# Chemical118/TREW

Hardware: NVIDIA B200
Metric: Gbases/s for trew short 5 32 at 1/2/4/8 B200; % of HBM roofline (higher is better)
Workload: dtype u64

## Files before the change

### trew_b200/csrc/device_ctx.cu

```cuda
#include <algorithm>
#include <chrono>
#include <cstdarg>
#include <cstdio>
#include <cstdlib>
#include <cstring>
#include <string>
#include <thread>
#include <vector>

#include <cuda_runtime.h>

#include "host_internal.h"
#include "scan_kernels.cuh"

using namespace trew;

namespace {

struct SlotRes {
    void* h_buf = nullptr;
    void* d_buf = nullptr;
    unsigned char* h_inv = nullptr;
    unsigned char* d_inv = nullptr;
    size_t inv_cap = 0;
    unsigned int* h_keys = nullptr;
    unsigned int* d_survivors = nullptr;
    unsigned int* d_counters = nullptr;
    unsigned char* d_scratch = nullptr;
    size_t scratch_bytes = 0;
    size_t survivors_cap = 0;
    cudaStream_t stream = nullptr;
    cudaEvent_t ev_start = nullptr, ev_done = nullptr;
    bool in_flight = false;
};

struct RangeInfo { uint32_t r0, r1; uint64_t bases; uint32_t max_len; };

}

struct trew_resident {
    void* d_buf = nullptr;
    DevBatch batch{};
    uint32_t n_reads = 0, n_units = 0, max_read_len = 0;
    uint64_t bases = 0;
    unsigned int* d_survivors = nullptr;
    unsigned int* d_counters = nullptr;
    unsigned char* d_scratch = nullptr;
    size_t scratch_bytes = 0;
    cudaEvent_t ev[4] = {nullptr, nullptr, nullptr, nullptr};
    bool ev_pending = false;
};

struct trew_ctx {
    trew_config cfg{};
    int sm_count = 0;
    LaunchPlan plan{};
    cudaStream_t aux_stream = nullptr;
    cudaEvent_t ev_join = nullptr;
    int resident_streams = 1;
    uint64_t resident_seq = 0;
    DevCfg dcfg{};
    size_t n_slots = 0;
    unsigned int* d_error = nullptr;
    unsigned short* d_thr = nullptr;
    unsigned long long* d_total_surv = nullptr;
    std::vector<SlotRes> slots;
    size_t next_slot = 0;
    size_t staging_bytes = 0;
    cudaStream_t main_stream = nullptr;
    cudaEvent_t ev_a = nullptr, ev_b = nullptr;
    trew_entry* d_entries = nullptr; size_t d_entries_cap = 0;
    trew_entry* d_sorted = nullptr; size_t d_sorted_cap = 0;
    trew_entry* d_concat = nullptr; size_t d_concat_cap = 0;
    bool sorted_valid = false;
    void* d_sort_tmp = nullptr; size_t sort_tmp_bytes = 0;
    unsigned int* d_n = nullptr;
    uint64_t n_export = 0;
    bool export_valid = false;
    trew_stats stats{};
    Pool* pool = nullptr;
    bool own_pool = true;
    std::string err;
    std::vector<RangeInfo> ranges_tmp;
    unsigned int keys_seen = 0;
    bool sparse_val = true;
    unsigned int exact_flags = 0;
    std::vector<InvList> inv_tmp;
    IngestScratch ingest;
    cudaEvent_t ev_t0 = nullptr, ev_t1 = nullptr;
    double screen_ms = 0, decide_ms = 0, exact_ms = 0; uint64_t n_prof_scans = 0;
    std::vector<trew_resident*> pending_prof;
    void* h_export = nullptr; size_t h_export_bytes = 0;
    unsigned int report_min = 0;
    trew_entry* d_filtered = nullptr; size_t d_filtered_cap = 0;
};

namespace {

int fail(trew_ctx* c, int status, const char* fmt, ...) {
    char buf[512];
    va_list ap; va_start(ap, fmt); vsnprintf(buf, sizeof(buf), fmt, ap); va_end(ap);
    if (c) c->err = buf;
    return status;
}

#define CK(call)                                                                                         \
    do {                                                                                                 \
        cudaError_t e_ = (call);                                                                         \
        if (e_ != cudaSuccess) return fail(ctx, TREW_ERR_CUDA, "%s: %s", #call, cudaGetErrorString(e_)); \
    } while (0)

void build_thr(double B, std::vector<unsigned short>& thr) {
    thr.assign(kThrTableSize, 0xFFFF);
    for (int T = 1; T < kThrTableSize; T++) {
        int lo = 0, hi = T;
        while (lo < hi) {
            int mid = (lo + hi) / 2;
            if ((double)mid / (double)T >= B) hi = mid; else lo = mid + 1;
        }
        thr[T] = (unsigned short)lo;
    }
}

int run_cap_for(const trew_config& cfg, uint32_t max_read_len) {
    uint32_t w = max_read_len;
    if (cfg.mode == TREW_MODE_LONG) w = std::min<uint32_t>(max_read_len, 2u * (uint32_t)cfg.slice_length);
    w = std::min<uint32_t>(w, (uint32_t)kMaxWindow);
    return (int)std::max<uint32_t>((w + 2 + 7) & ~7u, 32u);
}

constexpr unsigned int kLongThreadCap = 32768;

size_t scratch_need(const trew_ctx* ctx, uint32_t max_read_len, uint32_t n_units, unsigned int* stride, size_t* long_off,
                    unsigned int* s_cap, unsigned int* max_slices) {
    unsigned int st = 16;
    if (ctx->cfg.mode == TREW_MODE_LONG) st = 2u * (max_read_len / (uint32_t)ctx->cfg.slice_length + 2u);
    st = (st + 15u) & ~15u;
    *stride = st;
    size_t bytes = ((size_t)st * (size_t)exact_warps_total(ctx->sm_count) + 255) & ~(size_t)255;
    *long_off = bytes;
    *s_cap = 0; *max_slices = 0;
    if (long_thread_path_applies(ctx->dcfg) && (ctx->exact_flags & 16u)) {
        *s_cap = std::min<unsigned int>(std::max<unsigned int>(n_units, 1u), kLongThreadCap);
        *max_slices = max_read_len / (uint32_t)ctx->cfg.slice_length + 1u;
        bytes += long_thread_scratch_bytes(*s_cap, *max_slices);
    }
    return bytes;
}

constexpr int kScanCounters = 8;

static int env_blocks_thread() {
    static const int v = [] { const char* e = getenv("TREW_GRID_THREAD"); int x = e && *e ? atoi(e) : 0; return x > 0 ? x : 0; }();
    return v;
}

int launch_scan(trew_ctx* ctx, const DevBatch& b, uint32_t n_units, uint32_t max_read_len, unsigned int* d_survivors,
                unsigned int* d_counters, unsigned char** d_scratch, size_t* scratch_bytes, cudaStream_t st,
                cudaEvent_t* ev = nullptr) {
    unsigned int stride, s_cap, max_slices;
    size_t long_off;
    size_t need = scratch_need(ctx, max_read_len, n_units, &stride, &long_off, &s_cap, &max_slices);
    if (need > *scratch_bytes) {
        if (*d_scratch) { CK(cudaStreamSynchronize(st)); CK(cudaFree(*d_scratch)); *d_scratch = nullptr; }
        CK(cudaMalloc((void**)d_scratch, need));
        *scratch_bytes = need;
    }
    ctx->export_valid = false;
    CK(cudaMemsetAsync(d_counters, 0, kScanCounters * sizeof(unsigned int), st));
    if (ev) CK(cudaEventRecord(ev[0], st));
    const bool thread_path = thread_path_applies(ctx->dcfg, max_read_len) && !(ctx->exact_flags & 4u) && n_units < (1u << 28);
    launch_filter(ctx->dcfg, b, n_units, max_read_len, d_survivors + n_units, d_counters + 2, d_survivors, d_counters, ctx->plan, st,
                  ev ? ev[1] : nullptr, thread_path ? d_survivors + n_units - 1 : nullptr, thread_path ? d_counters + 4 : nullptr,
                  d_counters + 7);
    if (ev) CK(cudaEventRecord(ev[2], st));
    ExactArgs a{};
    a.survivors = d_survivors; a.n_survivors = d_counters; a.work_counter = d_counters + 1;
    a.slice_scratch = *d_scratch; a.slice_scratch_stride = stride; a.run_cap = run_cap_for(ctx->cfg, max_read_len);
    a.total_survivors = ctx->d_total_surv;
    a.packed_probes = n_units < (1u << 28) ? 1 : 0;
    a.exp_flags = ctx->exact_flags;
    if (thread_path) {
        unsigned int* hard = d_survivors + n_units;
        launch_exact_thread(ctx->dcfg, b, d_survivors, d_counters, a.packed_probes, hard, d_counters + 3, ctx->d_total_surv,
                            ctx->sm_count, env_blocks_thread(), d_counters + 6, st);
        ExactArgs ab = a;
        ab.survivors = d_survivors + n_units - 1; ab.reverse = 1; ab.n_survivors = d_counters + 4;
        launch_exact(ctx->dcfg, b, ab, ctx->plan, st);
        a.survivors = hard; a.n_survivors = d_counters + 3; a.work_counter = d_counters + 5; a.total_survivors = nullptr;
        ctx->stats.kernel_launches += 2;
    } else if (s_cap > 0 && n_units < (1u << 28)) {
        unsigned int* hard = d_survivors + n_units;
        launch_long_thread(ctx->dcfg, b, d_survivors, d_counters, a.packed_probes, s_cap, max_slices, *d_scratch + long_off, hard,
                           d_counters + 3, ctx->d_total_surv, ctx->sm_count, st);
        a.survivors = hard; a.n_survivors = d_counters + 3; a.total_survivors = nullptr;
        ctx->stats.kernel_launches += 3;
    }
    launch_exact(ctx->dcfg, b, a, ctx->plan, st);
    if (ev) CK(cudaEventRecord(ev[3], st));
    CK(cudaGetLastError());
    ctx->stats.kernel_launches += 3;
    return TREW_OK;
}

int retire_slot(trew_ctx* ctx, SlotRes& s) {
    if (!s.in_flight) return TREW_OK;
    CK(cudaEventSynchronize(s.ev_done));
    float ms = 0.f;
    CK(cudaEventElapsedTime(&ms, s.ev_start, s.ev_done));
    ctx->stats.device_ms += ms;
    s.in_flight = false;
    ctx->keys_seen = std::max(ctx->keys_seen, *s.h_keys);
    return TREW_OK;
}

int export_sorted(trew_ctx* ctx, uint64_t* n_out);
int check_device_error(trew_ctx* ctx);

int grow_table_to(trew_ctx* ctx, size_t min_slots) {
    size_t new_slots = ctx->n_slots;
    while (new_slots < ((size_t)1 << 28) && new_slots < min_slots) new_slots <<= 1;
    if (new_slots == ctx->n_slots) return TREW_OK;
    uint64_t n = 0;
    int rc = export_sorted(ctx, &n);
    if (rc) return rc;
    Slot* d_new = nullptr;
    CK(cudaMalloc((void**)&d_new, new_slots * sizeof(Slot)));
    CK(cudaMemsetAsync(d_new, 0, new_slots * sizeof(Slot), ctx->main_stream));
    CK(cudaMemsetAsync(ctx->d_error + 1, 0, sizeof(unsigned int), ctx->main_stream));
    Slot* d_old = ctx->dcfg.slots;
    ctx->dcfg.slots = d_new; ctx->dcfg.slot_mask = (unsigned int)(new_slots - 1); ctx->n_slots = new_slots;
    launch_merge_entries(ctx->dcfg, ctx->d_entries, (unsigned int)n, ctx->main_stream);
    CK(cudaGetLastError());
    CK(cudaStreamSynchronize(ctx->main_stream));
    CK(cudaFree(d_old));
    ctx->stats.kernel_launches += 1;
    ctx->keys_seen = (unsigned int)n;
    for (auto& sl : ctx->slots) *sl.h_keys = (unsigned int)n;
    return check_device_error(ctx);
}

int maybe_grow_table(trew_ctx* ctx) {
    if ((size_t)ctx->keys_seen * 16 <= ctx->n_slots) return TREW_OK;
    unsigned int keys = 0;
    CK(cudaMemcpy(&keys, ctx->d_error + 1, sizeof(keys), cudaMemcpyDeviceToHost));
    ctx->keys_seen = std::max(ctx->keys_seen, keys);
    if ((size_t)keys * 4 <= ctx->n_slots) return TREW_OK;
    return grow_table_to(ctx, (size_t)keys * 8);
}

int submit_ranges(trew_ctx* ctx, const ChunkView& cv, const RangeInfo* rg, int n_ranges) {
    uint64_t total_bases = 0; uint32_t max_len = 0;
    for (int i = 0; i < n_ranges; i++) { total_bases += rg[i].bases; max_len = std::max(max_len, rg[i].max_len); }
    const uint32_t n = n_ranges ? rg[n_ranges - 1].r1 - rg[0].r0 : 0u;
    if (n == 0) return TREW_OK;
    SlotRes& s = ctx->slots[ctx->next_slot];
    ctx->next_slot = (ctx->next_slot + 1) % ctx->slots.size();
    static const bool trace = getenv("TREW_SUBMIT_TRACE") != nullptr;
    auto now = [] { return std::chrono::duration<double, std::milli>(std::chrono::steady_clock::now().time_since_epoch()).count(); };
    const double t0 = trace ? now() : 0;
    int rc = retire_slot(ctx, s);
    if (rc) return rc;
    const double t1 = trace ? now() : 0;
    if ((rc = maybe_grow_table(ctx)) != TREW_OK) return rc;
    const double t2 = now();
    BatchView v;
    batch_layout(s.h_buf, n, total_bases, &v);
    std::vector<uint64_t> bit0((size_t)n_ranges);
    uint64_t acc = 0;
    for (int i = 0; i < n_ranges; i++) { bit0[i] = acc; acc += rg[i].bases; }
    v.bit_off[n] = (uint32_t)total_bases;
    const uint32_t first = rg[0].r0;
    std::vector<uint64_t> side_flat((size_t)3 * n_ranges);
    uint64_t (*side)[3] = (uint64_t (*)[3])side_flat.data();
    if (ctx->inv_tmp.size() < (size_t)n_ranges) ctx->inv_tmp.resize((size_t)n_ranges);
    auto pack = [&](bool list) {
        pack_prepare(bit0.data(), n_ranges, total_bases, v);
        ctx->pool->run(n_ranges, [&](int i) {
            pack_chunk_range(cv, rg[i].r0, rg[i].r1, rg[i].r0 - first, bit0[i], v, side[i], list ? &ctx->inv_tmp[(size_t)i] : nullptr, list,
                             rg[i].bases);
        });
        pack_fixup(bit0.data(), side, n_ranges, v);
    };
    size_t n_inv = 0;
    bool sparse = ctx->sparse_val;
    pack(sparse);
    const bool tail_pad = (total_bases & 31) != 0;
    if (sparse) {
        n_inv = tail_pad ? 1 : 0;
        for (int i = 0; i < n_ranges; i++) n_inv += ctx->inv_tmp[(size_t)i].size();
        if (n_inv > s.inv_cap) { sparse = false; pack(false); }
    }

    const double t3 = now();
    ctx->stats.host_pack_bytes += total_bases; ctx->stats.host_pack_ms += t3 - t2;
    CK(cudaEventRecord(s.ev_start, s.stream));
    const size_t head_bytes = (size_t)((char*)v.val - (char*)s.h_buf);
    unsigned int* d_val = (unsigned int*)((char*)s.d_buf + head_bytes);
    size_t sent = v.bytes;
    if (sparse) {
        std::vector<size_t> at((size_t)n_ranges + 1, 0);
        for (int i = 0; i < n_ranges; i++) at[(size_t)i + 1] = at[(size_t)i] + ctx->inv_tmp[(size_t)i].bytes();
        ctx->pool->run(n_ranges, [&](int i) {
            const InvList& l = ctx->inv_tmp[(size_t)i];
            if (l.bytes()) memcpy(s.h_inv + at[(size_t)i], l.buf.get(), l.bytes());
        });
        if (tail_pad) inv_record(s.h_inv + at[(size_t)n_ranges], (uint32_t)total_bases, (1ULL << (32 - (total_bases & 31))) - 1ULL);
        const size_t ones_words = (size_t)((total_bases + 31) / 32);
        CK(cudaMemsetAsync(d_val, 0xFF, ones_words * 4, s.stream));
        CK(cudaMemsetAsync(d_val + ones_words, 0, (v.plane_words - ones_words) * 4, s.stream));
        CK(cudaMemcpyAsync(s.d_buf, s.h_buf, head_bytes, cudaMemcpyHostToDevice, s.stream));
        if (n_inv) {
            CK(cudaMemcpyAsync(s.d_inv, s.h_inv, n_inv * kInvRecBytes, cudaMemcpyHostToDevice, s.stream));
            launch_clear_invalid(d_val, (const unsigned int*)s.d_inv, (unsigned int)n_inv, s.stream);
            ctx->stats.kernel_launches += 1;
        }
        sent = head_bytes + n_inv * kInvRecBytes;
    } else {
        CK(cudaMemcpyAsync(s.d_buf, s.h_buf, v.bytes, cudaMemcpyHostToDevice, s.stream));
    }
    DevBatch b{};
    b.n_reads = n;
    b.bit_off = (const unsigned int*)s.d_buf;
    b.hi = (const unsigned int*)((char*)s.d_buf + ((char*)v.hi - (char*)s.h_buf));
    b.lo = b.hi + v.plane_words; b.val = d_val;
    uint32_t n_units = ctx->cfg.mode == TREW_MODE_PAIR ? n / 2 : n;
    rc = launch_scan(ctx, b, n_units, max_len, s.d_survivors, s.d_counters, &s.d_scratch, &s.scratch_bytes, s.stream);
    if (rc) return rc;
    CK(cudaMemcpyAsync(s.h_keys, ctx->d_error + 1, sizeof(unsigned int), cudaMemcpyDeviceToHost, s.stream));
    CK(cudaEventRecord(s.ev_done, s.stream));
    s.in_flight = true;
    ctx->stats.reads += n; ctx->stats.bases += total_bases; ctx->stats.units += n_units; ctx->stats.h2d_bytes += sent;
    if (trace)
        fprintf(stderr, "[submit] %u reads: wait slot %.3f ms, table check %.3f ms, pack %.3f ms, enqueue %.3f ms\n", n, t1 - t0, t2 - t1,
                t3 - t2, now() - t3);
    return TREW_OK;
}

int submit_chunk_view(trew_ctx* ctx, const ChunkView& cv, uint32_t n) {
    if (n == 0) return TREW_OK;
    const uint32_t unit = cv.unit;
    const uint32_t n_units = n / unit;
    uint64_t span = 0;
    for (int sd = 0; sd < (int)unit; sd++) {
        const int32_t* l = cv.locs[sd];
        span += (uint64_t)std::max<int64_t>(0, (int64_t)l[2 * (size_t)(n_units - 1) + 1] - l[0] + 1);
    }
    uint64_t by_size = span / std::max<uint64_t>(1, ctx->staging_bytes / 16) + 1;
    uint32_t n_ranges = (uint32_t)std::min<uint64_t>(n_units, std::max<uint64_t>(by_size, (uint64_t)ctx->pool->size() * 4));
    auto& rg = ctx->ranges_tmp;
    rg.resize(n_ranges);
    for (uint32_t i = 0; i < n_ranges; i++) {
        rg[i].r0 = (uint32_t)((uint64_t)n_units * i / n_ranges) * unit;
        rg[i].r1 = (uint32_t)((uint64_t)n_units * (i + 1) / n_ranges) * unit;
    }
    ctx->pool->run((int)n_ranges, [&](int i) { chunk_stats(cv, rg[i].r0, rg[i].r1, &rg[i].bases, &rg[i].max_len); });
    uint32_t mx = 0;
    for (auto& r : rg) mx = std::max(mx, r.max_len);
    if (ctx->cfg.mode == TREW_MODE_SHORT && mx > 1000)
        return fail(ctx, TREW_ERR_TOO_LONG, "%s", trew_status_string(TREW_ERR_TOO_LONG));
    if (ctx->cfg.mode == TREW_MODE_PAIR && mx > (uint32_t)kMaxWindow) return fail(ctx, TREW_ERR_TOO_LONG, "paired read longer than %d", kMaxWindow);
    const size_t cap = ctx->slots[0].survivors_cap;
    uint32_t g = 0;
    while (g < n_ranges) {
        uint32_t h = g; uint64_t bases = 0; uint64_t reads = 0;
        while (h < n_ranges) {
            uint64_t nb = bases + rg[h].bases, nr = reads + (rg[h].r1 - rg[h].r0);
            if (batch_bytes((uint32_t)nr, nb) > ctx->staging_bytes || nr > cap || nb >= 0xfffff000ULL) break;
            bases = nb; reads = nr; h++;
        }
        if (h == g) {
            if (rg[g].r1 - rg[g].r0 <= unit)
                return fail(ctx, TREW_ERR_ARG, "a single read/pair (%llu bases) does not fit a staging buffer of %zu bytes",
                            (unsigned long long)rg[g].bases, ctx->staging_bytes);
            std::vector<RangeInfo> fine;
            for (uint32_t r = rg[g].r0; r < rg[g].r1; r += unit) {
                RangeInfo f{r, r + unit, 0, 0};
                chunk_stats(cv, f.r0, f.r1, &f.bases, &f.max_len);
                fine.push_back(f);
            }
            size_t a = 0;
            while (a < fine.size()) {
                size_t e = a; uint64_t fb = 0, fr = 0;
                while (e < fine.size()) {
                    uint64_t nb = fb + fine[e].bases, nr = fr + unit;
                    if (batch_bytes((uint32_t)nr, nb) > ctx->staging_bytes || nr > cap || nb >= 0xfffff000ULL) break;
                    fb = nb; fr = nr; e++;
                }
                if (e == a)
                    return fail(ctx, TREW_ERR_ARG, "a single read/pair (%llu bases) does not fit a staging buffer of %zu bytes",
                                (unsigned long long)fine[a].bases, ctx->staging_bytes);
                std::vector<RangeInfo> merged;
                size_t per = std::max<size_t>(1, (e - a) / (size_t)ctx->pool->size());
                for (size_t i = a; i < e; i += per) {
                    RangeInfo m{fine[i].r0, 0, 0, 0};
                    for (size_t j = i; j < std::min(e, i + per); j++) { m.r1 = fine[j].r1; m.bases += fine[j].bases; m.max_len = std::max(m.max_len, fine[j].max_len); }
                    merged.push_back(m);
                }
                int rc = submit_ranges(ctx, cv, merged.data(), (int)merged.size());
                if (rc) return rc;
                a = e;
            }
            g++;
            continue;
        }
        int rc = submit_ranges(ctx, cv, rg.data() + g, (int)(h - g));
        if (rc) return rc;
        g = h;
    }
    return TREW_OK;
}

int collect_prof(trew_ctx* ctx) {
    for (trew_resident* r : ctx->pending_prof) {
        if (!r->ev_pending) continue;
        CK(cudaEventSynchronize(r->ev[3]));
        float a = 0, b = 0, c = 0;
        CK(cudaEventElapsedTime(&a, r->ev[0], r->ev[1]));
        CK(cudaEventElapsedTime(&b, r->ev[1], r->ev[2]));
        CK(cudaEventElapsedTime(&c, r->ev[2], r->ev[3]));
        ctx->screen_ms += a; ctx->decide_ms += b; ctx->exact_ms += c; ctx->n_prof_scans++;
        ctx->stats.device_ms += a + b + c;
        r->ev_pending = false;
    }
    ctx->pending_prof.clear();
    return TREW_OK;
}

int join_aux(trew_ctx* ctx) {
    if (ctx->resident_streams != 2) return TREW_OK;
    CK(cudaEventRecord(ctx->ev_join, ctx->aux_stream));
    CK(cudaStreamWaitEvent(ctx->main_stream, ctx->ev_join, 0));
    return TREW_OK;
}

int fork_aux(trew_ctx* ctx) {
    if (ctx->resident_streams != 2) return TREW_OK;
    CK(cudaEventRecord(ctx->ev_join, ctx->main_stream));
    CK(cudaStreamWaitEvent(ctx->aux_stream, ctx->ev_join, 0));
    return TREW_OK;
}

int check_device_error(trew_ctx* ctx) {
    unsigned int e = 0;
    CK(cudaMemcpy(&e, ctx->d_error, sizeof(e), cudaMemcpyDeviceToHost));
    if (e == 3u) return fail(ctx, TREW_ERR_TABLE_FULL, "device count table full (%zu slots): raise table_log2_slots", ctx->n_slots);
    if (e) return fail(ctx, TREW_ERR_CUDA, "device error flag %u", e);
    return TREW_OK;
}

}

extern "C" {

int trew_abi_version(void) { return TREW_ABI_VERSION; }

const char* trew_status_string(int status) {
    switch (status) {
        case TREW_OK: return "ok";
        case TREW_ERR_ARG: return "bad argument";
        case TREW_ERR_CUDA: return "CUDA failure";
        case TREW_ERR_TABLE_FULL: return "device count table full";
        case TREW_ERR_TOO_LONG: return "This mode is designed for short-read sequencing. Please use 'trew long'.";
        case TREW_ERR_IO: return "file I/O error";
        case TREW_ERR_PAIRING: return "paired-end record mismatch";
        case TREW_ERR_NOMEM: return "memory allocation failure";
        default: return "unknown status";
    }
}

static thread_local std::string g_create_error;

static int default_host_threads(int asked) {
    return asked > 0 ? asked : (int)std::min(64u, std::max(1u, std::thread::hardware_concurrency()));
}

const char* trew_dev_last_error(const trew_ctx* ctx) { return ctx ? ctx->err.c_str() : g_create_error.c_str(); }

static int create_ctx(const trew_config* cfg, trew_ctx** out, std::string& g_create_error, Pool* shared_pool) {
    if (!cfg || !out) return TREW_ERR_ARG;
    *out = nullptr;
    g_create_error.clear();
    auto bad_arg = [&](const char* msg) { g_create_error = msg; return TREW_ERR_ARG; };
    if (cfg->mode < 0 || cfg->mode > 2) return bad_arg("mode must be TREW_MODE_SHORT, _PAIR or _LONG");
    if (cfg->min_mer < 3 || cfg->max_mer > 64 || cfg->min_mer > cfg->max_mer) return bad_arg("need 3 <= MIN_MER <= MAX_MER <= 64");
    if (!(0 < cfg->low_baseline && cfg->low_baseline <= 1) || !(0 < cfg->high_baseline && cfg->high_baseline <= 1) ||
        cfg->low_baseline > cfg->high_baseline) return bad_arg("need 0 < LOW_BASELINE <= HIGH_BASELINE <= 1");
    if (cfg->mode == TREW_MODE_LONG && cfg->slice_length > 0 && cfg->slice_length < 2 * cfg->max_mer)
        return bad_arg("SLICE_LENGTH must be greater than or equal to twice of MAX_MER.");
    if (cfg->mode == TREW_MODE_LONG && cfg->slice_length > 512)
        return bad_arg("SLICE_LENGTH above 512 is not supported by the GPU path (a slice of up to 2*SLICE_LENGTH-1 bases must fit "
                       "a 1023-base window); use -s 512 or less.");
    trew_ctx* ctx = new trew_ctx();
    ctx->cfg = *cfg;
    if (ctx->cfg.slice_length <= 0) ctx->cfg.slice_length = 150;
    auto bail = [&](int rc) { g_create_error = ctx->err; trew_dev_destroy(ctx); return rc; };
#define CKC(call)                                                                                   \
    do {                                                                                            \
        cudaError_t e_ = (call);                                                                    \
        if (e_ != cudaSuccess) { fail(ctx, TREW_ERR_CUDA, "%s: %s", #call, cudaGetErrorString(e_)); return bail(TREW_ERR_CUDA); } \
    } while (0)
    const bool timing = getenv("TREW_CLI_TIMING") != nullptr;
    auto now = [] { return std::chrono::duration<double, std::milli>(std::chrono::steady_clock::now().time_since_epoch()).count(); };
    double t_prev = now();
    auto lap = [&](const char* what) {
        if (!timing) return;
        const double t = now();
        fprintf(stderr, "[trew] create, device %d: %s %.1f ms\n", cfg->device, what, t - t_prev);
        t_prev = t;
    };
    int ndev = 0;
    CKC(cudaGetDeviceCount(&ndev));
    lap("driver init");
    if (cfg->device < 0 || cfg->device >= ndev) { fail(ctx, TREW_ERR_CUDA, "no CUDA device %d (found %d)", cfg->device, ndev); return bail(TREW_ERR_CUDA); }
    CKC(cudaSetDevice(cfg->device));
    cudaDeviceProp prop;
    CKC(cudaGetDeviceProperties(&prop, cfg->device));
    ctx->sm_count = prop.multiProcessorCount;
    ctx->plan = default_launch_plan(ctx->sm_count);
    {
        auto env_int = [](const char* name, int dflt) { const char* e = getenv(name); return e && *e ? atoi(e) : dflt; };
        int v;
        if ((v = env_int("TREW_GRID_SCREEN", 0)) > 0) ctx->plan.screen_blocks = ctx->sm_count * v;
        if ((v = env_int("TREW_GRID_DECIDE", 0)) > 0) ctx->plan.decide_blocks = ctx->sm_count * v;
        if ((v = env_int("TREW_GRID_EXACT", 0)) > 0) ctx->plan.exact_blocks = std::min(ctx->plan.exact_blocks, ctx->sm_count * v);
        ctx->resident_streams = env_int("TREW_RESIDENT_STREAMS", 1) >= 2 ? 2 : 1;
        ctx->sparse_val = env_int("TREW_DENSE_VAL", 0) == 0;
        ctx->exact_flags = (unsigned int)env_int("TREW_EXACT_FLAGS", 0);
    }
    int lg = cfg->table_log2_slots > 0 ? cfg->table_log2_slots : 22;
    if (lg < 10 || lg > 28) { fail(ctx, TREW_ERR_ARG, "table_log2_slots out of range"); return bail(TREW_ERR_ARG); }
    ctx->n_slots = (size_t)1 << lg;
    Slot* d_slots = nullptr;
    CKC(cudaMalloc((void**)&d_slots, ctx->n_slots * sizeof(Slot)));
    CKC(cudaMemset(d_slots, 0, ctx->n_slots * sizeof(Slot)));
    lap("primary context + count table");
    CKC(cudaMalloc((void**)&ctx->d_error, 2 * sizeof(unsigned int)));
    CKC(cudaMemset(ctx->d_error, 0, 2 * sizeof(unsigned int)));
    CKC(cudaMalloc((void**)&ctx->d_total_surv, sizeof(unsigned long long)));
    CKC(cudaMemset(ctx->d_total_surv, 0, sizeof(unsigned long long)));
    std::vector<unsigned short> thr;
    build_thr(cfg->low_baseline, thr);
    std::vector<unsigned short> thr_hi;
    build_thr(cfg->high_baseline, thr_hi);
    CKC(cudaMalloc((void**)&ctx->d_thr, 2 * thr.size() * sizeof(unsigned short)));
    CKC(cudaMemcpy(ctx->d_thr, thr.data(), thr.size() * sizeof(unsigned short), cudaMemcpyHostToDevice));
    CKC(cudaMemcpy(ctx->d_thr + thr.size(), thr_hi.data(), thr_hi.size() * sizeof(unsigned short), cudaMemcpyHostToDevice));
    ctx->dcfg.mode = cfg->mode; ctx->dcfg.min_mer = cfg->min_mer; ctx->dcfg.max_mer = cfg->max_mer;
    ctx->dcfg.slice_len = ctx->cfg.slice_length; ctx->dcfg.low = cfg->low_baseline; ctx->dcfg.high = cfg->high_baseline;
    ctx->dcfg.slots = d_slots; ctx->dcfg.slot_mask = (unsigned int)(ctx->n_slots - 1);
    ctx->dcfg.error_flag = ctx->d_error; ctx->dcfg.thr_low = ctx->d_thr; ctx->dcfg.thr_high = ctx->d_thr + kThrTableSize;
    CKC(prepare_exact(kMaxWindow + 9));
    lap("kernel attributes (module load)");
    CKC(cudaStreamCreateWithFlags(&ctx->main_stream, cudaStreamNonBlocking));
    CKC(cudaStreamCreateWithFlags(&ctx->aux_stream, cudaStreamNonBlocking));
    CKC(cudaEventCreateWithFlags(&ctx->ev_join, cudaEventDisableTiming));
    CKC(cudaEventCreate(&ctx->ev_a));
    CKC(cudaEventCreate(&ctx->ev_b));
    CKC(cudaEventCreate(&ctx->ev_t0));
    CKC(cudaEventCreate(&ctx->ev_t1));
    ctx->staging_bytes = cfg->staging_bytes ? (size_t)cfg->staging_bytes : ((size_t)64 << 20);
    int ns = cfg->n_staging > 0 ? cfg->n_staging : 3;
    ctx->slots.resize((size_t)ns);
    for (auto& s : ctx->slots) {
        CKC(cudaHostAlloc(&s.h_buf, ctx->staging_bytes, cudaHostAllocDefault));
        CKC(cudaMalloc(&s.d_buf, ctx->staging_bytes));
        s.inv_cap = ctx->staging_bytes / 8 / kInvRecBytes;
        CKC(cudaHostAlloc((void**)&s.h_inv, (s.inv_cap + 1) * kInvRecBytes, cudaHostAllocDefault));
        CKC(cudaMalloc((void**)&s.d_inv, (s.inv_cap + 1) * kInvRecBytes));
        CKC(cudaHostAlloc((void**)&s.h_keys, sizeof(unsigned int), cudaHostAllocDefault));
        *s.h_keys = 0;
        s.survivors_cap = ctx->staging_bytes / 8;
        CKC(cudaMalloc((void**)&s.d_survivors, 2 * s.survivors_cap * sizeof(unsigned int)));
        CKC(cudaMalloc((void**)&s.d_counters, kScanCounters * sizeof(unsigned int)));
        CKC(cudaStreamCreateWithFlags(&s.stream, cudaStreamNonBlocking));
        CKC(cudaEventCreate(&s.ev_start));
        CKC(cudaEventCreate(&s.ev_done));
    }
    CKC(cudaMalloc((void**)&ctx->d_n, sizeof(unsigned int)));
    lap("staging ring (pinned + device buffers)");
    if (shared_pool) { ctx->pool = shared_pool; ctx->own_pool = false; }
    else ctx->pool = new Pool(default_host_threads(cfg->host_threads));
#undef CKC
    *out = ctx;
    return TREW_OK;
}

int trew_dev_create(const trew_config* cfg, trew_ctx** out) { return create_ctx(cfg, out, g_create_error, nullptr); }

void trew_dev_destroy(trew_ctx* ctx) {
    if (!ctx) return;
    cudaSetDevice(ctx->cfg.device);
    cudaDeviceSynchronize();
    for (auto& s : ctx->slots) {
        if (s.h_buf) cudaFreeHost(s.h_buf);
        if (s.d_buf) cudaFree(s.d_buf);
        if (s.h_inv) cudaFreeHost(s.h_inv);
        if (s.d_inv) cudaFree(s.d_inv);
        if (s.h_keys) cudaFreeHost(s.h_keys);
        if (s.d_survivors) cudaFree(s.d_survivors);
        if (s.d_counters) cudaFree(s.d_counters);
        if (s.d_scratch) cudaFree(s.d_scratch);
        if (s.stream) cudaStreamDestroy(s.stream);
        if (s.ev_start) cudaEventDestroy(s.ev_start);
        if (s.ev_done) cudaEventDestroy(s.ev_done);
    }
    if (ctx->dcfg.slots) cudaFree(ctx->dcfg.slots);
    if (ctx->d_error) cudaFree(ctx->d_error);
    if (ctx->d_thr) cudaFree(ctx->d_thr);
    if (ctx->d_total_surv) cudaFree(ctx->d_total_surv);
    if (ctx->d_entries) cudaFree(ctx->d_entries);
    if (ctx->d_sorted) cudaFree(ctx->d_sorted);
    if (ctx->d_concat) cudaFree(ctx->d_concat);
    if (ctx->d_filtered) cudaFree(ctx->d_filtered);
    if (ctx->d_sort_tmp) cudaFree(ctx->d_sort_tmp);
    if (ctx->d_n) cudaFree(ctx->d_n);
    if (ctx->h_export) cudaFreeHost(ctx->h_export);
    if (ctx->main_stream) cudaStreamDestroy(ctx->main_stream);
    if (ctx->aux_stream) cudaStreamDestroy(ctx->aux_stream);
    if (ctx->ev_join) cudaEventDestroy(ctx->ev_join);
    if (ctx->ev_a) cudaEventDestroy(ctx->ev_a);
    if (ctx->ev_b) cudaEventDestroy(ctx->ev_b);
    if (ctx->ev_t0) cudaEventDestroy(ctx->ev_t0);
    if (ctx->ev_t1) cudaEventDestroy(ctx->ev_t1);
    if (ctx->own_pool) delete ctx->pool;
    delete ctx;
}

int trew_dev_submit_chunk(trew_ctx* ctx, const char* buffer1, const int32_t* locs1, uint32_t n1,
                          const char* buffer2, const int32_t* locs2, uint32_t n2) {
    if (!ctx) return TREW_ERR_ARG;
    CK(cudaSetDevice(ctx->cfg.device));
    const bool pair = ctx->cfg.mode == TREW_MODE_PAIR;
    if (pair ? (!buffer2 && n2) : (buffer2 != nullptr || n2 != 0)) return fail(ctx, TREW_ERR_ARG, "second chunk only in pair mode");
    if ((n1 && (!buffer1 || !locs1)) || (n2 && !locs2)) return fail(ctx, TREW_ERR_ARG, "null chunk");
    ChunkView cv{{buffer1, buffer2}, {locs1, locs2}, {nullptr, nullptr}, pair ? 2u : 1u};
    const uint32_t n = pair ? 2u * std::min(n1, n2) : n1;
    if (n == 0) return TREW_OK;
    for (int sd = 0; sd < (pair ? 2 : 1); sd++) {
        const int32_t* l = cv.locs[sd];
        uint32_t cnt = pair ? n / 2 : n;
        int32_t last = l[2 * (size_t)(cnt - 1) + 1];
        if (last >= l[2 * (size_t)(cnt - 1)]) cv.end[sd] = cv.buf[sd] + last + 1;
    }
    return submit_chunk_view(ctx, cv, n);
}

int trew_dev_submit_packed(trew_ctx* ctx, const trew_batch* batch) {
    if (!ctx || !batch) return TREW_ERR_ARG;
    CK(cudaSetDevice(ctx->cfg.device));
    uint32_t n = batch->n_reads;
    if (n == 0) return TREW_OK;
    uint64_t bases = batch->bit_off[n];
    size_t bytes = batch_bytes(n, bases);
    if (bytes > ctx->staging_bytes || n > ctx->slots[0].survivors_cap)
        return fail(ctx, TREW_ERR_ARG, "packed batch (%zu bytes) larger than a staging buffer (%zu)", bytes, ctx->staging_bytes);
    if (batch->bit_off[0] != 0) return fail(ctx, TREW_ERR_ARG, "bit_off[0] must be 0");
    SlotRes& s = ctx->slots[ctx->next_slot];
    ctx->next_slot = (ctx->next_slot + 1) % ctx->slots.size();
    int rc = retire_slot(ctx, s);
    if (rc) return rc;
    BatchView v;
    batch_layout(s.h_buf, n, bases, &v);
    size_t words = (size_t)((bases + 31) / 32);
    memcpy(v.bit_off, batch->bit_off, (size_t)(n + 1) * 4);
    const uint32_t* src[3] = {batch->hi, batch->lo, batch->val};
    uint32_t* dst[3] = {v.hi, v.lo, v.val};
    ctx->pool->run(3, [&](int i) {
        memcpy(dst[i], src[i], words * 4);
        memset(dst[i] + words, 0, (v.plane_words - words) * 4);
    });
    CK(cudaEventRecord(s.ev_start, s.stream));
    CK(cudaMemcpyAsync(s.d_buf, s.h_buf, v.bytes, cudaMemcpyHostToDevice, s.stream));
    DevBatch b{};
    b.n_reads = n;
    b.bit_off = (const unsigned int*)s.d_buf;
    b.hi = (const unsigned int*)((char*)s.d_buf + ((char*)v.hi - (char*)s.h_buf));
    b.lo = b.hi + v.plane_words; b.val = b.lo + v.plane_words;
    uint32_t n_units = ctx->cfg.mode == TREW_MODE_PAIR ? n / 2 : n;
    rc = launch_scan(ctx, b, n_units, batch->max_read_len, s.d_survivors, s.d_counters, &s.d_scratch, &s.scratch_bytes, s.stream);
    if (rc) return rc;
    CK(cudaMemcpyAsync(s.h_keys, ctx->d_error + 1, sizeof(unsigned int), cudaMemcpyDeviceToHost, s.stream));
    CK(cudaEventRecord(s.ev_done, s.stream));
    s.in_flight = true;
    ctx->stats.reads += n; ctx->stats.bases += bases; ctx->stats.units += n_units; ctx->stats.h2d_bytes += v.bytes;
    return TREW_OK;
}

int trew_dev_upload(trew_ctx* ctx, const trew_batch* batch, trew_resident** out) {
    if (!ctx || !batch || !out) return TREW_ERR_ARG;
    CK(cudaSetDevice(ctx->cfg.device));
    uint32_t n = batch->n_reads;
    uint64_t bases = n ? batch->bit_off[n] : 0;
    trew_resident* r = new trew_resident();
    size_t bytes = batch_bytes(n, bases);
    std::vector<char> tmp(bytes, 0);
    BatchView v;
    batch_layout(tmp.data(), n, bases, &v);
    size_t words = (size_t)((bases + 31) / 32);
    if (n) {
        memcpy(v.bit_off, batch->bit_off, (size_t)(n + 1) * 4);
        memcpy(v.hi, batch->hi, words * 4); memcpy(v.lo, batch->lo, words * 4); memcpy(v.val, batch->val, words * 4);
    }
    CK(cudaMalloc(&r->d_buf, bytes));
    CK(cudaMemcpy(r->d_buf, tmp.data(), bytes, cudaMemcpyHostToDevice));
    r->batch.n_reads = n;
    r->batch.bit_off = (const unsigned int*)r->d_buf;
    r->batch.hi = (const unsigned int*)((char*)r->d_buf + ((char*)v.hi - tmp.data()));
    r->batch.lo = r->batch.hi + v.plane_words; r->batch.val = r->batch.lo + v.plane_words;
    r->n_reads = n; r->n_units = ctx->cfg.mode == TREW_MODE_PAIR ? n / 2 : n; r->max_read_len = batch->max_read_len; r->bases = bases;
    CK(cudaMalloc((void**)&r->d_survivors, 2 * (size_t)std::max<uint32_t>(r->n_units, 1) * sizeof(unsigned int)));
    CK(cudaMalloc((void**)&r->d_counters, kScanCounters * sizeof(unsigned int)));
    *out = r;
    return TREW_OK;
}

int trew_dev_scan_resident(trew_ctx* ctx, const trew_resident* rb) {
    if (!ctx || !rb) return TREW_ERR_ARG;
    CK(cudaSetDevice(ctx->cfg.device));
    trew_resident* r = const_cast<trew_resident*>(rb);
    ctx->keys_seen = std::max<unsigned int>(ctx->keys_seen, (unsigned int)(ctx->n_slots / 16 + 1));
    if (r->ev_pending) { int rc0 = collect_prof(ctx); if (rc0) return rc0; }
    if (!r->ev[0]) for (int i = 0; i < 4; i++) CK(cudaEventCreate(&r->ev[i]));
    cudaStream_t st = (ctx->resident_streams == 2 && (ctx->resident_seq++ & 1)) ? ctx->aux_stream : ctx->main_stream;
    CK(cudaEventRecord(ctx->ev_a, st));
    int rc = launch_scan(ctx, r->batch, r->n_units, r->max_read_len, r->d_survivors, r->d_counters, &r->d_scratch,
                         &r->scratch_bytes, st, r->ev);
    r->ev_pending = true; ctx->pending_prof.push_back(r);
    if (rc) return rc;
    CK(cudaEventRecord(ctx->ev_b, st));
    ctx->stats.reads += r->n_reads; ctx->stats.bases += r->bases; ctx->stats.units += r->n_units;
    return TREW_OK;
}

void trew_dev_free_resident(trew_ctx* ctx, trew_resident* r) {
    if (!r) return;
    if (ctx) { cudaSetDevice(ctx->cfg.device); cudaStreamSynchronize(ctx->main_stream); cudaStreamSynchronize(ctx->aux_stream); collect_prof(ctx); }
    for (int i = 0; i < 4; i++) if (r->ev[i]) cudaEventDestroy(r->ev[i]);
    if (r->d_buf) cudaFree(r->d_buf);
    if (r->d_survivors) cudaFree(r->d_survivors);
    if (r->d_counters) cudaFree(r->d_counters);
    if (r->d_scratch) cudaFree(r->d_scratch);
    delete r;
}

int trew_dev_sync(trew_ctx* ctx) {
    if (!ctx) return TREW_ERR_ARG;
    CK(cudaSetDevice(ctx->cfg.device));
    for (auto& s : ctx->slots) { int rc = retire_slot(ctx, s); if (rc) return rc; }
    { int rc = join_aux(ctx); if (rc) return rc; }
    CK(cudaStreamSynchronize(ctx->main_stream));
    { int rc = collect_prof(ctx); if (rc) return rc; }
    return check_device_error(ctx);
}

}

namespace {

int export_entries(trew_ctx* ctx, bool need_sorted, const trew_entry** out, uint64_t* n_out) {
    int rc = trew_dev_sync(ctx);
    if (rc) return rc;
    if (!ctx->export_valid) {
        unsigned int n = 0;
        for (int pass = 0; pass < 2; pass++) {
            CK(cudaMemsetAsync(ctx->d_n, 0, sizeof(unsigned int), ctx->main_stream));
            if (pass == 0 && ctx->d_entries_cap == 0) {
                ctx->d_entries_cap = (size_t)1 << 20;
                CK(cudaMalloc((void**)&ctx->d_entries, ctx->d_entries_cap * sizeof(trew_entry)));
            }
            launch_compact(ctx->dcfg.slots, (unsigned int)ctx->n_slots, ctx->d_entries, ctx->d_n, ctx->main_stream,
                           (unsigned int)ctx->d_entries_cap);
            CK(cudaGetLastError());
            ctx->stats.kernel_launches += 1;
            CK(cudaMemcpyAsync(&n, ctx->d_n, sizeof(n), cudaMemcpyDeviceToHost, ctx->main_stream));
            CK(cudaStreamSynchronize(ctx->main_stream));
            if (n <= ctx->d_entries_cap) break;
            CK(cudaFree(ctx->d_entries));
            ctx->d_entries = nullptr;
            ctx->d_entries_cap = (size_t)n + n / 4 + 1024;
            CK(cudaMalloc((void**)&ctx->d_entries, ctx->d_entries_cap * sizeof(trew_entry)));
        }
        ctx->n_export = n;
        ctx->export_valid = true;
        ctx->sorted_valid = false;
    }
    const unsigned int n = (unsigned int)ctx->n_export;
    if (need_sorted && !ctx->sorted_valid) {
        if (n > ctx->d_sorted_cap) {
            if (ctx->d_sorted) CK(cudaFree(ctx->d_sorted));
            ctx->d_sorted = nullptr;
            ctx->d_sorted_cap = std::max<size_t>((size_t)n + n / 4 + 1024, (size_t)1 << 20);
            CK(cudaMalloc((void**)&ctx->d_sorted, ctx->d_sorted_cap * sizeof(trew_entry)));
        }
        if (n == 1) CK(cudaMemcpyAsync(ctx->d_sorted, ctx->d_entries, sizeof(trew_entry), cudaMemcpyDeviceToDevice, ctx->main_stream));
        if (n > 1) {
            const bool wide = ctx->cfg.max_mer > 32;
            size_t need = 0;
            CK(sort_entries_radix(ctx->d_entries, ctx->d_sorted, n, wide, nullptr, &need, ctx->main_stream));
            if (need > ctx->sort_tmp_bytes) {
                if (ctx->d_sort_tmp) CK(cudaFree(ctx->d_sort_tmp));
                ctx->d_sort_tmp = nullptr;
                ctx->sort_tmp_bytes = need + need / 4;
                CK(cudaMalloc(&ctx->d_sort_tmp, ctx->sort_tmp_bytes));
            }
            size_t bytes = ctx->sort_tmp_bytes;
            CK(sort_entries_radix(ctx->d_entries, ctx->d_sorted, n, wide, ctx->d_sort_tmp, &bytes, ctx->main_stream));
            ctx->stats.kernel_launches += wide ? 11 : 8;
        }
        CK(cudaStreamSynchronize(ctx->main_stream));
        ctx->sorted_valid = true;
    }
    if (out) *out = need_sorted ? ctx->d_sorted : ctx->d_entries;
    if (n_out) *n_out = n;
    return TREW_OK;
}

int export_sorted(trew_ctx* ctx, uint64_t* n_out) { return export_entries(ctx, false, nullptr, n_out); }

int rows_to_host(trew_ctx* ctx, const trew_entry* d_rows, uint64_t n, const trew_entry** entries, uint64_t* n_entries) {
    size_t need_host = (size_t)n * sizeof(trew_entry) + 64;
    if (need_host > ctx->h_export_bytes) {
        if (ctx->h_export) CK(cudaFreeHost(ctx->h_export));
        ctx->h_export = nullptr;
        size_t cap = std::max(need_host * 2, (size_t)1 << 20);
        CK(cudaHostAlloc(&ctx->h_export, cap, cudaHostAllocDefault));
        ctx->h_export_bytes = cap;
    }
    if (n) {
        CK(cudaMemcpyAsync(ctx->h_export, d_rows, n * sizeof(trew_entry), cudaMemcpyDeviceToHost, ctx->main_stream));
        CK(cudaStreamSynchronize(ctx->main_stream));
    }
    ctx->stats.d2h_bytes += n * sizeof(trew_entry) + 4;
    if (entries) *entries = (const trew_entry*)ctx->h_export;
    if (n_entries) *n_entries = n;
    return TREW_OK;
}

int finish_rows(trew_ctx* ctx, const trew_entry* d_in, uint64_t n_in, bool combine, const trew_entry** entries, uint64_t* n_entries) {
    auto ensure = [&](trew_entry** buf, size_t* cap, size_t want) -> int {
        if (want <= *cap) return TREW_OK;
        if (*buf) CK(cudaFree(*buf));
        *buf = nullptr;
        *cap = std::max<size_t>(want + want / 4 + 1024, (size_t)1 << 20);
        CK(cudaMalloc((void**)buf, *cap * sizeof(trew_entry)));
        return TREW_OK;
    };
    auto ensure_tmp = [&](size_t need) -> int {
        if (need <= ctx->sort_tmp_bytes) return TREW_OK;
        CK(cudaStreamSynchronize(ctx->main_stream));
        if (ctx->d_sort_tmp) CK(cudaFree(ctx->d_sort_tmp));
        ctx->d_sort_tmp = nullptr;
        ctx->sort_tmp_bytes = need + need / 4;
        CK(cudaMalloc(&ctx->d_sort_tmp, ctx->sort_tmp_bytes));
        return TREW_OK;
    };
    int rc;
    if ((rc = ensure(&ctx->d_sorted, &ctx->d_sorted_cap, (size_t)n_in)) != TREW_OK) return rc;
    if ((rc = ensure(&ctx->d_filtered, &ctx->d_filtered_cap, (size_t)n_in)) != TREW_OK) return rc;
    ctx->sorted_valid = false;
    const bool wide = ctx->cfg.max_mer > 32;
    const trew_entry* src = d_in;
    unsigned int n = (unsigned int)n_in;
    if (ctx->report_min > 0 && n > 0) {
        size_t need = 0;
        CK(filter_report_rows(src, n, ctx->report_min, ctx->d_filtered, ctx->d_n, nullptr, &need, ctx->main_stream));
        if ((rc = ensure_tmp(need)) != TREW_OK) return rc;
        size_t bytes = ctx->sort_tmp_bytes;
        CK(filter_report_rows(src, n, ctx->report_min, ctx->d_filtered, ctx->d_n, ctx->d_sort_tmp, &bytes, ctx->main_stream));
        CK(cudaMemcpyAsync(&n, ctx->d_n, sizeof(n), cudaMemcpyDeviceToHost, ctx->main_stream));
        CK(cudaStreamSynchronize(ctx->main_stream));
        ctx->stats.kernel_launches += 5;
        src = ctx->d_filtered;
    }
    if (n == 1) CK(cudaMemcpyAsync(ctx->d_sorted, src, sizeof(trew_entry), cudaMemcpyDeviceToDevice, ctx->main_stream));
    if (n > 1) {
        size_t need = 0;
        CK(sort_entries_radix(src, ctx->d_sorted, n, wide, nullptr, &need, ctx->main_stream));
        if ((rc = ensure_tmp(need)) != TREW_OK) return rc;
        size_t bytes = ctx->sort_tmp_bytes;
        CK(sort_entries_radix(src, ctx->d_sorted, n, wide, ctx->d_sort_tmp, &bytes, ctx->main_stream));
        ctx->stats.kernel_launches += wide ? 11 : 8;
    }
    const trew_entry* rows = ctx->d_sorted;
    if (combine && n > 0) {
        size_t need = 0;
        CK(combine_sorted_rows(ctx->d_sorted, n, ctx->d_filtered, ctx->d_n, nullptr, &need, ctx->main_stream));
        if ((rc = ensure_tmp(need)) != TREW_OK) return rc;
        size_t bytes = ctx->sort_tmp_bytes;
        CK(combine_sorted_rows(ctx->d_sorted, n, ctx->d_filtered, ctx->d_n, ctx->d_sort_tmp, &bytes, ctx->main_stream));
        CK(cudaMemcpyAsync(&n, ctx->d_n, sizeof(n), cudaMemcpyDeviceToHost, ctx->main_stream));
        CK(cudaStreamSynchronize(ctx->main_stream));
        ctx->stats.kernel_launches += 3;
        rows = ctx->d_filtered;
    }
    return rows_to_host(ctx, rows, n, entries, n_entries);
}

}

extern "C" {

int trew_dev_export_device(trew_ctx* ctx, const trew_entry** d_entries, uint64_t* n_entries) {
    if (!ctx) return TREW_ERR_ARG;
    return export_entries(ctx, true, d_entries, n_entries);
}

int trew_dev_finish(trew_ctx* ctx, const trew_entry** entries, uint64_t* n_entries) {
    if (!ctx) return TREW_ERR_ARG;
    uint64_t n = 0;
    const trew_entry* d_rows = nullptr;
    if (ctx->report_min > 0) {
        int rc = export_entries(ctx, false, &d_rows, &n);
        if (rc) return rc;
        return finish_rows(ctx, d_rows, n, false, entries, n_entries);
    }
    int rc = export_entries(ctx, true, &d_rows, &n);
    if (rc) return rc;
    return rows_to_host(ctx, d_rows, n, entries, n_entries);
}

int trew_dev_finish_merged(trew_ctx* ctx, const trew_entry* const* d_lists, const uint64_t* n_rows, uint32_t n_lists,
                           const trew_entry** entries, uint64_t* n_entries) {
    if (!ctx || (n_lists && (!d_lists || !n_rows))) return TREW_ERR_ARG;
    uint64_t n0 = 0;
    const trew_entry* d_own = nullptr;
    int rc = export_entries(ctx, false, &d_own, &n0);
    if (rc) return rc;
    uint64_t total = n0;
    for (uint32_t i = 0; i < n_lists; i++) total += n_rows[i];
    if (total > 0xfffffff0ULL) return fail(ctx, TREW_ERR_ARG, "too many rows to merge (%llu)", (unsigned long long)total);
    auto ensure = [&](trew_entry** buf, size_t* cap) -> int {
        if (total <= *cap) return TREW_OK;
        if (*buf) CK(cudaFree(*buf));
        *buf = nullptr;
        *cap = std::max<size_t>((size_t)total + total / 4 + 1024, (size_t)1 << 20);
        CK(cudaMalloc((void**)buf, *cap * sizeof(trew_entry)));
        return TREW_OK;
    };
    if ((rc = ensure(&ctx->d_concat, &ctx->d_concat_cap)) != TREW_OK) return rc;
    uint64_t at = 0;
    if (n0) CK(cudaMemcpyAsync(ctx->d_concat, d_own, n0 * sizeof(trew_entry), cudaMemcpyDeviceToDevice, ctx->main_stream));
    at += n0;
    for (uint32_t i = 0; i < n_lists; i++) {
        if (n_rows[i]) CK(cudaMemcpyAsync(ctx->d_concat + at, d_lists[i], n_rows[i] * sizeof(trew_entry), cudaMemcpyDeviceToDevice, ctx->main_stream));
        at += n_rows[i];
    }
    return finish_rows(ctx, ctx->d_concat, total, true, entries, n_entries);
}

int trew_dev_export_rows(trew_ctx* ctx, trew_entry* d_rows, uint64_t capacity_rows, uint64_t* n_rows) {
    if (!ctx || !n_rows) return TREW_ERR_ARG;
    uint64_t n = 0;
    const trew_entry* d_src = nullptr;
    int rc = export_entries(ctx, false, &d_src, &n);
    if (rc) return rc;
    *n_rows = n;
    if (!d_rows) return TREW_OK;
    if (n > capacity_rows) return fail(ctx, TREW_ERR_ARG, "row buffer too small: %llu rows, capacity %llu", (unsigned long long)n,
                                       (unsigned long long)capacity_rows);
    if (n) CK(cudaMemcpyAsync(d_rows, d_src, n * sizeof(trew_entry), cudaMemcpyDeviceToDevice, ctx->main_stream));
    CK(cudaStreamSynchronize(ctx->main_stream));
    return TREW_OK;
}

int trew_dev_merge_rows(trew_ctx* ctx, const trew_entry* d_rows, uint64_t n_rows) {
    if (!ctx || (n_rows && !d_rows) || n_rows > 0xffffffffULL) return TREW_ERR_ARG;
    CK(cudaSetDevice(ctx->cfg.device));
    ctx->export_valid = false;
    ctx->keys_seen = std::max<unsigned int>(ctx->keys_seen, (unsigned int)(ctx->n_slots / 16 + 1));
    launch_merge_entries(ctx->dcfg, d_rows, (unsigned int)n_rows, ctx->main_stream);
    CK(cudaGetLastError());
    ctx->stats.kernel_launches += n_rows ? 1 : 0;
    return TREW_OK;
}

int trew_dev_set_report_filter(trew_ctx* ctx, uint32_t min_total) {
    if (!ctx) return TREW_ERR_ARG;
    ctx->report_min = min_total;
    return TREW_OK;
}

int trew_dev_reserve(trew_ctx* ctx, uint64_t expected_new_keys) {
    if (!ctx) return TREW_ERR_ARG;
    int rc = trew_dev_sync(ctx);
    if (rc) return rc;
    unsigned int keys = 0;
    CK(cudaMemcpy(&keys, ctx->d_error + 1, sizeof(keys), cudaMemcpyDeviceToHost));
    const uint64_t want = ((uint64_t)keys + expected_new_keys) * 4;
    if (want <= ctx->n_slots) return TREW_OK;
    return grow_table_to(ctx, (size_t)std::min<uint64_t>(want, (uint64_t)1 << 28));
}

int trew_dev_reset(trew_ctx* ctx) {
    if (!ctx) return TREW_ERR_ARG;
    int rc = trew_dev_sync(ctx);
    if (rc && rc != TREW_ERR_TABLE_FULL) return rc;
    ctx->export_valid = false;
    CK(cudaMemsetAsync(ctx->dcfg.slots, 0, ctx->n_slots * sizeof(Slot), ctx->main_stream));
    CK(cudaMemsetAsync(ctx->d_error, 0, 2 * sizeof(unsigned int), ctx->main_stream));
    CK(cudaStreamSynchronize(ctx->main_stream));
    ctx->keys_seen = 0;
    for (auto& sl : ctx->slots) *sl.h_keys = 0;
    return TREW_OK;
}

int trew_dev_get_stats(trew_ctx* ctx, trew_stats* out) {
    if (!ctx || !out) return TREW_ERR_ARG;
    CK(cudaSetDevice(ctx->cfg.device));
    unsigned long long s = 0;
    CK(cudaMemcpy(&s, ctx->d_total_surv, sizeof(s), cudaMemcpyDeviceToHost));
    ctx->stats.survivors = s;
    *out = ctx->stats;
    return TREW_OK;
}

int trew_dev_last_resident_ms(trew_ctx* ctx, float* ms) {
    if (!ctx || !ms) return TREW_ERR_ARG;
    CK(cudaEventSynchronize(ctx->ev_b));
    CK(cudaEventElapsedTime(ms, ctx->ev_a, ctx->ev_b));
    return TREW_OK;
}

int trew_dev_timer_start(trew_ctx* ctx) {
    if (!ctx) return TREW_ERR_ARG;
    CK(cudaSetDevice(ctx->cfg.device));
    CK(cudaEventRecord(ctx->ev_t0, ctx->main_stream));
    return fork_aux(ctx);
}

int trew_dev_timer_stop(trew_ctx* ctx, float* ms) {
    if (!ctx || !ms) return TREW_ERR_ARG;
    CK(cudaSetDevice(ctx->cfg.device));
    { int rc = join_aux(ctx); if (rc) return rc; }
    CK(cudaEventRecord(ctx->ev_t1, ctx->main_stream));
    CK(cudaEventSynchronize(ctx->ev_t1));
    CK(cudaEventElapsedTime(ms, ctx->ev_t0, ctx->ev_t1));
    return TREW_OK;
}

int trew_dev_kernel_times(trew_ctx* ctx, double* screen_ms, double* decide_ms, double* exact_ms, uint64_t* n_scans) {
    if (!ctx) return TREW_ERR_ARG;
    CK(cudaSetDevice(ctx->cfg.device));
    { int rc0 = join_aux(ctx); if (rc0) return rc0; }
    CK(cudaStreamSynchronize(ctx->main_stream));
    int rc = collect_prof(ctx);
    if (rc) return rc;
    if (screen_ms) *screen_ms = ctx->screen_ms;
    if (decide_ms) *decide_ms = ctx->decide_ms;
    if (exact_ms) *exact_ms = ctx->exact_ms;
    if (n_scans) *n_scans = ctx->n_prof_scans;
    ctx->screen_ms = ctx->decide_ms = ctx->exact_ms = 0; ctx->n_prof_scans = 0;
    return TREW_OK;
}

int trew_synth_resident(trew_ctx* ctx, uint64_t seed, uint32_t n_reads, uint32_t read_len, uint32_t tel_ppm,
                        uint32_t half_ppm, uint32_t n_ppm, uint32_t sub_ppm, trew_resident** out) {
    return trew_synth_resident_ex(ctx, seed, n_reads, read_len, tel_ppm, half_ppm, n_ppm, sub_ppm, 0, out);
}

int trew_synth_resident_ex(trew_ctx* ctx, uint64_t seed, uint32_t n_reads, uint32_t read_len, uint32_t tel_ppm,
                           uint32_t half_ppm, uint32_t n_ppm, uint32_t sub_ppm, uint32_t flavor, trew_resident** out) {
    if (!ctx || !out || read_len == 0 || flavor > 2 || (uint64_t)n_reads * read_len >= 0xfffff000ULL) return TREW_ERR_ARG;
    CK(cudaSetDevice(ctx->cfg.device));
    auto thr = [](uint32_t ppm) { return (unsigned int)(((unsigned long long)ppm << 32) / 1000000ULL); };
    uint64_t bases = (uint64_t)n_reads * read_len;
    size_t bytes = batch_bytes(n_reads, bases);
    trew_resident* r = new trew_resident();
    CK(cudaMalloc(&r->d_buf, bytes));
    BatchView v;
    batch_layout(r->d_buf, n_reads, bases, &v);
    launch_synth(seed, n_reads, read_len, thr(tel_ppm), thr(half_ppm), thr(n_ppm), thr(sub_ppm), flavor, v.bit_off, v.hi, v.lo, v.val,
                 v.plane_words, ctx->main_stream);
    CK(cudaGetLastError());
    CK(cudaStreamSynchronize(ctx->main_stream));
    r->batch.n_reads = n_reads; r->batch.bit_off = v.bit_off; r->batch.hi = v.hi; r->batch.lo = v.lo; r->batch.val = v.val;
    r->n_reads = n_reads; r->n_units = ctx->cfg.mode == TREW_MODE_PAIR ? n_reads / 2 : n_reads;
    r->max_read_len = read_len; r->bases = bases;
    CK(cudaMalloc((void**)&r->d_survivors, 2 * (size_t)std::max<uint32_t>(r->n_units, 1) * sizeof(unsigned int)));
    CK(cudaMalloc((void**)&r->d_counters, kScanCounters * sizeof(unsigned int)));
    *out = r;
    return TREW_OK;
}

int trew_dev_process_file(trew_ctx* ctx, const char* file1, int is_gz1, const char* file2, int is_gz2) {
    if (!ctx || !file1) return TREW_ERR_ARG;
    if ((ctx->cfg.mode == TREW_MODE_PAIR) != (file2 != nullptr)) return fail(ctx, TREW_ERR_ARG, "second file only in pair mode");
    const size_t chunk = 0;
    IngestResult r = ingest_file(ctx->cfg.mode, ctx->cfg.slice_length, file1, is_gz1 != 0, file2, is_gz2 != 0, chunk,
                                 [&](const char* b1, const std::vector<int32_t>& l1, const char* b2, const std::vector<int32_t>& l2) {
                                     return trew_dev_submit_chunk(ctx, b1, l1.data(), (uint32_t)(l1.size() / 2), b2,
                                                                  b2 ? l2.data() : nullptr, b2 ? (uint32_t)(l2.size() / 2) : 0u);
                                 },
                                 ctx->pool, &ctx->ingest);
    if (r.status != TREW_OK && r.status != TREW_ERR_CUDA && !r.message.empty()) ctx->err = r.message;
    return r.status;
}

}


struct trew_multi {
    std::vector<trew_ctx*> ctx;
    Pool* pool = nullptr;
    size_t next = 0;
    std::string err;
    std::vector<trew_entry*> d_peer; std::vector<size_t> d_peer_cap;
};

namespace {
int mfail(trew_multi* m, int status, const std::string& msg) { if (m) m->err = msg; return status; }
}

extern "C" {

int trew_multi_create(const trew_config* cfg, const int32_t* devices, int32_t n_devices, trew_multi** out) {
    if (!cfg || !out || n_devices < 0 || (n_devices > 0 && !devices)) return TREW_ERR_ARG;
    *out = nullptr;
    std::vector<int32_t> dev;
    if (n_devices == 0) {
        int nd = 0;
        if (cudaGetDeviceCount(&nd) != cudaSuccess || nd <= 0) { g_create_error = "no CUDA device"; return TREW_ERR_CUDA; }
        for (int i = 0; i < nd; i++) dev.push_back(i);
    } else {
        dev.assign(devices, devices + n_devices);
    }
    trew_multi* m = new trew_multi();
    m->pool = new Pool(default_host_threads(cfg->host_threads));
    int rc = TREW_OK;
    {
        std::vector<trew_ctx*> made(dev.size(), nullptr);
        std::vector<int> rcs(dev.size(), TREW_OK);
        std::vector<std::string> errs(dev.size());
        std::vector<std::thread> th;
        auto make = [&](size_t i) {
            trew_config c = *cfg;
            c.device = dev[i];
            rcs[i] = create_ctx(&c, &made[i], errs[i], m->pool);
        };
        for (size_t i = 1; i < dev.size(); i++) th.emplace_back(make, i);
        make(0);
        for (auto& t : th) t.join();
        for (size_t i = 0; i < dev.size(); i++) {
            if (rcs[i] != TREW_OK && rc == TREW_OK) { rc = rcs[i]; g_create_error = errs[i]; }
            if (made[i]) m->ctx.push_back(made[i]);
        }
    }
    if (rc != TREW_OK) { trew_multi_destroy(m); return rc; }
    for (size_t i = 1; i < m->ctx.size(); i++) {
        int can = 0;
        if (dev[i] != dev[0] && cudaDeviceCanAccessPeer(&can, dev[0], dev[i]) == cudaSuccess && can) {
            cudaSetDevice(dev[0]);
            cudaError_t e = cudaDeviceEnablePeerAccess(dev[i], 0);
            if (e != cudaSuccess) cudaGetLastError();
        }
    }
    m->d_peer.assign(m->ctx.size(), nullptr);
    m->d_peer_cap.assign(m->ctx.size(), 0);
    *out = m;
    return TREW_OK;
}

void trew_multi_destroy(trew_multi* m) {
    if (!m) return;
    if (!m->ctx.empty()) {
        cudaSetDevice(m->ctx[0]->cfg.device);
        for (trew_entry* p : m->d_peer) if (p) cudaFree(p);
    }
    for (trew_ctx* x : m->ctx) trew_dev_destroy(x);
    delete m->pool;
    delete m;
}

int trew_multi_device_count(const trew_multi* m) { return m ? (int)m->ctx.size() : 0; }

const char* trew_multi_last_error(const trew_multi* m) { return m ? m->err.c_str() : g_create_error.c_str(); }

trew_ctx* trew_multi_ctx(trew_multi* m, int32_t i) { return m && i >= 0 && (size_t)i < m->ctx.size() ? m->ctx[(size_t)i] : nullptr; }

int trew_multi_submit_chunk(trew_multi* m, const char* buffer1, const int32_t* locs1, uint32_t n1, const char* buffer2,
                            const int32_t* locs2, uint32_t n2) {
    if (!m) return TREW_ERR_ARG;
    trew_ctx* x = m->ctx[m->next];
    m->next = (m->next + 1) % m->ctx.size();
    int rc = trew_dev_submit_chunk(x, buffer1, locs1, n1, buffer2, locs2, n2);
    if (rc != TREW_OK) return mfail(m, rc, x->err);
    return TREW_OK;
}

int trew_multi_process_file(trew_multi* m, const char* file1, int is_gz1, const char* file2, int is_gz2) {
    if (!m || !file1) return TREW_ERR_ARG;
    trew_ctx* x0 = m->ctx[0];
    if ((x0->cfg.mode == TREW_MODE_PAIR) != (file2 != nullptr)) return mfail(m, TREW_ERR_ARG, "second file only in pair mode");
    IngestResult r = ingest_file(x0->cfg.mode, x0->cfg.slice_length, file1, is_gz1 != 0, file2, is_gz2 != 0, 0,
                                 [&](const char* b1, const std::vector<int32_t>& l1, const char* b2, const std::vector<int32_t>& l2) {
                                     return trew_multi_submit_chunk(m, b1, l1.data(), (uint32_t)(l1.size() / 2), b2, b2 ? l2.data() : nullptr,
                                                                    b2 ? (uint32_t)(l2.size() / 2) : 0u);
                                 },
                                 m->pool, &x0->ingest);
    if (r.status != TREW_OK && !r.message.empty()) m->err = r.message;
    return r.status;
}

int trew_multi_reset(trew_multi* m) {
    if (!m) return TREW_ERR_ARG;
    for (trew_ctx* x : m->ctx) { int rc = trew_dev_reset(x); if (rc != TREW_OK) return mfail(m, rc, x->err); }
    m->next = 0;
    return TREW_OK;
}

int trew_multi_finish(trew_multi* m, const trew_entry** entries, uint64_t* n_entries) {
    if (!m) return TREW_ERR_ARG;
    trew_ctx* x0 = m->ctx[0];
    const size_t nd = m->ctx.size();
    if (nd == 1) {
        int rc = trew_dev_finish(x0, entries, n_entries);
        return rc == TREW_OK ? rc : mfail(m, rc, x0->err);
    }
    std::vector<const trew_entry*> d_src(nd, nullptr);
    std::vector<uint64_t> n_rows(nd, 0);
    for (size_t i = 1; i < nd; i++) {
        int rc = export_entries(m->ctx[i], false, &d_src[i], &n_rows[i]);
        if (rc != TREW_OK) return mfail(m, rc, m->ctx[i]->err);
    }
    trew_ctx* ctx = x0;
    CK(cudaSetDevice(x0->cfg.device));
    std::vector<const trew_entry*> lists;
    std::vector<uint64_t> sizes;
    for (size_t i = 1; i < nd; i++) {
        if (n_rows[i] == 0) continue;
        if (n_rows[i] > m->d_peer_cap[i]) {
            if (m->d_peer[i]) CK(cudaFree(m->d_peer[i]));
            m->d_peer[i] = nullptr;
            m->d_peer_cap[i] = (size_t)n_rows[i] + n_rows[i] / 4 + 1024;
            CK(cudaMalloc((void**)&m->d_peer[i], m->d_peer_cap[i] * sizeof(trew_entry)));
        }
        CK(cudaMemcpyPeerAsync(m->d_peer[i], x0->cfg.device, d_src[i], m->ctx[i]->cfg.device, n_rows[i] * sizeof(trew_entry), x0->main_stream));
        lists.push_back(m->d_peer[i]);
        sizes.push_back(n_rows[i]);
    }
    int rc = trew_dev_finish_merged(x0, lists.data(), sizes.data(), (uint32_t)lists.size(), entries, n_entries);
    return rc == TREW_OK ? rc : mfail(m, rc, x0->err);
}

int trew_multi_set_report_filter(trew_multi* m, uint32_t min_total) {
    if (!m) return TREW_ERR_ARG;
    return trew_dev_set_report_filter(m->ctx[0], min_total);
}

int trew_multi_get_stats(trew_multi* m, trew_stats* out) {
    if (!m || !out) return TREW_ERR_ARG;
    trew_stats t;
    memset(&t, 0, sizeof(t));
    for (trew_ctx* x : m->ctx) {
        trew_stats s;
        int rc = trew_dev_get_stats(x, &s);
        if (rc != TREW_OK) return mfail(m, rc, x->err);
        t.reads += s.reads; t.bases += s.bases; t.units += s.units; t.survivors += s.survivors;
        t.kernel_launches += s.kernel_launches; t.h2d_bytes += s.h2d_bytes; t.d2h_bytes += s.d2h_bytes;
        t.host_pack_bytes += s.host_pack_bytes; t.host_pack_ms += s.host_pack_ms;
        t.device_ms = std::max(t.device_ms, s.device_ms);
    }
    *out = t;
    return TREW_OK;
}

}
```

### trew_b200/csrc/scan_kernels.cu

```cuda
#include "scan_kernels.cuh"
#include "exact_thread.cuh"

#include <cstdio>

namespace trew {

typedef unsigned int u32;
typedef unsigned long long u64;
typedef unsigned __int128 u128;


__device__ __forceinline__ u32 lane_id() { return threadIdx.x & 31; }

__device__ __forceinline__ u32 low_mask(int bits) {
    return bits >= 32 ? 0xffffffffu : ((1u << bits) - 1u);
}

__device__ __forceinline__ u32 prefix_xor32(u32 x) {
    x ^= x << 1; x ^= x << 2; x ^= x << 4; x ^= x << 8; x ^= x << 16;
    return x;
}

__device__ __forceinline__ u64 mix64(u64 x) {
    x ^= x >> 33; x *= 0xff51afd7ed558ccdULL; x ^= x >> 33; x *= 0xc4ceb9fe1a85ec53ULL; x ^= x >> 33;
    return x;
}


__device__ __noinline__ void table_add_impl(Slot* slots, u32 slot_mask, u32* error_flag, u32 meta, u64 lo, u64 hi, u64 cnt) {
#ifdef TREW_EXP_NOADD
    return;
#endif
    u64 h = mix64(lo ^ mix64(hi + 0x9e3779b97f4a7c15ULL * (u64)(meta + 1)));
    u32 i = (u32)h & slot_mask;
    for (u32 probe = 0; probe <= slot_mask; probe++, i = (i + 1) & slot_mask) {
        Slot* s = slots + i;
        const uint4 a = __ldcg(reinterpret_cast<const uint4*>(s)), c = __ldcg(reinterpret_cast<const uint4*>(s) + 1);
        u32 st = c.w;
        if (st == 2u) {
            if (c.z == meta && a.x == (u32)lo && a.y == (u32)(lo >> 32) && a.z == (u32)hi && a.w == (u32)(hi >> 32)) {
                atomicAdd(&s->count, cnt);
                return;
            }
            __threadfence();
            if (__ldcg(&s->meta) == meta && __ldcg(&s->seq_lo) == lo && __ldcg(&s->seq_hi) == hi) {
                atomicAdd(&s->count, cnt);
                return;
            }
            continue;
        }
        int outcome = 0;
        do {
            st = atomicCAS(&s->state, 0u, 1u);
            if (st == 0u) {
                s->seq_lo = lo; s->seq_hi = hi; s->meta = meta;
                __threadfence();
                atomicExch(&s->state, 2u);
                atomicAdd(&s->count, cnt);
                atomicAdd(error_flag + 1, 1u);
                outcome = 1;
            } else if (st == 2u) {
                __threadfence();
                if (__ldcg(&s->meta) == meta && __ldcg(&s->seq_lo) == lo && __ldcg(&s->seq_hi) == hi) {
                    atomicAdd(&s->count, cnt);
                    outcome = 1;
                } else outcome = 2;
            }
        } while (outcome == 0);
        if (outcome == 1) return;
    }
    atomicExch(error_flag, 3u);
}

__global__ void merge_entries_kernel(Slot* slots, u32 slot_mask, u32* error_flag, const trew_entry* __restrict__ e, u32 n) {
    for (u32 i = blockIdx.x * blockDim.x + threadIdx.x; i < n; i += gridDim.x * blockDim.x)
        table_add_impl(slots, slot_mask, error_flag, ((u32)e[i].table << 8) | (u32)e[i].k, e[i].seq_lo, e[i].seq_hi, e[i].count);
}

void launch_merge_entries(const DevCfg& cfg, const trew_entry* entries, unsigned int n, cudaStream_t stream) {
    if (n) merge_entries_kernel<<<(n + 255) / 256, 256, 0, stream>>>(cfg.slots, cfg.slot_mask, cfg.error_flag, entries, n);
}


__host__ __device__ inline u32 synth_hash(u64 seed, u64 a, u64 b) {
    u64 x = seed + 0x9e3779b97f4a7c15ULL * (a + 1) + 0xbf58476d1ce4e5b9ULL * (b + 1);
    x ^= x >> 30; x *= 0xbf58476d1ce4e5b9ULL; x ^= x >> 27; x *= 0x94d049bb133111ebULL; x ^= x >> 31;
    return (u32)(x >> 32);
}

__global__ void synth_kernel(u64 seed, u32 n_reads, u32 L, u32 tel_thr, u32 half_thr, u32 n_thr, u32 sub_thr, u32 flavor,
                             u32* __restrict__ bit_off, u32* __restrict__ hi, u32* __restrict__ lo, u32* __restrict__ val,
                             size_t plane_words) {
    const u64 total = (u64)n_reads * L;
    const size_t stride = (size_t)gridDim.x * blockDim.x;
    for (size_t i = (size_t)blockIdx.x * blockDim.x + threadIdx.x; i <= n_reads; i += stride) bit_off[i] = (u32)(i * L);
    const int unit_f[6] = {0, 0, 3, 1, 1, 1};
    const int unit_r[6] = {2, 2, 2, 0, 3, 3};
    for (size_t w = (size_t)blockIdx.x * blockDim.x + threadIdx.x; w < plane_words; w += stride) {
        u32 h = 0, l = 0, v = 0;
        for (int b = 0; b < 32; b++) {
            u64 pos = (u64)w * 32 + b;
            if (pos >= total) break;
            u64 r = pos / L; u32 j = (u32)(pos % L);
            const u64 frag = flavor == 1 ? r >> 1 : r;
            u32 kind = synth_hash(seed, frag, 0xffffffffULL);
            u32 aux = synth_hash(seed, frag, 0xfffffffeULL);
            u32 code = synth_hash(seed, r, j) & 3u;
            bool tel = kind < tel_thr;
            bool halfk = !tel && kind < tel_thr + half_thr;
            if (halfk) tel = ((aux >> 8) & 1u) ? (j < L / 2) : (j >= L / 2);
            if (flavor == 2 && tel) {
                u32 tl = 500u + synth_hash(seed, frag, 0xfffffffdULL) % 4501u;
                if (tl > L) tl = L;
                tel = ((aux >> 9) & 1u) ? (j < tl) : (j >= L - tl);
            }
            if (tel) {
                u32 phase = aux % 6u;
                bool rc = (((aux >> 4) & 1u) ^ (flavor == 1 ? (u32)(r & 1u) : 0u)) != 0u;
                u32 idx = (j + phase) % 6u;
                u32 c = rc ? unit_r[idx] : unit_f[idx];
                u32 sh = synth_hash(seed ^ 0x5555555555555555ULL, r, j);
                code = sh < sub_thr ? (sh >> 3) & 3u : c;
            }
            bool inval = synth_hash(seed ^ 0xaaaaaaaaaaaaaaaaULL, r, j) < n_thr;
            if (!inval) { v |= 1u << b; h |= (code >> 1) << b; l |= (code & 1u) << b; }
        }
        hi[w] = h; lo[w] = l; val[w] = v;
    }
}

void launch_synth(unsigned long long seed, unsigned int n_reads, unsigned int read_len, unsigned int tel_thr,
                  unsigned int half_thr, unsigned int n_thr, unsigned int sub_thr, unsigned int flavor, unsigned int* bit_off,
                  unsigned int* hi, unsigned int* lo, unsigned int* val, size_t plane_words, cudaStream_t stream) {
    synth_kernel<<<1184, 256, 0, stream>>>(seed, n_reads, read_len, tel_thr, half_thr, n_thr, sub_thr, flavor, bit_off, hi, lo, val,
                                            plane_words);
}


struct Probe { u32 pos; int wl, k0, k1; };

__device__ __forceinline__ int unit_probes(const DevCfg& c, const DevBatch& b, u32 u, Probe* p) {
    const int MINM = c.min_mer, MAXM = c.max_mer;
    int np = 0;
    if (c.mode == 0) {
        u32 b0 = __ldg(b.bit_off + u);
        int n = (int)(__ldg(b.bit_off + u + 1) - b0);
        if (n < 2 * MINM) return 0;
        if (n >= 4 * MINM) {
            int kmax = min(n / 4, MAXM);
            p[np++] = Probe{b0, n / 2, MINM, kmax};
            p[np++] = Probe{b0 + (u32)(n - (n + 1) / 2), (n + 1) / 2, MINM, kmax};
        }
        if (4 * MAXM > n) p[np++] = Probe{b0, n, max(n / 4 + 1, MINM), min(n / 2, MAXM)};
    } else if (c.mode == 1) {
        u32 a0 = __ldg(b.bit_off + 2 * u), a1 = __ldg(b.bit_off + 2 * u + 1), a2 = __ldg(b.bit_off + 2 * u + 2);
        int n1 = (int)(a1 - a0), n2 = (int)(a2 - a1);
        int n = min(n1, n2);
        if (n < 2 * MINM) return 0;
        if (n >= 4 * MINM) {
            int kmax = min(n / 4, MAXM);
            p[np++] = Probe{a0, n1 / 2, MINM, kmax};
            p[np++] = Probe{a1, n2 / 2, MINM, kmax};
        }
        if (4 * MAXM > n) {
            int lo = max(n / 4 + 1, MINM), hi = min(n / 2, MAXM);
            p[np++] = Probe{a0, n1, lo, hi};
            p[np++] = Probe{a1, n2, lo, hi};
        }
    } else {
        u32 b0 = __ldg(b.bit_off + u);
        int n = (int)(__ldg(b.bit_off + u + 1) - b0);
        const int SL = c.slice_len;
        if (n < SL) return 0;
        int snum = n / SL, mid = (snum + 1) / 2, bonus = n % SL;
        int l1 = SL + (1 == mid ? bonus : 0);
        p[np++] = Probe{b0, l1, MINM, MAXM};
        if (snum > 1) {
            int l2 = SL + (snum == mid ? bonus : 0);
            p[np++] = Probe{b0 + (u32)(n - l2), l2, MINM, MAXM};
        }
    }
    return np;
}


template <int NW>
__device__ __forceinline__ void load_bits(const u32* __restrict__ plane, u32 pos, u32 (&out)[NW]) {
    const u32* p = plane + (pos >> 5);
    u32 sh = pos & 31;
    u32 prev = __ldg(p);
#pragma unroll
    for (int j = 0; j < NW; j++) {
        u32 nxt = __ldg(p + j + 1);
        out[j] = __funnelshift_r(prev, nxt, sh);
        prev = nxt;
    }
}

template <int NW>
__device__ __forceinline__ void mask_bits(u32 (&x)[NW], int wl) {
#pragma unroll
    for (int j = 0; j < NW; j++) {
        int v = wl - 32 * j;
        x[j] &= v <= 0 ? 0u : low_mask(v);
    }
}

template <int NW>
__device__ __forceinline__ void prefix_xor_excl(const u32 (&in)[NW], u32 (&out)[NW]) {
    u32 carry = 0, prev_top = 0;
#pragma unroll
    for (int j = 0; j < NW; j++) {
        u32 inc = prefix_xor32(in[j]) ^ carry;
        out[j] = (inc << 1) | prev_top;
        prev_top = inc >> 31;
        carry = 0u - prev_top;
    }
}

template <int NW>
__device__ __forceinline__ void shr1(u32 (&x)[NW]) {
#pragma unroll
    for (int j = 0; j < NW; j++) x[j] = __funnelshift_r(x[j], j + 1 < NW ? x[j + 1] : 0u, 1);
}

template <int NW>
__device__ __forceinline__ void shr_var(const u32 (&in)[NW], int k, u32 (&out)[NW]) {
#pragma unroll
    for (int j = 0; j < NW; j++) out[j] = in[j];
    for (int s = k >> 5; s > 0; s--) {
#pragma unroll
        for (int j = 0; j < NW; j++) out[j] = j + 1 < NW ? out[j + 1] : 0u;
    }
    u32 r = k & 31;
#pragma unroll
    for (int j = 0; j < NW; j++) out[j] = __funnelshift_r(out[j], j + 1 < NW ? out[j + 1] : 0u, r);
}

template <int NW>
__device__ __forceinline__ void sliding_and(u32 (&a)[NW], int k) {
    u32 t[NW];
    int w = 1;
    while (2 * w <= k) {
        shr_var<NW>(a, w, t);
#pragma unroll
        for (int j = 0; j < NW; j++) a[j] &= t[j];
        w *= 2;
    }
    if (k > w) {
        shr_var<NW>(a, k - w, t);
#pragma unroll
        for (int j = 0; j < NW; j++) a[j] &= t[j];
    }
}

__device__ __forceinline__ void csa(u32 a, u32 b, u32 c, u32& s, u32& cy) {
    s = a ^ b ^ c;
    cy = (a & b) | (c & (a ^ b));
}

template <int NW>
__device__ __forceinline__ int popc_multi(const u32 (&x)[NW]) {
    if constexpr (NW == 1) return __popc(x[0]);
    else if constexpr (NW == 2) return __popc(x[0]) + __popc(x[1]);
    else if constexpr (NW == 3) {
        u32 s, c; csa(x[0], x[1], x[2], s, c);
        return __popc(s) + 2 * __popc(c);
    } else if constexpr (NW == 5) {
        u32 s1, c1, s2, c2; csa(x[0], x[1], x[2], s1, c1); csa(s1, x[3], x[4], s2, c2);
        return __popc(s2) + 2 * (__popc(c1) + __popc(c2));
    } else if constexpr (NW == 8) {
        u32 s1, c1, s2, c2, s3, c3, s4, c4;
        csa(x[0], x[1], x[2], s1, c1); csa(x[3], x[4], x[5], s2, c2); csa(s1, s2, x[6], s3, c3);
        csa(c1, c2, c3, s4, c4);
        return __popc(s3) + __popc(x[7]) + 2 * __popc(s4) + 4 * __popc(c4);
    } else {
        int t = 0;
#pragma unroll
        for (int j = 0; j < NW; j++) t += __popc(x[j]);
        return t;
    }
}

template <int NW>
__device__ __noinline__ bool probe_filter(const DevBatch& b, u32 pos, int wl, int k0, int k1,
                                          const unsigned short* __restrict__ thr) {
    u32 PH[NW], PL[NW], QH[NW], QL[NW], WV[NW];
    {
        u32 t[NW];
        load_bits<NW>(b.hi, pos, t); prefix_xor_excl<NW>(t, PH);
        load_bits<NW>(b.lo, pos, t); prefix_xor_excl<NW>(t, PL);
        load_bits<NW>(b.val, pos, WV); mask_bits<NW>(WV, wl);
    }
    shr_var<NW>(PH, k0, QH);
    shr_var<NW>(PL, k0, QL);
    sliding_and<NW>(WV, k0);
    u32 PA[NW];
    bool have_pa = false;
    for (int k = k0; k <= k1; k++) {
        u32 a[NW], bb[NW], c[NW];
#pragma unroll
        for (int j = 0; j < NW; j++) {
            u32 dh = QH[j] ^ PH[j], dl = QL[j] ^ PL[j];
            a[j] = dh & WV[j]; bb[j] = dl & WV[j]; c[j] = a[j] & dl;
        }
        int T = popc_multi<NW>(WV);
        if (T == 0) break;
        int cH = popc_multi<NW>(a), cL = popc_multi<NW>(bb), c11 = popc_multi<NW>(c);
        int c10 = cH - c11, c01 = cL - c11, c00 = T - cH - cL + c11;
        int U = max(max(c00, c01), max(c10, c11));
        int need = thr[T];
        if (U >= need) {
            u32 QA[NW];
            if (!have_pa) {
                u32 A[NW], t[NW];
                load_bits<NW>(b.hi, pos, A); load_bits<NW>(b.lo, pos, t);
#pragma unroll
                for (int j = 0; j < NW; j++) A[j] &= t[j];
                prefix_xor_excl<NW>(A, PA);
                have_pa = true;
            }
            shr_var<NW>(PA, k, QA);
            u32 x11[NW], x10[NW], x01[NW], x00[NW];
#pragma unroll
            for (int j = 0; j < NW; j++) {
                u32 da = QA[j] ^ PA[j];
                u32 dh = QH[j] ^ PH[j], dl = QL[j] ^ PL[j];
                x11[j] = c[j] & da; x10[j] = a[j] & ~dl & da; x01[j] = bb[j] & ~dh & da; x00[j] = WV[j] & ~dh & ~dl & da;
            }
            int n11 = popc_multi<NW>(x11), n10 = popc_multi<NW>(x10), n01 = popc_multi<NW>(x01), n00 = popc_multi<NW>(x00);
            int U2 = max(max(max(n11, c11 - n11), max(n10, c10 - n10)), max(max(n01, c01 - n01), max(n00, c00 - n00)));
            if (U2 >= need) return true;
        }
        shr1<NW>(QH); shr1<NW>(QL);
        u32 t[NW];
#pragma unroll
        for (int j = 0; j < NW; j++) t[j] = WV[j];
        shr1<NW>(t);
#pragma unroll
        for (int j = 0; j < NW; j++) WV[j] &= t[j];
    }
    return false;
}

template <int MAXNW>
__device__ __forceinline__ bool probe_dispatch(const DevBatch& b, const Probe& p, const unsigned short* thr) {
    if (p.k1 < p.k0) return false;
    int need_bits = p.wl + 1;
    if (need_bits <= 96) return probe_filter<3>(b, p.pos, p.wl, p.k0, p.k1, thr);
    if constexpr (MAXNW >= 5) { if (need_bits <= 160) return probe_filter<5>(b, p.pos, p.wl, p.k0, p.k1, thr); }
    if constexpr (MAXNW >= 8) { if (need_bits <= 256) return probe_filter<8>(b, p.pos, p.wl, p.k0, p.k1, thr); }
    return true;
}


constexpr u32 kPackC11 = 1u - (1u << 8) - (1u << 16) + (1u << 24);
constexpr u32 kPackH = (1u << 8) - (1u << 24);
constexpr u32 kPackL = (1u << 16) - (1u << 24);
#ifndef TREW_SCREEN_UNROLL
#define TREW_SCREEN_UNROLL 2
#endif
constexpr int kScreenUnroll = TREW_SCREEN_UNROLL;
constexpr int kFastMaxWl = 95;
constexpr int kFastTabSize = kFastMaxWl + 2;
constexpr int kProbeShift = 28;
constexpr int kMod4BelowWindows = 48;
constexpr int kThreadMinWindows = 36;

__device__ __forceinline__ uint4 fast_entry(int T, int need) {
    uint4 e = make_uint4(0u, 0u, 0u, 0u);
    if (T <= 0) return e;
    int T01 = min(T, 64);
    e.y = T >= 32 ? 0xffffffffu : ((1u << T) - 1u);
    e.z = T <= 32 ? 0u : (T >= 64 ? 0xffffffffu : ((1u << (T - 32)) - 1u));
    int np = need - (T - T01);
    if (np <= 0) e.x = 0x80808080u;
    else if (np > 64) e.x = (u32)T01 << 24;
    else e.x = ((u32)T01 << 24) + (u32)(128 - np) * 0x01010101u;
    return e;
}

template <int S>
__device__ __forceinline__ bool fast_span(const u32 (&ph)[5], const u32 (&pl)[5], int wl, int ka, int kb,
                                          const uint4* __restrict__ tab) {
    const uint4* tp = tab + (wl - ka + 1);
#pragma unroll (kScreenUnroll)
    for (int k = ka; k <= kb; k++, tp--) {
        const uint4 e = *tp;
        u32 qh0 = __funnelshift_r(ph[S], ph[S + 1], k), qh1 = __funnelshift_r(ph[S + 1], ph[S + 2], k);
        u32 ql0 = __funnelshift_r(pl[S], pl[S + 1], k), ql1 = __funnelshift_r(pl[S + 1], pl[S + 2], k);
        u32 a0 = (qh0 ^ ph[0]) & e.y, a1 = (qh1 ^ ph[1]) & e.z;
        u32 b0 = (ql0 ^ pl[0]) & e.y, b1 = (ql1 ^ pl[1]) & e.z;
        u32 x = e.x + (u32)(__popc(a0) + __popc(a1)) * kPackH + (u32)(__popc(b0) + __popc(b1)) * kPackL +
                (u32)(__popc(a0 & b0) + __popc(a1 & b1)) * kPackC11;
        if (x & 0x80808080u) return true;
    }
    return false;
}

__device__ __forceinline__ bool probe_is_fast(const Probe& p) { return p.wl <= kFastMaxWl && p.k1 <= 63 && p.k1 <= p.wl; }

__device__ __forceinline__ bool screen_probe(const DevBatch& b, const Probe& p, const uint4* __restrict__ tab) {
    if (p.k1 < p.k0) return false;
    if (!probe_is_fast(p)) return true;
    u32 t[3], full[3] = {0xffffffffu, 0xffffffffu, 0xffffffffu};
    mask_bits<3>(full, p.wl);
    load_bits<3>(b.val, p.pos, t);
    if ((((t[0] & full[0]) ^ full[0]) | ((t[1] & full[1]) ^ full[1]) | ((t[2] & full[2]) ^ full[2])) != 0u) return true;
    u32 ph[5], pl[5], q[3];
    load_bits<3>(b.hi, p.pos, t); mask_bits<3>(t, p.wl); prefix_xor_excl<3>(t, q);
    ph[0] = q[0]; ph[1] = q[1]; ph[2] = q[2]; ph[3] = 0u; ph[4] = 0u;
    load_bits<3>(b.lo, p.pos, t); mask_bits<3>(t, p.wl); prefix_xor_excl<3>(t, q);
    pl[0] = q[0]; pl[1] = q[1]; pl[2] = q[2]; pl[3] = 0u; pl[4] = 0u;
    int k0 = p.k0;
    if (k0 < 32) {
        if (fast_span<0>(ph, pl, p.wl, k0, min(p.k1, 31), tab)) return true;
        k0 = 32;
    }
    return p.k1 >= 32 && fast_span<1>(ph, pl, p.wl, k0, p.k1, tab);
}

constexpr int kFastMaxWlLong = 159;
constexpr int kFastTabSizeLong = kFastMaxWlLong + 2;
struct __align__(16) FastEntryLong { u32 base, m0, m1, m2, m3, pad0, pad1, pad2; };

__device__ __forceinline__ FastEntryLong fast_entry_long(int T, int need) {
    FastEntryLong e = {0u, 0u, 0u, 0u, 0u, 0u, 0u, 0u};
    if (T <= 0) return e;
    const int T01 = min(T, 128);
    u32 m[4];
#pragma unroll
    for (int j = 0; j < 4; j++) { int vb = T - 32 * j; m[j] = vb <= 0 ? 0u : low_mask(min(32, vb)); }
    e.m0 = m[0]; e.m1 = m[1]; e.m2 = m[2]; e.m3 = m[3];
    const int np = need - (T - T01);
    if (np <= 0) e.base = 0x80808080u;
    else if (np > 128) e.base = 0u;
    else e.base = ((u32)T01 << 24) + (u32)(128 - np) * 0x01010101u;
    return e;
}

template <int S>
__device__ __forceinline__ bool fast_span_long(const u32 (&ph)[8], const u32 (&pl)[8], int wl, int ka, int kb,
                                               const FastEntryLong* __restrict__ tab) {
    const FastEntryLong* tp = tab + (wl - ka + 1);
    for (int k = ka; k <= kb; k++, tp--) {
        const uint4 e0 = *reinterpret_cast<const uint4*>(tp);
        const u32 m3 = tp->m3;
        if (e0.x == 0u) continue;
        const u32 mk[4] = {e0.y, e0.z, e0.w, m3};
        int cH = 0, cL = 0, c11 = 0;
#pragma unroll
        for (int j = 0; j < 4; j++) {
            u32 a = (__funnelshift_r(ph[S + j], ph[S + j + 1], k) ^ ph[j]) & mk[j];
            u32 bb = (__funnelshift_r(pl[S + j], pl[S + j + 1], k) ^ pl[j]) & mk[j];
            cH += __popc(a); cL += __popc(bb); c11 += __popc(a & bb);
        }
        u32 x = e0.x + (u32)cH * kPackH + (u32)cL * kPackL + (u32)c11 * kPackC11;
        if (x & 0x80808080u) return true;
    }
    return false;
}

__device__ __forceinline__ bool probe_is_fast_long(const Probe& p) { return p.wl <= kFastMaxWlLong && p.k1 <= 64 && p.k1 <= p.wl; }

__device__ __noinline__ bool screen_probe_long(const DevBatch& b, const Probe& p, const FastEntryLong* __restrict__ tab) {
    u32 t[5], full[5] = {0xffffffffu, 0xffffffffu, 0xffffffffu, 0xffffffffu, 0xffffffffu};
    mask_bits<5>(full, p.wl);
    load_bits<5>(b.val, p.pos, t);
    u32 bad = 0;
#pragma unroll
    for (int j = 0; j < 5; j++) bad |= (t[j] & full[j]) ^ full[j];
    if (bad) return true;
    u32 ph[8], pl[8], q[5];
    load_bits<5>(b.hi, p.pos, t); mask_bits<5>(t, p.wl); prefix_xor_excl<5>(t, q);
#pragma unroll
    for (int j = 0; j < 8; j++) ph[j] = j < 5 ? q[j] : 0u;
    load_bits<5>(b.lo, p.pos, t); mask_bits<5>(t, p.wl); prefix_xor_excl<5>(t, q);
#pragma unroll
    for (int j = 0; j < 8; j++) pl[j] = j < 5 ? q[j] : 0u;
    int k0 = p.k0;
    if (k0 < 32) {
        if (fast_span_long<0>(ph, pl, p.wl, k0, min(p.k1, 31), tab)) return true;
        k0 = 32;
    }
    if (k0 < 64 && p.k1 >= 32) {
        if (fast_span_long<1>(ph, pl, p.wl, k0, min(p.k1, 63), tab)) return true;
        k0 = 64;
    }
    return p.k1 >= 64 && fast_span_long<2>(ph, pl, p.wl, k0, p.k1, tab);
}

__device__ __forceinline__ void list_append(bool flag, u32 value, u32* __restrict__ list, u32* __restrict__ count) {
    u32 m = __ballot_sync(0xffffffffu, flag);
    if (m) {
        u32 base = 0;
        if (lane_id() == 0) base = atomicAdd(count, (u32)__popc(m));
        base = __shfl_sync(0xffffffffu, base, 0);
        if (flag) list[base + __popc(m & ((1u << lane_id()) - 1u))] = value;
    }
}

__device__ __forceinline__ void list_append_rev(bool flag, u32 value, u32* __restrict__ top, u32* __restrict__ count) {
    u32 m = __ballot_sync(0xffffffffu, flag);
    if (m) {
        u32 base = 0;
        if (lane_id() == 0) base = atomicAdd(count, (u32)__popc(m));
        base = __shfl_sync(0xffffffffu, base, 0);
        if (flag) *(top - (base + __popc(m & ((1u << lane_id()) - 1u)))) = value;
    }
}

#ifndef TREW_SCREEN_BPS
#define TREW_SCREEN_BPS 8
#endif
template <bool LONG>
__global__ void __launch_bounds__(256, LONG ? 4 : TREW_SCREEN_BPS) trew_screen_kernel(DevCfg cfg, DevBatch b, u32 n_units,
                                                                                     u32* __restrict__ deferred, u32* __restrict__ n_deferred) {
    __shared__ uint4 tab[kFastTabSize];
    __shared__ FastEntryLong tab_long[LONG ? kFastTabSizeLong : 1];
    for (int T = threadIdx.x; T < kFastTabSize; T += blockDim.x) tab[T] = fast_entry(T, (int)cfg.thr_low[T]);
    if (LONG) for (int T = threadIdx.x; T < kFastTabSizeLong; T += blockDim.x) tab_long[T] = fast_entry_long(T, (int)cfg.thr_low[T]);
    __syncthreads();
    u32 stride = gridDim.x * blockDim.x;
    u32 n_round = (n_units + 31u) & ~31u;
    for (u32 u = blockIdx.x * blockDim.x + threadIdx.x; u < n_round; u += stride) {
        u32 pm = 0;
        if (u < n_units) {
            Probe p[4];
            int np = unit_probes(cfg, b, u, p);
            for (int i = 0; i < np; i++) {
                bool d;
                if (LONG && p[i].k1 >= p[i].k0 && !probe_is_fast(p[i]) && probe_is_fast_long(p[i])) d = screen_probe_long(b, p[i], tab_long);
                else d = screen_probe(b, p[i], tab);
                pm |= d ? 1u << i : 0u;
            }
        }
        list_append(pm != 0, u | (pm << kProbeShift), deferred, n_deferred);
    }
}

__device__ __forceinline__ int max4(int a, int b, int c, int d) { return max(max(a, b), max(c, d)); }

__device__ __forceinline__ u32 shr3(const u32 (&p)[3], int j, int k) {
    const int s = k >> 5;
    const u32 lo = j + s < 3 ? (s ? (j == 0 ? p[1] : p[2]) : p[j]) : 0u;
    const u32 hi = j + s + 1 < 3 ? (s ? p[2] : (j == 0 ? p[1] : p[2])) : 0u;
    return __funnelshift_r(lo, hi, k);
}
constexpr int kDecideThreads = 256;
__device__ __noinline__ bool mod4_level(const DevBatch& b, u32 pos, int wl, int k, int need, u32 pass8, u32 wv0, u32 wv1, u32 wv2, u32* cache,
                                        bool& cached) {
    const u32 wv[3] = {wv0, wv1, wv2};
    u32 p0[3][3], p1[3][3];
    if (!cached) {
        u32 x[3][3];
        load_bits<3>(b.hi, pos, x[0]); mask_bits<3>(x[0], wl);
        load_bits<3>(b.lo, pos, x[1]); mask_bits<3>(x[1], wl);
#pragma unroll
        for (int j = 0; j < 3; j++) x[2][j] = x[0][j] & x[1][j];
#pragma unroll
        for (int p = 0; p < 3; p++) {
            prefix_xor_excl<3>(x[p], p0[p]);
            u32 c[3];
#pragma unroll
            for (int j = 0; j < 3; j++) c[j] = x[p][j] & p0[p][j];
            prefix_xor_excl<3>(c, p1[p]);
#pragma unroll
            for (int j = 0; j < 3; j++) { cache[(6 * p + j) * kDecideThreads] = p0[p][j]; cache[(6 * p + 3 + j) * kDecideThreads] = p1[p][j]; }
        }
        cached = true;
    } else {
#pragma unroll
        for (int p = 0; p < 3; p++)
#pragma unroll
            for (int j = 0; j < 3; j++) { p0[p][j] = cache[(6 * p + j) * kDecideThreads]; p1[p][j] = cache[(6 * p + 3 + j) * kDecideThreads]; }
    }
    u32 d0[3][3], d1[3][3];
#pragma unroll
    for (int p = 0; p < 3; p++) {
#pragma unroll
        for (int j = 0; j < 3; j++) {
            const u32 q0 = shr3(p0[p], j, k);
            d0[p][j] = q0 ^ p0[p][j];
            d1[p][j] = shr3(p1[p], j, k) ^ p1[p][j] ^ (~q0 & p0[p][j]);
        }
    }
#pragma unroll 1
    for (int c2 = 0; c2 < 8; c2++) {
        if (!((pass8 >> c2) & 1u)) continue;
        u32 mw[3];
        int cnt = 0;
#pragma unroll
        for (int j = 0; j < 3; j++) {
            mw[j] = wv[j] & (d0[0][j] ^ ((c2 & 1) ? 0u : ~0u)) & (d0[1][j] ^ ((c2 & 2) ? 0u : ~0u)) & (d0[2][j] ^ ((c2 & 4) ? 0u : ~0u));
            cnt += __popc(mw[j]);
        }
        if (cnt < need) continue;
        bool may = true;
#pragma unroll
        for (int p = 0; p < 3 && may; p++) {
            const int one = __popc(mw[0] & d1[p][0]) + __popc(mw[1] & d1[p][1]) + __popc(mw[2] & d1[p][2]);
            const int zero = cnt - one;
            if (min(one, zero) >= need) return true;
            const u32 flip = one >= zero ? 0u : ~0u;
#pragma unroll
            for (int j = 0; j < 3; j++) mw[j] &= d1[p][j] ^ flip;
            cnt = max(one, zero);
            may = cnt >= need;
        }
        if (may) return true;
    }
    return false;
}

template <int S>
__device__ __forceinline__ bool decide_span(const u32 (&ph)[5], const u32 (&pl)[5], const u32 (&pa)[5], u32 (&wv)[3], int ka, int kb,
                                            const unsigned short* __restrict__ thr, bool& done, int& t_hit, const DevBatch& bt, u32 pos, int wl,
                                            u32* cache, bool& cached, int m4_below) {
    for (int k = ka; k <= kb; k++) {
        const int T01 = __popc(wv[0]) + __popc(wv[1]), E = __popc(wv[2]), T = T01 + E;
        if (T == 0) { done = true; return false; }
        const int need = thr[T];
        u32 a0 = (__funnelshift_r(ph[S], ph[S + 1], k) ^ ph[0]) & wv[0], a1 = (__funnelshift_r(ph[S + 1], ph[S + 2], k) ^ ph[1]) & wv[1];
        u32 b0 = (__funnelshift_r(pl[S], pl[S + 1], k) ^ pl[0]) & wv[0], b1 = (__funnelshift_r(pl[S + 1], pl[S + 2], k) ^ pl[1]) & wv[1];
        int cH = __popc(a0) + __popc(a1), cL = __popc(b0) + __popc(b1), c11 = __popc(a0 & b0) + __popc(a1 & b1);
        if (max4(c11, cH - c11, cL - c11, T01 - cH - cL + c11) + E >= need) {
            u32 a2 = (__funnelshift_r(ph[S + 2], ph[S + 3], k) ^ ph[2]) & wv[2], b2 = (__funnelshift_r(pl[S + 2], pl[S + 3], k) ^ pl[2]) & wv[2];
            cH += __popc(a2); cL += __popc(b2); c11 += __popc(a2 & b2);
            const int c10 = cH - c11, c01 = cL - c11, c00 = T - cH - cL + c11;
            if (max4(c11, c10, c01, c00) >= need) {
                u32 x0 = __funnelshift_r(pa[S], pa[S + 1], k) ^ pa[0], x1 = __funnelshift_r(pa[S + 1], pa[S + 2], k) ^ pa[1];
                u32 x2 = __funnelshift_r(pa[S + 2], pa[S + 3], k) ^ pa[2];
                int n11 = __popc(a0 & b0 & x0) + __popc(a1 & b1 & x1) + __popc(a2 & b2 & x2);
                int n10 = __popc(a0 & ~b0 & x0) + __popc(a1 & ~b1 & x1) + __popc(a2 & ~b2 & x2);
                int n01 = __popc(b0 & ~a0 & x0) + __popc(b1 & ~a1 & x1) + __popc(b2 & ~a2 & x2);
                int n00 = __popc(wv[0] & ~a0 & ~b0 & x0) + __popc(wv[1] & ~a1 & ~b1 & x1) + __popc(wv[2] & ~a2 & ~b2 & x2);
                int U2 = max(max4(n11, c11 - n11, n10, c10 - n10), max4(n01, c01 - n01, n00, c00 - n00));
                if (U2 >= need) {
                    const u32 pass8 = (u32)(c00 - n00 >= need) | (u32)(c10 - n10 >= need) << 1 | (u32)(c01 - n01 >= need) << 2 |
                                      (u32)(c11 - n11 >= need) << 3 | (u32)(n00 >= need) << 4 | (u32)(n10 >= need) << 5 |
                                      (u32)(n01 >= need) << 6 | (u32)(n11 >= need) << 7;
                    if (T >= m4_below || mod4_level(bt, pos, wl, k, need, pass8, wv[0], wv[1], wv[2], cache, cached)) { t_hit = T; return true; }
                }
            }
        }
        u32 t0 = __funnelshift_r(wv[0], wv[1], 1), t1 = __funnelshift_r(wv[1], wv[2], 1), t2 = wv[2] >> 1;
        wv[0] &= t0; wv[1] &= t1; wv[2] &= t2;
    }
    return false;
}

__device__ __noinline__ bool decide_short(const DevBatch& b, u32 pos, int wl, int k0, int k1, const unsigned short* __restrict__ thr, int& t_hit,
                                          u32* cache, int m4_below) {
    bool cached = false;
    u32 wv[3], ph[5], pl[5], pa[5];
    load_bits<3>(b.val, pos, wv); mask_bits<3>(wv, wl);
    {
        u32 h[3], l[3], q[3];
        load_bits<3>(b.hi, pos, h); mask_bits<3>(h, wl); prefix_xor_excl<3>(h, q);
        ph[0] = q[0]; ph[1] = q[1]; ph[2] = q[2]; ph[3] = 0u; ph[4] = 0u;
        load_bits<3>(b.lo, pos, l); mask_bits<3>(l, wl); prefix_xor_excl<3>(l, q);
        pl[0] = q[0]; pl[1] = q[1]; pl[2] = q[2]; pl[3] = 0u; pl[4] = 0u;
#pragma unroll
        for (int j = 0; j < 3; j++) h[j] &= l[j];
        prefix_xor_excl<3>(h, q);
        pa[0] = q[0]; pa[1] = q[1]; pa[2] = q[2]; pa[3] = 0u; pa[4] = 0u;
    }
    sliding_and<3>(wv, k0);
    bool done = false;
    if (k0 < 32) {
        if (decide_span<0>(ph, pl, pa, wv, k0, min(k1, 31), thr, done, t_hit, b, pos, wl, cache, cached, m4_below)) return true;
        if (done) return false;
        k0 = 32;
    }
    return k1 >= 32 && decide_span<1>(ph, pl, pa, wv, k0, k1, thr, done, t_hit, b, pos, wl, cache, cached, m4_below);
}

template <int MAXNW>
__global__ void __launch_bounds__(kDecideThreads, (MAXNW <= 5 ? 4 : 2)) trew_filter_kernel(DevCfg cfg, DevBatch b, const u32* __restrict__ units,
                                                          const u32* __restrict__ n_units_ptr, u32 n_units_all,
                                                          u32* __restrict__ survivors, u32* __restrict__ n_survivors,
                                                          u32* __restrict__ surv_b_top, u32* __restrict__ n_surv_b, int thread_min_windows, int third_level,
                                                          u32* __restrict__ work_counter) {
    __shared__ unsigned short thr[kThrTableSize];
    __shared__ u32 s_m4[18 * kDecideThreads];
    for (int i = threadIdx.x; i < kThrTableSize; i += blockDim.x) thr[i] = cfg.thr_low[i];
    __syncthreads();
    const u32 n_units = units ? *n_units_ptr : n_units_all;
    const bool pack_probes = n_units_all < (1u << kProbeShift);
    const u32 lane = lane_id();
    bool have = false, maybe = false, exhausted = false;
    u32 u = 0, live = 0, todo = 0;
    int t_hit = 1 << 20;
    Probe p[4];
    for (;;) {
        const u32 idle = __ballot_sync(0xffffffffu, !have);
        if (idle != 0u && !exhausted) {
            u32 base = 0;
            if (lane == 0) base = atomicAdd(work_counter, (u32)__popc(idle));
            base = __shfl_sync(0xffffffffu, base, 0);
            exhausted = base + (u32)__popc(idle) >= n_units;
            const u32 i = base + (u32)__popc(idle & ((1u << lane) - 1u));
            if (!have && i < n_units) {
                u32 pm = 0xfu;
                u = i;
                if (units) { const u32 e = units[i]; u = e & ((1u << kProbeShift) - 1u); pm = e >> kProbeShift; }
                const int np = unit_probes(cfg, b, u, p);
                live = todo = pm & ((1u << np) - 1u);
                maybe = false; t_hit = 1 << 20; have = true;
            }
        }
        if (__ballot_sync(0xffffffffu, have) == 0u) break;
        if (have && todo != 0u) {
            const int j = __ffs(todo) - 1;
            todo &= todo - 1u;
            if (p[j].k1 >= p[j].k0)
                maybe = probe_is_fast(p[j]) ? decide_short(b, p[j].pos, p[j].wl, p[j].k0, p[j].k1, thr, t_hit, s_m4 + threadIdx.x, third_level)
                                            : probe_dispatch<MAXNW>(b, p[j], thr);
            if (!maybe) live &= ~(1u << j);
        }
        const bool fin = have && (todo == 0u || maybe);
        const bool keep = fin && maybe;
        const u32 entry = pack_probes ? u | (live << kProbeShift) : u;
        if (surv_b_top == nullptr) {
            list_append(keep, entry, survivors, n_survivors);
        } else {
            bool to_b = false;
            if (keep) {
                int len;
                if (cfg.mode == 1) {
                    const u32 a0 = __ldg(b.bit_off + 2 * u), a1 = __ldg(b.bit_off + 2 * u + 1), a2 = __ldg(b.bit_off + 2 * u + 2);
                    len = (int)max(a1 - a0, a2 - a1);
                } else {
                    len = (int)(__ldg(b.bit_off + u + 1) - __ldg(b.bit_off + u));
                }
                to_b = len > et::kMaxRead || t_hit < thread_min_windows;
            }
            list_append(keep && !to_b, entry, survivors, n_survivors);
            list_append_rev(keep && to_b, entry, surv_b_top, n_surv_b);
        }
        if (fin) have = false;
    }
}

void launch_filter(const DevCfg& cfg, const DevBatch& b, unsigned int n_units, unsigned int max_read_len,
                   unsigned int* deferred, unsigned int* n_deferred, unsigned int* survivors, unsigned int* n_survivors,
                   const LaunchPlan& plan, cudaStream_t stream, cudaEvent_t after_screen, unsigned int* surv_b_top,
                   unsigned int* n_surv_b, unsigned int* work_counter) {
    if (n_units == 0) return;
    unsigned int longest;
    if (cfg.mode == 2) longest = 2u * (unsigned)cfg.slice_len;
    else longest = (max_read_len < 4u * (unsigned)cfg.max_mer) ? max_read_len : (max_read_len + 1) / 2;
    unsigned int need = (n_units + 255) / 256;
    const bool screen = deferred != nullptr && !(cfg.mode == 2 && cfg.slice_len > kFastMaxWlLong) && n_units < (1u << kProbeShift);
    if (screen) {
        int blocks = plan.screen_blocks;
        if ((unsigned)blocks > need) blocks = (int)need;
        if (longest <= (unsigned)kFastMaxWl) trew_screen_kernel<false><<<blocks, 256, 0, stream>>>(cfg, b, n_units, deferred, n_deferred);
        else trew_screen_kernel<true><<<blocks, 256, 0, stream>>>(cfg, b, n_units, deferred, n_deferred);
    }
    if (after_screen) cudaEventRecord(after_screen, stream);
    static const int tmw = [] { const char* e = getenv("TREW_THREAD_MIN_WINDOWS"); return e && *e ? atoi(e) : kThreadMinWindows; }();
    static const int m4_on = [] { const char* e = getenv("TREW_MOD4_BELOW"); return e && *e ? atoi(e) : kMod4BelowWindows; }();
    const unsigned int* list = screen ? deferred : nullptr;
    int blocks = plan.decide_blocks;
    if ((unsigned)blocks > need) blocks = (int)need;
    if (longest + 1 <= 96) trew_filter_kernel<3><<<blocks, 256, 0, stream>>>(cfg, b, list, n_deferred, n_units, survivors, n_survivors, surv_b_top, n_surv_b, tmw, m4_on, work_counter);
    else if (longest + 1 <= 160) trew_filter_kernel<5><<<blocks, 256, 0, stream>>>(cfg, b, list, n_deferred, n_units, survivors, n_survivors, surv_b_top, n_surv_b, tmw, m4_on, work_counter);
    else trew_filter_kernel<8><<<blocks, 256, 0, stream>>>(cfg, b, list, n_deferred, n_units, survivors, n_survivors, surv_b_top, n_surv_b, tmw, m4_on, work_counter);
}


extern __shared__ __align__(16) unsigned char g_smem[];

constexpr int kPlaneWords = 36;
#ifndef TREW_EXACT_BPS
#define TREW_EXACT_BPS 8
#endif
#ifndef TREW_EXACT_WARPS
#define TREW_EXACT_WARPS 4
#endif
constexpr int kExactWarps = TREW_EXACT_WARPS;
constexpr u32 kEmptySlot = 0xffffffffu;
constexpr int kSerialMaxRuns = 12;

enum { HD_CUR_POS = 0, HD_CUR_LEN, HD_ALLVALID, HD_EV_POS, HD_EV_LEN, HD_EV_K, HD_EV_PACK, HD_S = 8 ,
       HD_BLK_L = 12 , HD_BLK_H = 14 , HD_NEED_L = 16, HD_NEED_H = 17, HD_BLK64 = 18, HD_RES = 19,
       HD_SH = 20 , HD_SL = 24  };
constexpr int kHeaderBytes = 128;

__host__ __device__ inline int exact_hash_slots(int cap) {
    int hs = 64;
    while (hs < cap + cap / 4) hs <<= 1;
    return hs;
}

__host__ __device__ inline size_t exact_warp_bytes(int cap) {
    size_t b = kHeaderBytes + 5 * kPlaneWords * sizeof(u32) + kPlaneWords * sizeof(u64);
    b += (size_t)2 * cap * sizeof(u64) + (size_t)exact_hash_slots(cap) * sizeof(u32) + (size_t)2 * cap * sizeof(u32);
    b += (size_t)(3 * cap + 4) * sizeof(unsigned short);
    return (b + 15) & ~(size_t)15;
}

size_t exact_smem_bytes(int run_cap, bool) { return exact_warp_bytes(run_cap) * kExactWarps; }

struct WS {
    u32 off; int cap; int hs; u32 lane; u32 flags;
    __device__ __forceinline__ u32* hdr() const { return (u32*)(g_smem + off); }
    __device__ __forceinline__ u32* H() const { return (u32*)(g_smem + off + kHeaderBytes); }
    __device__ __forceinline__ u32* L() const { return H() + kPlaneWords; }
    __device__ __forceinline__ u32* V() const { return H() + 2 * kPlaneWords; }
    __device__ __forceinline__ u32* PH() const { return H() + 3 * kPlaneWords; }
    __device__ __forceinline__ u32* PL() const { return H() + 4 * kPlaneWords; }
    __device__ __forceinline__ u64* rev2() const { return (u64*)(H() + 5 * kPlaneWords); }
    __device__ __forceinline__ u64* run_lo() const { return rev2() + kPlaneWords; }
    __device__ __forceinline__ u64* run_hi() const { return run_lo() + cap; }
    __device__ __forceinline__ u32* htab() const { return (u32*)(run_hi() + cap); }
    __device__ __forceinline__ u32* grp_tot() const { return htab() + hs; }
    __device__ __forceinline__ u32* grp_last() const { return grp_tot() + cap; }
    __device__ __forceinline__ unsigned short* run_start() const { return (unsigned short*)(grp_last() + cap); }
    __device__ __forceinline__ unsigned short* run_cw() const { return run_start() + cap; }
    __device__ __forceinline__ unsigned short* run_total() const { return run_cw() + cap + 4; }
};

struct TableRef { Slot* slots; u32 mask; u32* err; };

struct ScanRes { int th, tl; u64 sh_lo, sh_hi, sl_lo, sl_hi; };

__device__ __forceinline__ int pk_T(u32 p) { return (int)(p & 1023u); }
__device__ __forceinline__ int pk_M(u32 p) { return (int)((p >> 10) & 1023u); }
__device__ __forceinline__ int pk_runs(u32 p) { return (int)((p >> 20) & 1023u); }
__device__ __forceinline__ bool pk_homo(u32 p) { return ((p >> 30) & 1u) != 0; }


__device__ __noinline__ u64 canon64(u64 w, int k) {
    int sh = 2 * (k - 1);
    if (k <= 16) {
        u32 b32 = (u32)w, c32 = (u32)w;
        for (int r = 1; r < k; r++) {
            c32 = ((c32 & 3u) << sh) | (c32 >> 2);
            b32 = min(b32, c32);
        }
        return b32;
    }
    u64 best = w, cur = w;
    for (int r = 1; r < k; r++) {
        cur = ((cur & 3ULL) << sh) | (cur >> 2);
        best = cur < best ? cur : best;
    }
    return best;
}

__device__ __noinline__ u128 canon128(u128 w, int k) {
    u128 best = w, cur = w;
    int sh = 2 * (k - 1);
    for (int r = 1; r < k; r++) {
        cur = ((cur & 3) << sh) | (cur >> 2);
        best = cur < best ? cur : best;
    }
    return best;
}

__device__ __forceinline__ u64 rev_pairs64(u64 x) {
    x = __brevll(x);
    return ((x >> 1) & 0x5555555555555555ULL) | ((x & 0x5555555555555555ULL) << 1);
}

__device__ __forceinline__ void canon_pair(u64& lo, u64& hi, int k) {
    if (k <= 32) { lo = canon64(lo, k); hi = 0; }
    else { u128 c = canon128(((u128)hi << 64) | lo, k); lo = (u64)c; hi = (u64)(c >> 64); }
}

__device__ __forceinline__ void crc_pair(u64& lo, u64& hi, int k) {
    if (k <= 32) {
        u64 r = ~rev_pairs64(lo) >> (64 - 2 * k);
        lo = canon64(r, k); hi = 0;
    } else {
        u128 r = ((u128)(~rev_pairs64(lo)) << 64) | (u128)(~rev_pairs64(hi));
        r >>= (128 - 2 * k);
        u128 c = canon128(r, k); lo = (u64)c; hi = (u64)(c >> 64);
    }
}

__device__ __forceinline__ bool homo_pair(u64 lo, u64 hi, int k) {
    if (k <= 1) return true;
    if (k <= 32) return ((lo ^ (lo >> 2)) & ((1ULL << (2 * (k - 1))) - 1ULL)) == 0;
    u128 w = ((u128)hi << 64) | lo;
    u128 m = (((u128)1 << (2 * (k - 1))) - 1);
    return ((w ^ (w >> 2)) & m) == 0;
}

__device__ __forceinline__ bool less_pair(u64 alo, u64 ahi, u64 blo, u64 bhi) {
    return ahi < bhi || (ahi == bhi && alo < blo);
}

__device__ __forceinline__ u32 shfl_next_bit0(u32 x, u32 lane) {
    u32 nx = __shfl_down_sync(0xffffffffu, x, 1);
    return lane == 31 ? 0u : (nx & 1u);
}


__device__ __noinline__ void load_window(WS ws, const u32* __restrict__ bhi, const u32* __restrict__ blo,
                                         const u32* __restrict__ bval, u32 pos, int len) {
    u32* hd = ws.hdr();
    if ((int)hd[HD_CUR_LEN] == len && hd[HD_CUR_POS] == pos) return;
    __syncwarp();
    const u32 lane = ws.lane;
    int vbits = len - 32 * (int)lane;
    u32 msk = vbits <= 0 ? 0u : low_mask(vbits);
    u32 h = 0, l = 0, v = 0;
    if (vbits > 0) {
        u32 wi = (pos >> 5) + lane, sh = pos & 31;
        h = __funnelshift_r(__ldg(bhi + wi), __ldg(bhi + wi + 1), sh) & msk;
        l = __funnelshift_r(__ldg(blo + wi), __ldg(blo + wi + 1), sh) & msk;
        v = __funnelshift_r(__ldg(bval + wi), __ldg(bval + wi + 1), sh) & msk;
    }
    const bool all_valid = __all_sync(0xffffffffu, v == msk);
    u32 ih = prefix_xor32(h), il = prefix_xor32(l);
    u32 bh = __ballot_sync(0xffffffffu, ih >> 31), bl = __ballot_sync(0xffffffffu, il >> 31);
    u32 lt = (1u << lane) - 1u;
    if (__popc(bh & lt) & 1) ih = ~ih;
    if (__popc(bl & lt) & 1) il = ~il;
    u32 ph_prev = __shfl_up_sync(0xffffffffu, ih, 1), pl_prev = __shfl_up_sync(0xffffffffu, il, 1);
    u32 ph = (ih << 1) | (lane ? ph_prev >> 31 : 0u);
    u32 pl = (il << 1) | (lane ? pl_prev >> 31 : 0u);
    u32 *H = ws.H(), *L = ws.L(), *V = ws.V(), *PH = ws.PH(), *PL = ws.PL();
    u64* rev2 = ws.rev2();
    H[lane] = h; L[lane] = l; V[lane] = v; PH[lane] = ph; PL[lane] = pl;
    if (lane < kPlaneWords - 32) {
        H[32 + lane] = 0; L[32 + lane] = 0; V[32 + lane] = 0; PH[32 + lane] = 0; PL[32 + lane] = 0;
        rev2[32 + lane] = 0;
    }
    __syncwarp();
    {
        int cs = len - 32 * (int)lane - 32;
        u32 hb = 0, lb = 0;
        if (cs > -32) {
            if (cs >= 0) {
                int wi = cs >> 5, sh = cs & 31;
                hb = __funnelshift_r(H[wi], H[wi + 1], sh);
                lb = __funnelshift_r(L[wi], L[wi + 1], sh);
            } else {
                hb = H[0] << (-cs);
                lb = L[0] << (-cs);
            }
        }
        hb = __brev(hb); lb = __brev(lb);
        u64 x = hb, y = lb;
        x = (x | (x << 16)) & 0x0000FFFF0000FFFFULL; y = (y | (y << 16)) & 0x0000FFFF0000FFFFULL;
        x = (x | (x << 8)) & 0x00FF00FF00FF00FFULL;  y = (y | (y << 8)) & 0x00FF00FF00FF00FFULL;
        x = (x | (x << 4)) & 0x0F0F0F0F0F0F0F0FULL;  y = (y | (y << 4)) & 0x0F0F0F0F0F0F0F0FULL;
        x = (x | (x << 2)) & 0x3333333333333333ULL;  y = (y | (y << 2)) & 0x3333333333333333ULL;
        x = (x | (x << 1)) & 0x5555555555555555ULL;  y = (y | (y << 1)) & 0x5555555555555555ULL;
        rev2[lane] = (x << 1) | y;
    }
    if (lane == 0) { hd[HD_CUR_POS] = pos; hd[HD_CUR_LEN] = (u32)len; hd[HD_ALLVALID] = all_valid ? 1u : 0u; }
    __syncwarp();
}

__device__ __forceinline__ void kmer_at(const u64* __restrict__ rev2, int len, int i, int k, u64& lo, u64& hi) {
    int o = 2 * (len - i - k);
    int wi = o >> 6, sh = o & 63;
    u64 a = rev2[wi], b = rev2[wi + 1];
    lo = sh ? (a >> sh) | (b << (64 - sh)) : a;
    if (k <= 32) {
        if (k < 32) lo &= (1ULL << (2 * k)) - 1ULL;
        hi = 0;
    } else {
        u64 c = rev2[wi + 2];
        hi = sh ? (b >> sh) | (c << (64 - sh)) : b;
        if (k < 64) hi &= (1ULL << (2 * k - 64)) - 1ULL;
    }
}

__device__ __forceinline__ u32 wv_for_k(WS ws, int len, int k) {
    const u32 lane = ws.lane;
    if (ws.hdr()[HD_ALLVALID]) {
        int vb = len - k + 1 - 32 * (int)lane;
        return vb <= 0 ? 0u : low_mask(min(32, vb));
    }
    u32 wv = ws.V()[lane];
    for (int t = 1; t < k; t++) {
        u32 nb = shfl_next_bit0(wv, lane);
        wv &= (wv >> 1) | (nb << 31);
    }
    return wv;
}

__device__ __forceinline__ u32 wv_step(u32 wv, u32 lane) {
    u32 nb = shfl_next_bit0(wv, lane);
    return wv & ((wv >> 1) | (nb << 31));
}

__device__ __forceinline__ int bound_k(WS ws, int k, u32 wv, int T) {
    const u32 lane = ws.lane;
    const u32 *PH = ws.PH(), *PL = ws.PL();
    int s = k >> 5, r = k & 31;
    u32 qh = __funnelshift_r(PH[lane + s], PH[lane + s + 1], r);
    u32 ql = __funnelshift_r(PL[lane + s], PL[lane + s + 1], r);
    u32 dh = (qh ^ PH[lane]) & wv, dl = (ql ^ PL[lane]) & wv;
    u32 packed = (u32)__popc(dh) | ((u32)__popc(dl) << 10) | ((u32)__popc(dh & dl) << 20);
    packed = __reduce_add_sync(0xffffffffu, packed);
    int cH = packed & 1023, cL = (packed >> 10) & 1023, c11 = packed >> 20;
    int c10 = cH - c11, c01 = cL - c11, c00 = T - cH - cL + c11;
    return max(max(c00, c01), max(c10, c11));
}

__device__ __noinline__ int comp_bound(WS ws, int k, u32 wv, int T) {
    const u32 lane = ws.lane;
    const u32 cnt = (u32)__popc(wv);
    u32 inc = cnt;
#pragma unroll
    for (int d = 1; d < 32; d <<= 1) {
        u32 t = __shfl_up_sync(0xffffffffu, inc, d);
        if ((int)lane >= d) inc += t;
    }
    unsigned short* pos = ws.run_start();
    {
        u32 rb = inc - cnt, x = wv;
        while (x) {
            int bit = __ffs(x) - 1;
            x &= x - 1;
            pos[rb++] = (unsigned short)(32 * lane + bit);
        }
    }
    __syncwarp();
    const bool act = (int)lane < T;
    u32 key = 0;
    if (act) {
        const u32 *H = ws.H(), *L = ws.L();
        const int p = pos[lane], w0 = p >> 5, o = p & 31;
        const u32 m0 = low_mask(min(k, 32)), m1 = k <= 32 ? 0u : low_mask(k - 32);
        const u32 h0 = __funnelshift_r(H[w0], H[w0 + 1], o) & m0, h1 = __funnelshift_r(H[w0 + 1], H[w0 + 2], o) & m1;
        const u32 l0 = __funnelshift_r(L[w0], L[w0 + 1], o) & m0, l1 = __funnelshift_r(L[w0 + 1], L[w0 + 2], o) & m1;
        key = (u32)(__popc(h0) + __popc(h1)) | ((u32)(__popc(l0) + __popc(l1)) << 8) | ((u32)(__popc(h0 & l0) + __popc(h1 & l1)) << 16);
    }
    const u32 actm = __ballot_sync(0xffffffffu, act);
    const u32 same = __match_any_sync(0xffffffffu, key) & actm;
    const u32 best = __reduce_max_sync(0xffffffffu, act ? (u32)__popc(same) : 0u);
    __syncwarp();
    return (int)best;
}

__device__ __noinline__ u32 eval_k(WS ws, int len, int k, u32 wv) {
    const u32 lane = ws.lane;
    u32* hd = ws.hdr();
    const u32 *H = ws.H(), *L = ws.L();
    int s = k >> 5, r = k & 31;
    u32 hs = __funnelshift_r(H[lane + s], H[lane + s + 1], r);
    u32 ls = __funnelshift_r(L[lane + s], L[lane + s + 1], r);
    u32 eq = ~((hs ^ H[lane]) | (ls ^ L[lane]));
    u32 nb = shfl_next_bit0(wv, lane);
    u32 link = eq & wv & ((wv >> 1) | (nb << 31));
    u32 link_prev = __shfl_up_sync(0xffffffffu, link, 1);
    u32 rs = wv & ~((link << 1) | (lane ? link_prev >> 31 : 0u));
    u32 pk = (u32)__popc(wv) | ((u32)__popc(rs) << 16);
    const u32 tot_pk = __reduce_add_sync(0xffffffffu, pk);
    const int T = (int)(tot_pk & 0xffffu), R = (int)(tot_pk >> 16);
    if (T == 0) return 0u;
    unsigned short *run_start = ws.run_start(), *run_cw = ws.run_cw(), *run_total = ws.run_total();
    u64 *run_lo = ws.run_lo(), *run_hi = ws.run_hi();
    u32 *htab = ws.htab(), *grp_tot = ws.grp_tot(), *grp_last = ws.grp_last();
    const u64* rev2 = ws.rev2();
    const bool wide = k > 32;
    if (!wide && R <= kSerialMaxRuns && (ws.flags & 1u)) {
        u32* scr = htab;
        scr[lane] = wv; scr[32 + lane] = link; scr[64 + lane] = rs;
        __syncwarp();
        unsigned short* cls_last = run_cw;
        int ncls = 0, ord = 0;
        const int nw = (len + 31) >> 5;
        for (int j = 0; j < nw; j++) {
            const u32 wvj = scr[j];
            u32 rr = scr[64 + j];
            while (rr) {
                const int b = __ffs(rr) - 1;
                rr &= rr - 1;
                const int c0 = ord + __popc(wvj & ((1u << b) - 1u));
                int jj = j;
                u32 x = ~scr[32 + j] & (0xffffffffu << b);
                while (!x) { jj++; x = ~scr[32 + jj]; }
                const int cnt = 32 * (jj - j) + (__ffs(x) - 1) - b + 1;
                u64 lo, hi;
                kmer_at(rev2, len, 32 * j + b, k, lo, hi);
                lo = canon64(lo, k);
                int q = 0;
                while (q < ncls && run_lo[q] != lo) q++;
                u32 tot = (u32)cnt;
                if (q == ncls) { ncls++; run_lo[q] = lo; }
                else tot += run_total[q];
                run_total[q] = (unsigned short)tot;
                cls_last[q] = (unsigned short)(c0 + cnt - 1);
            }
            ord += __popc(wvj);
        }
        u32 best = 0; int bq = 0;
        for (int q = 0; q < ncls; q++) {
            const u32 score = ((u32)run_total[q] << 10) | (1023u - cls_last[q]);
            if (score > best) { best = score; bq = q; }
        }
        const u64 s_lo = run_lo[bq];
        const bool homo = homo_pair(s_lo, 0ULL, k);
        __syncwarp();
        if (lane == 0) { hd[HD_S] = (u32)s_lo; hd[HD_S + 1] = (u32)(s_lo >> 32); hd[HD_S + 2] = 0u; hd[HD_S + 3] = 0u; }
        __syncwarp();
        return (u32)T | ((best >> 10) << 10) | ((u32)ncls << 20) | (homo ? 1u << 30 : 0u);
    }
    u32 inc = pk;
#pragma unroll
    for (int d = 1; d < 32; d <<= 1) {
        u32 t = __shfl_up_sync(0xffffffffu, inc, d);
        if ((int)lane >= d) inc += t;
    }
    u32 exc = inc - pk;
    {
        u32 cwb = exc & 0xffffu, rb = exc >> 16;
        u32 x = rs;
        while (x) {
            int bit = __ffs(x) - 1;
            x &= x - 1;
            run_start[rb] = (unsigned short)(32 * lane + bit);
            run_cw[rb] = (unsigned short)(cwb + __popc(wv & ((1u << bit) - 1u)));
            rb++;
        }
        if (lane == 0) run_cw[R] = (unsigned short)T;
    }
    int hsz = 32;
    while (hsz < R + (R >> 1) && hsz < ws.hs) hsz <<= 1;
    const u32 hmask = (u32)hsz - 1u;
    for (int i = lane; i < hsz; i += 32) {
        htab[i] = kEmptySlot;
        if (i < R) { grp_tot[i] = 0u; grp_last[i] = 0u; }
    }
    __syncwarp();
    for (int q = lane; q < R; q += 32) {
        u64 lo, hi;
        kmer_at(rev2, len, run_start[q], k, lo, hi);
        canon_pair(lo, hi, k);
        run_lo[q] = lo; if (wide) run_hi[q] = hi;
    }
    __syncwarp();
    for (int q = lane; q < R; q += 32) {
        u64 lo = run_lo[q], hi = wide ? run_hi[q] : 0ULL;
        u32 hsh = (u32)lo ^ (u32)(lo >> 32) ^ (u32)hi ^ (u32)(hi >> 32);
        u32 slot = (hsh * 0x9e3779b1u) >> 7 & hmask;
        int leader;
        for (;;) {
            u32 old = atomicCAS(&htab[slot], kEmptySlot, (u32)q);
            if (old == kEmptySlot) { leader = q; break; }
            if (run_lo[old] == lo && (!wide || run_hi[old] == hi)) { leader = (int)old; break; }
            slot = (slot + 1) & hmask;
        }
        u32 c0 = run_cw[q], c1 = run_cw[q + 1];
        atomicAdd(&grp_tot[leader], c1 - c0);
        atomicMax(&grp_last[leader], c1 - 1u);
    }
    __syncwarp();
    u32 best = 0; int best_q = -1;
    for (int q = lane; q < R; q += 32) {
        u32 total = grp_tot[q];
        run_total[q] = (unsigned short)total;
        if (total) {
            u32 score = (total << 10) | (1023u - grp_last[q]);
            if (score > best) { best = score; best_q = q; }
        }
    }
    u32 wbest = __reduce_max_sync(0xffffffffu, best);
    u32 who = __ballot_sync(0xffffffffu, best == wbest && best_q >= 0);
    int bq = __shfl_sync(0xffffffffu, best_q, __ffs(who) - 1);
    u64 s_lo = run_lo[bq], s_hi = wide ? run_hi[bq] : 0ULL;
    bool homo = homo_pair(s_lo, s_hi, k);
    u32 packed = (u32)T | ((wbest >> 10) << 10) | ((u32)R << 20) | (homo ? 1u << 30 : 0u);
    if (lane == 0) {
        hd[HD_S] = (u32)s_lo; hd[HD_S + 1] = (u32)(s_lo >> 32); hd[HD_S + 2] = (u32)s_hi; hd[HD_S + 3] = (u32)(s_hi >> 32);
    }
    __syncwarp();
    return packed;
}

__device__ __forceinline__ void eval_S(WS ws, u64& lo, u64& hi) {
    const u32* hd = ws.hdr();
    lo = (u64)hd[HD_S] | ((u64)hd[HD_S + 1] << 32);
    hi = (u64)hd[HD_S + 2] | ((u64)hd[HD_S + 3] << 32);
}

__device__ __noinline__ void emit_classes(TableRef tr, WS ws, int k, int nruns, int table, bool folded) {
    u32 meta = ((u32)table << 8) | (u32)k;
    const unsigned short* run_total = ws.run_total();
    const u64 *run_lo = ws.run_lo(), *run_hi = ws.run_hi();
    for (int q = ws.lane; q < nruns; q += 32) {
        u32 total = run_total[q];
        if (total == 0) continue;
        u64 lo = run_lo[q], hi = k > 32 ? run_hi[q] : 0ULL;
        if (folded) {
            u64 rlo = lo, rhi = hi;
            crc_pair(rlo, rhi, k);
            if (less_pair(rlo, rhi, lo, hi)) { lo = rlo; hi = rhi; }
        }
        table_add_impl(tr.slots, tr.mask, tr.err, meta, lo, hi, (u64)total);
    }
    __syncwarp();
}

struct MultTab { u64 m[65]; };
constexpr MultTab make_mult_tab() {
    MultTab t{};
    for (int k = 1; k <= 64; k++) {
        u64 m = 0;
        for (int j = k; j < 64; j += k) m |= 1ULL << j;
        t.m[k] = m;
    }
    return t;
}
__constant__ MultTab c_mult = make_mult_tab();

__device__ __forceinline__ int thr_at(const WS& ws, const unsigned short* thr_low, bool high, int T) {
    return (int)__ldg(thr_low + (high ? kThrTableSize : 0) + T);
}
__device__ __forceinline__ bool need_pass(const WS& ws, const unsigned short* thr_low, bool high, u32 need, int M, int T) {
    const u32 m = need & 0xffffu, t = need >> 16;
    return M >= thr_at(ws, thr_low, high, T) && (t == 0u || (u32)M * t >= m * (u32)T);
}
__device__ __forceinline__ bool need_pre(double B, u32 need, int U, int T) {
    const u32 m = need & 0xffffu, t = need >> 16;
    return (double)U >= B * (double)T * (1.0 - 1e-12) && (t == 0u || (u32)U * t >= m * (u32)T);
}

__device__ __forceinline__ bool blocked_k(const u32* hd, int which , int k) {
    if (k >= 64) return (hd[HD_BLK64] >> (which == HD_BLK_H ? 1 : 0)) & 1u;
    return (hd[which + (k >> 5)] >> (k & 31)) & 1u;
}

__device__ __forceinline__ bool try_k(WS ws, const unsigned short* thr_low, double low, double high, u32 pos, int len, int kk, int Uk, int Tk, u32 wv) {
    u32* hd = ws.hdr();
    const bool blkL = blocked_k(hd, HD_BLK_L, kk), blkH = blocked_k(hd, HD_BLK_H, kk);
    if (blkL && blkH) return false;
    const u32 needL = hd[HD_NEED_L], needH = hd[HD_NEED_H];
    bool candL = !blkL && need_pre(low, needL, Uk, Tk), candH = !blkH && need_pre(high, needH, Uk, Tk);
    if (!candL && !candH) return false;
#ifndef TREW_NO_COMP_BOUND
    if (Tk <= 32 && !(ws.flags & 2u)) {
        const int Mc = comp_bound(ws, kk, wv, Tk);
        if (Mc < Uk) {
            candL = !blkL && need_pre(low, needL, Mc, Tk); candH = !blkH && need_pre(high, needH, Mc, Tk);
            if (!candL && !candH) return false;
        }
    }
#endif
    const u32 ev = eval_k(ws, len, kk, wv);
    if (ws.lane == 0) { hd[HD_EV_POS] = pos; hd[HD_EV_LEN] = (u32)len; hd[HD_EV_K] = (u32)kk; hd[HD_EV_PACK] = ev; }
    __syncwarp();
    if (pk_homo(ev) || pk_T(ev) == 0) return false;
    const int M = pk_M(ev), T = pk_T(ev);
    const bool accL = !blkL && need_pass(ws, thr_low, false, needL, M, T), accH = !blkH && need_pass(ws, thr_low, true, needH, M, T);
    if (!(accL || accH)) return false;
    if (ws.lane == 0) {
        const u64 mm = c_mult.m[kk];
        const u32 m64 = (64 % kk) == 0 ? 1u : 0u;
        const u32 need = (u32)M | ((u32)T << 16);
        u32 res = hd[HD_RES];
        if (accL) {
            hd[HD_NEED_L] = need; hd[HD_BLK_L] |= (u32)mm; hd[HD_BLK_L + 1] |= (u32)(mm >> 32); hd[HD_BLK64] |= m64;
            res = (res & 0xffu) | ((u32)kk << 8);
            hd[HD_SL] = hd[HD_S]; hd[HD_SL + 1] = hd[HD_S + 1]; hd[HD_SL + 2] = hd[HD_S + 2]; hd[HD_SL + 3] = hd[HD_S + 3];
        }
        if (accH) {
            hd[HD_NEED_H] = need; hd[HD_BLK_H] |= (u32)mm; hd[HD_BLK_H + 1] |= (u32)(mm >> 32); hd[HD_BLK64] |= m64 << 1;
            res = (res & 0xff00u) | (u32)kk;
            hd[HD_SH] = hd[HD_S]; hd[HD_SH + 1] = hd[HD_S + 1]; hd[HD_SH + 2] = hd[HD_S + 2]; hd[HD_SH + 3] = hd[HD_S + 3];
        }
        hd[HD_RES] = res;
    }
    __syncwarp();
    return true;
}

__device__ __noinline__ u32 scan_core(WS ws, DevBatch b, u32 pos, int len, int kmin, int kmax, const unsigned short* thr_low, double low,
                                      double high) {
    if (kmax < kmin) return 0u;
    load_window(ws, b.hi, b.lo, b.val, pos, len);
    const u32 lane = ws.lane;
    u32* hd = ws.hdr();
    if (lane >= HD_BLK_L && lane <= HD_SL + 3) hd[lane] = 0u;
    __syncwarp();
    const bool all_valid = hd[HD_ALLVALID] != 0;

    if (len <= 127 || all_valid) {
        const u32 *PH = ws.PH(), *PL = ws.PL(), *V = ws.V();
        const int nw = (len + 31) >> 5;
        for (int kb = kmin; kb <= kmax; kb += 32) {
            const int k = kb + (int)lane;
            int U = 0, T = 0;
            u32 wvv[4] = {0u, 0u, 0u, 0u};
            if (k <= kmax && k <= len) {
                const int s = k >> 5, r = k & 31;
                int cH = 0, cL = 0, c11 = 0;
                if (all_valid) {
                    T = len - k + 1;
                    for (int j = 0; j * 32 < T; j++) {
                        u32 wvj = low_mask(min(32, T - 32 * j));
                        u32 dh = (__funnelshift_r(PH[j + s], PH[j + s + 1], r) ^ PH[j]) & wvj;
                        u32 dl = (__funnelshift_r(PL[j + s], PL[j + s + 1], r) ^ PL[j]) & wvj;
                        cH += __popc(dh); cL += __popc(dl); c11 += __popc(dh & dl);
                    }
                } else {
#pragma unroll
                    for (int j = 0; j < 4; j++) wvv[j] = V[j];
                    sliding_and<4>(wvv, k);
#pragma unroll
                    for (int j = 0; j < 4; j++) {
                        if (j < nw) {
                            u32 dh = (__funnelshift_r(PH[j + s], PH[j + s + 1], r) ^ PH[j]) & wvv[j];
                            u32 dl = (__funnelshift_r(PL[j + s], PL[j + s + 1], r) ^ PL[j]) & wvv[j];
                            T += __popc(wvv[j]); cH += __popc(dh); cL += __popc(dl); c11 += __popc(dh & dl);
                        }
                    }
                }
                int c10 = cH - c11, c01 = cL - c11, c00 = T - cH - cL + c11;
                U = max(max(c00, c01), max(c10, c11));
            }
            bool cand = T > 0 && need_pre(low, 0u, U, T);
            u32 cm = __ballot_sync(0xffffffffu, cand);
            while (cm) {
                int bit = __ffs(cm) - 1;
                cm &= cm - 1;
                int Uk = __shfl_sync(0xffffffffu, U, bit), Tk = __shfl_sync(0xffffffffu, T, bit);
                u32 wv;
                if (all_valid) {
                    int vb = Tk - 32 * (int)lane;
                    wv = vb <= 0 ? 0u : low_mask(min(32, vb));
                } else {
                    u32 a0 = __shfl_sync(0xffffffffu, wvv[0], bit), a1 = __shfl_sync(0xffffffffu, wvv[1], bit);
                    u32 a2 = __shfl_sync(0xffffffffu, wvv[2], bit), a3 = __shfl_sync(0xffffffffu, wvv[3], bit);
                    wv = lane == 0 ? a0 : lane == 1 ? a1 : lane == 2 ? a2 : lane == 3 ? a3 : 0u;
                }
                if (try_k(ws, thr_low, low, high, pos, len, kb + bit, Uk, Tk, wv) && cm) {
                    bool still = false;
                    if (T > 0 && k <= 64)
                        still = (!blocked_k(hd, HD_BLK_L, k) && need_pre(low, hd[HD_NEED_L], U, T)) ||
                                (!blocked_k(hd, HD_BLK_H, k) && need_pre(high, hd[HD_NEED_H], U, T));
                    cm &= __ballot_sync(0xffffffffu, still);
                }
            }
        }
        return hd[HD_RES];
    }

    u32 wv = wv_for_k(ws, len, kmin);
    for (int k = kmin; k <= kmax; k++, wv = wv_step(wv, lane)) {
        int T = (int)__reduce_add_sync(0xffffffffu, (u32)__popc(wv));
        if (T == 0) break;
        int U = bound_k(ws, k, wv, T);
        try_k(ws, thr_low, low, high, pos, len, k, U, T, wv);
    }
    return hd[HD_RES];
}

__device__ __forceinline__ ScanRes scan_stats(WS ws, const DevBatch& b, u32 pos, int len, int kmin, int kmax, const DevCfg& cfg) {
    const u32 r = scan_core(ws, b, pos, len, kmin, kmax, cfg.thr_low, cfg.low, cfg.high);
    const u32* hd = ws.hdr();
    ScanRes res;
    res.th = (int)(r & 0xffu); res.tl = (int)(r >> 8);
    res.sh_lo = (u64)hd[HD_SH] | ((u64)hd[HD_SH + 1] << 32); res.sh_hi = (u64)hd[HD_SH + 2] | ((u64)hd[HD_SH + 3] << 32);
    res.sl_lo = (u64)hd[HD_SL] | ((u64)hd[HD_SL + 1] << 32); res.sl_hi = (u64)hd[HD_SL + 2] | ((u64)hd[HD_SL + 3] << 32);
    return res;
}

__device__ __noinline__ u32 eval_cached(WS ws, DevBatch b, u32 pos, int len, int k) {
    u32* hd = ws.hdr();
    if ((int)hd[HD_EV_K] == k && hd[HD_EV_POS] == pos && (int)hd[HD_EV_LEN] == len) return hd[HD_EV_PACK];
    load_window(ws, b.hi, b.lo, b.val, pos, len);
    u32 wv = wv_for_k(ws, len, k);
    u32 ev = eval_k(ws, len, k, wv);
    if (ws.lane == 0) { hd[HD_EV_POS] = pos; hd[HD_EV_LEN] = (u32)len; hd[HD_EV_K] = (u32)k; hd[HD_EV_PACK] = ev; }
    __syncwarp();
    return ev;
}

__device__ void emit_window(TableRef tr, WS ws, const DevBatch& b, u32 pos, int len, int k, int table, bool folded) {
    u32 ev = eval_cached(ws, b, pos, len, k);
    emit_classes(tr, ws, k, pk_runs(ev), table, folded);
}

__device__ void target_window(TableRef tr, WS ws, const DevBatch& b, u32 pos, int len, int k, const unsigned short* thr_low, bool high, int table) {
    u32 ev = eval_cached(ws, b, pos, len, k);
    if (pk_T(ev) > 0 && !pk_homo(ev) && pk_M(ev) >= thr_at(ws, thr_low, high, pk_T(ev))) emit_classes(tr, ws, k, pk_runs(ev), table, true);
}


enum { T_F = 0, T_B = 2, T_O = 4 };

__device__ void route_short(const DevCfg& cfg, TableRef tr, WS ws, const DevBatch& b, u32 u, u32 pm) {
    const int MINM = cfg.min_mer, MAXM = cfg.max_mer;
    u32 b0 = __ldg(b.bit_off + u);
    int n = (int)(__ldg(b.bit_off + u + 1) - b0);
    if (n < 2 * MINM || n > kMaxWindow) return;
    int L[2] = {0, 0}, R[2] = {0, 0};
    if (n >= 4 * MINM) {
        int kmax = min(n / 4, MAXM);
        u32 lpos = b0, rpos = b0 + (u32)(n - (n + 1) / 2);
        int llen = n / 2, rlen = (n + 1) / 2;
        if (pm & 1u) { ScanRes l = scan_stats(ws, b, lpos, llen, MINM, kmax, cfg); L[0] = l.th; L[1] = l.tl; }
        if (pm & 2u) { ScanRes r = scan_stats(ws, b, rpos, rlen, MINM, kmax, cfg); R[0] = r.th; R[1] = r.tl; }
        pm >>= 2;
#pragma unroll
        for (int c = 0; c < 2; c++) {
            if (L[c] > 0 && L[c] == R[c]) target_window(tr, ws, b, b0, n, L[c], cfg.thr_low, c == 0, T_O + c);
            else if (L[c] > 0) emit_window(tr, ws, b, lpos, llen, L[c], T_F + c, false);
            else if (R[c] > 0) emit_window(tr, ws, b, rpos, rlen, R[c], T_B + c, false);
        }
    }
    bool hc[2] = {L[0] == 0 && R[0] == 0, L[1] == 0 && R[1] == 0};
    if (4 * MAXM > n && (hc[0] || hc[1]) && (pm & 1u)) {
        ScanRes s = scan_stats(ws, b, b0, n, max(n / 4 + 1, MINM), min(n / 2, MAXM), cfg);
        if (hc[0] && s.th) emit_window(tr, ws, b, b0, n, s.th, T_O + 0, false);
        if (hc[1] && s.tl) emit_window(tr, ws, b, b0, n, s.tl, T_O + 1, false);
    }
}

__device__ void route_pair(const DevCfg& cfg, TableRef tr, WS ws, const DevBatch& b, u32 u) {
    const int MINM = cfg.min_mer, MAXM = cfg.max_mer;
    u32 a0 = __ldg(b.bit_off + 2 * u), a1 = __ldg(b.bit_off + 2 * u + 1), a2 = __ldg(b.bit_off + 2 * u + 2);
    int n1 = (int)(a1 - a0), n2 = (int)(a2 - a1);
    int n = min(n1, n2);
    if (n < 2 * MINM || n1 > kMaxWindow || n2 > kMaxWindow) return;
    int lef[2] = {0, 0}, km[2] = {0, 0};
    if (n >= 4 * MINM) {
        u32 spos[5] = {0, a0, a0 + (u32)(n1 - (n1 + 1) / 2), a1 + (u32)(n2 - (n2 + 1) / 2), a1};
        int slen[5] = {0, n1 / 2, (n1 + 1) / 2, (n2 + 1) / 2, n2 / 2};
        int kmax = min(n / 4, MAXM);
        ScanRes sr[5]; bool have[5] = {false, false, false, false, false};
        int pseg[2][8], ptmp[2][8], np[2] = {0, 0};
        int si[2] = {1, 1}; bool ended[2] = {false, false};
        u64 ks_lo[2] = {0, 0}, ks_hi[2] = {0, 0};
        for (int ti = 1; ti <= 4 && !(ended[0] && ended[1]); ti++) {
            if (!have[ti]) { sr[ti] = scan_stats(ws, b, spos[ti], slen[ti], MINM, kmax, cfg); have[ti] = true; }
            int k[2] = {sr[ti].th, sr[ti].tl};
            u64 slo[2] = {sr[ti].sh_lo, sr[ti].sl_lo}, shi[2] = {sr[ti].sh_hi, sr[ti].sl_hi};
#pragma unroll
            for (int c = 0; c < 2; c++) {
                if (!ended[c] && k[c]) { pseg[c][np[c]] = ti; ptmp[c][np[c]] = ti <= 2 ? 0 : 1; np[c]++; }
                bool ok = !ended[c] && k[c] > 0;
                if (ok && ti != 1) {
                    u64 dlo = slo[c], dhi = shi[c];
                    if (ti > 2) crc_pair(dlo, dhi, k[c]);
                    ok = km[c] == k[c] && ks_lo[c] == dlo && ks_hi[c] == dhi;
                }
                if (ok) { si[c]++; km[c] = k[c]; if (ti == 1) { ks_lo[c] = slo[c]; ks_hi[c] = shi[c]; } }
                else ended[c] = true;
            }
        }
        lef[0] = km[0]; lef[1] = km[1];
#pragma unroll
        for (int c = 0; c < 2; c++) {
            if (si[c] == 5) {
                for (int e = 0; e < np[c]; e++) {
                    int sg = pseg[c][e];
                    emit_window(tr, ws, b, spos[sg], slen[sg], c == 0 ? sr[sg].th : sr[sg].tl, T_O + c, true);
                }
            }
        }
        if (si[0] <= 4 || si[1] <= 4) {
            int sj[2] = {4, 4}; km[0] = km[1] = 0; ended[0] = ended[1] = false;
            for (int tj = 4; tj >= 1 && !(ended[0] && ended[1]); tj--) {
                if (!have[tj]) { sr[tj] = scan_stats(ws, b, spos[tj], slen[tj], MINM, kmax, cfg); have[tj] = true; }
                int k[2] = {sr[tj].th, sr[tj].tl};
                u64 slo[2] = {sr[tj].sh_lo, sr[tj].sl_lo}, shi[2] = {sr[tj].sh_hi, sr[tj].sl_hi};
#pragma unroll
                for (int c = 0; c < 2; c++) {
                    if (!ended[c] && k[c]) { pseg[c][np[c]] = tj; ptmp[c][np[c]] = tj <= 2 ? 1 : 0; np[c]++; }
                    bool ok = sj[c] >= si[c] && !ended[c] && k[c] > 0;
                    if (ok && tj != 4) {
                        u64 dlo = slo[c], dhi = shi[c];
                        if (tj <= 2) crc_pair(dlo, dhi, k[c]);
                        ok = km[c] == k[c] && ks_lo[c] == dlo && ks_hi[c] == dhi;
                    }
                    if (ok) { sj[c]--; km[c] = k[c]; if (tj == 4) { ks_lo[c] = slo[c]; ks_hi[c] = shi[c]; } }
                    else ended[c] = true;
                }
            }
        }
#pragma unroll
        for (int c = 0; c < 2; c++) {
            if (si[c] <= 4) {
                for (int e = 0; e < np[c]; e++) {
                    int sg = pseg[c][e];
                    emit_window(tr, ws, b, spos[sg], slen[sg], c == 0 ? sr[sg].th : sr[sg].tl,
                                (ptmp[c][e] == 0 ? T_F : T_B) + c, false);
                }
            }
        }
    }
    if (4 * MAXM > n && (lef[0] == 0 || lef[1] == 0 || km[0] == 0 || km[1] == 0)) {
        int lo = max(n / 4 + 1, MINM), hi = min(n / 2, MAXM);
        ScanRes l, r; l.th = l.tl = r.th = r.tl = 0; l.sh_lo = l.sh_hi = l.sl_lo = l.sl_hi = 0; r = l;
        if (lef[0] == 0 || lef[1] == 0) l = scan_stats(ws, b, a0, n1, lo, hi, cfg);
        if (km[0] == 0 || km[1] == 0) r = scan_stats(ws, b, a1, n2, lo, hi, cfg);
        int ltk[2] = {l.th, l.tl}, rtk[2] = {r.th, r.tl};
        u64 llo[2] = {l.sh_lo, l.sl_lo}, lhi[2] = {l.sh_hi, l.sl_hi}, rlo[2] = {r.sh_lo, r.sl_lo}, rhi[2] = {r.sh_hi, r.sl_hi};
#pragma unroll
        for (int c = 0; c < 2; c++) {
            bool el = lef[c] == 0 && ltk[c] > 0, er = km[c] == 0 && rtk[c] > 0;
            bool both = lef[c] == 0 && km[c] == 0 && ltk[c] == rtk[c] && ltk[c] > 0;
            if (both) {
                u64 dlo = rlo[c], dhi = rhi[c];
                crc_pair(dlo, dhi, rtk[c]);
                both = llo[c] == dlo && lhi[c] == dhi;
            }
            if (both) {
                if (el) emit_window(tr, ws, b, a0, n1, ltk[c], T_O + c, true);
                if (er) emit_window(tr, ws, b, a1, n2, rtk[c], T_O + c, true);
            }
            if (el) emit_window(tr, ws, b, a0, n1, ltk[c], T_F + c, false);
            if (er) emit_window(tr, ws, b, a1, n2, rtk[c], T_F + c, false);
        }
    }
}

__device__ void route_long(const DevCfg& cfg, TableRef tr, WS ws, const DevBatch& b, u32 u, unsigned char* scratch) {
    const int MINM = cfg.min_mer, MAXM = cfg.max_mer, SL = cfg.slice_len;
    u32 b0 = __ldg(b.bit_off + u);
    int n = (int)(__ldg(b.bit_off + u + 1) - b0);
    if (n < SL) return;
    int snum = n / SL, mid = (snum + 1) / 2, bonus = n % SL;
    auto s_start = [&](int t) { return (u32)((t - 1) * SL + (t > mid ? bonus : 0)); };
    auto s_len = [&](int t) { return SL + (t == mid ? bonus : 0); };
    int si[2] = {1, 1}, km[2] = {0, 0}; bool ended[2] = {false, false};
    int nf = 0;
    for (int ti = 1; ti <= snum && !(ended[0] && ended[1]); ti++) {
        ScanRes sr = scan_stats(ws, b, b0 + s_start(ti), s_len(ti), MINM, MAXM, cfg);
        if (ws.lane == 0) { scratch[2 * (ti - 1)] = (unsigned char)sr.th; scratch[2 * (ti - 1) + 1] = (unsigned char)sr.tl; }
        int k[2] = {sr.th, sr.tl};
#pragma unroll
        for (int c = 0; c < 2; c++) {
            if (!ended[c] && k[c] > 0 && (ti == 1 || km[c] == k[c])) { si[c]++; km[c] = k[c]; }
            else ended[c] = true;
        }
        nf = ti;
    }
    __syncwarp();
    {
        bool en[2] = {false, false}; int kk[2] = {0, 0};
        bool full[2] = {si[0] == snum + 1, si[1] == snum + 1};
        for (int ti = 1; ti <= nf; ti++) {
            int k[2] = {scratch[2 * (ti - 1)], scratch[2 * (ti - 1) + 1]};
#pragma unroll
            for (int c = 0; c < 2; c++) {
                if (!en[c] && k[c]) emit_window(tr, ws, b, b0 + s_start(ti), s_len(ti), k[c], (full[c] ? T_O : T_F) + c, full[c]);
                if (!en[c] && k[c] > 0 && (ti == 1 || kk[c] == k[c])) kk[c] = k[c];
                else en[c] = true;
            }
        }
    }
    if (si[0] <= snum || si[1] <= snum) {
        int sj[2] = {snum, snum}; km[0] = km[1] = 0; ended[0] = ended[1] = false;
        for (int tj = snum; tj >= 1 && !(ended[0] && ended[1]); tj--) {
            ScanRes sr = scan_stats(ws, b, b0 + s_start(tj), s_len(tj), MINM, MAXM, cfg);
            int k[2] = {sr.th, sr.tl};
#pragma unroll
            for (int c = 0; c < 2; c++) {
                if (!ended[c] && k[c]) emit_window(tr, ws, b, b0 + s_start(tj), s_len(tj), k[c], T_B + c, false);
                if (sj[c] >= si[c] && !ended[c] && k[c] > 0 && (tj == snum || km[c] == k[c])) { sj[c]--; km[c] = k[c]; }
                else ended[c] = true;
            }
        }
    }
}


constexpr int kStageSlots = 256;
constexpr int kStageProbes = 6;
constexpr u32 kStageLock = 0xffffffffu;

struct StageEmit {
    u32* s_meta; u32* s_cnt; u64* s_key;
    Slot* slots; u32 mask; u32* err;
    __device__ __forceinline__ void operator()(int table, int k, et::u128 key, u64 count) const {
        const u64 hi = (u64)(key >> 64);
        if (hi) table_add_impl(slots, mask, err, ((u32)table << 8) | (u32)k, (u64)key, hi, count);
        else (*this)(table, k, (et::u64)key, count);
    }
    __device__ __forceinline__ void operator()(int table, int k, et::u64 key_, u64 count) const {
        const u64 key = (u64)key_;
        const u32 meta = ((u32)table << 8) | (u32)k, tag = meta | 0x80000000u;
        u32 i = (u32)(mix64(key ^ ((u64)meta << 53)) >> 40) & (kStageSlots - 1);
        bool done = false;
        for (int p = 0; p < kStageProbes && !done; p++, i = (i + 1) & (kStageSlots - 1)) {
            int outcome = 0;
            do {
                const u32 st = atomicCAS(&s_meta[i], 0u, kStageLock);
                if (st == 0u) {
                    s_key[i] = key;
                    __threadfence_block();
                    atomicExch(&s_meta[i], tag);
                    atomicAdd(&s_cnt[i], (u32)count);
                    outcome = 1;
                } else if (st != kStageLock) {
                    __threadfence_block();
                    if (st == tag && *(volatile u64*)&s_key[i] == key) { atomicAdd(&s_cnt[i], (u32)count); outcome = 1; }
                    else outcome = 2;
                }
            } while (outcome == 0);
            done = outcome == 1;
        }
        if (!done) table_add_impl(slots, mask, err, meta, key, 0ULL, count);
    }
};

#ifndef TREW_THREAD_BLOCK
#define TREW_THREAD_BLOCK 128
#endif
template <class K>
constexpr size_t thread_kernel_smem() { return (size_t)et::Lay<K>::WORDS * TREW_THREAD_BLOCK * sizeof(u32) + (size_t)kStageSlots * 16; }
constexpr size_t kThreadKernelSmem = thread_kernel_smem<et::u64>();
template <int MODE, class K>
constexpr int thread_kernel_bps() { return (sizeof(K) == 8 ? 6 : 5) - (MODE == 1 ? 1 : 0); }

struct PlaneLoad {
    et::Mem m; const u32 *hi, *lo, *val; u32 b0[2];
    __device__ __forceinline__ void operator()(int mate, int off, int len) const {
        const u32 pos = b0[mate] + (u32)off, w0 = pos >> 5, sh = pos & 31u;
        for (int j = 0; j < et::kReadWords + 2; j++) {
            const u32 msk = low_mask(min(32, max(0, len - 32 * j)));
            u32 h = 0u, l = 0u;
            if (msk) {
                h = __funnelshift_r(__ldg(hi + w0 + j), __ldg(hi + w0 + j + 1), sh) & msk;
                l = __funnelshift_r(__ldg(lo + w0 + j), __ldg(lo + w0 + j + 1), sh) & msk;
            }
            m[et::W_H + j] = h; m[et::W_L + j] = l;
            if (j < et::kReadWords) m[et::W_V + j] = msk ? __funnelshift_r(__ldg(val + w0 + j), __ldg(val + w0 + j + 1), sh) & msk : 0u;
        }
    }
};

template <int MODE, class K>
__global__ void __launch_bounds__(TREW_THREAD_BLOCK, (thread_kernel_bps<MODE, K>())) trew_exact_thread_kernel(DevCfg cfg, DevBatch b, const u32* __restrict__ survivors,
                                                                              const u32* __restrict__ n_survivors, int packed_probes,
                                                                              u32* __restrict__ hard, u32* __restrict__ n_hard,
                                                                              unsigned long long* total_survivors, u32* work_counter) {
    u32* work = reinterpret_cast<u32*>(g_smem);
    u64* s_key = reinterpret_cast<u64*>(work + et::Lay<K>::WORDS * TREW_THREAD_BLOCK);
    u32* s_meta = reinterpret_cast<u32*>(s_key + kStageSlots);
    u32* s_cnt = s_meta + kStageSlots;
    for (int i = threadIdx.x; i < kStageSlots; i += blockDim.x) { s_meta[i] = 0u; s_cnt[i] = 0u; }
    __syncthreads();
    const et::Mem m{work + threadIdx.x, TREW_THREAD_BLOCK};
    const u32 n = *n_survivors;
    if (blockIdx.x == 0 && threadIdx.x == 0 && total_survivors) atomicAdd(total_survivors, (unsigned long long)n);
    StageEmit emit{s_meta, s_cnt, s_key, cfg.slots, cfg.slot_mask, cfg.error_flag};
    for (;;) {
        u32 base = 0;
        if (lane_id() == 0) base = atomicAdd(work_counter, 32u);
        base = __shfl_sync(0xffffffffu, base, 0);
        if (base >= n) break;
        const u32 i = base + lane_id();
        bool bail = false;
        u32 entry = 0;
        if (i < n) {
            entry = survivors[i];
            u32 u = entry, pm = 3u;
            if (packed_probes) { pm = entry >> kProbeShift; u &= (1u << kProbeShift) - 1u; }
            if (MODE == 0) {
                const u32 b0 = __ldg(b.bit_off + u);
                const int len = (int)(__ldg(b.bit_off + u + 1) - b0);
                if (len > et::kMaxRead) {
                    bail = true;
                } else {
                    PlaneLoad load{m, b.hi, b.lo, b.val, {b0, 0u}};
                    bail = !et::route_short_thread<K>(m, len, pm & 7u, cfg.min_mer, cfg.max_mer, cfg.thr_low, cfg.thr_high, load, emit);
                }
            } else {
                const u32 a0 = __ldg(b.bit_off + 2 * u), a1 = __ldg(b.bit_off + 2 * u + 1), a2 = __ldg(b.bit_off + 2 * u + 2);
                const int n1 = (int)(a1 - a0), n2 = (int)(a2 - a1);
                PlaneLoad load{m, b.hi, b.lo, b.val, {a0, a1}};
                bail = !et::route_pair_thread<K>(m, n1, n2, cfg.min_mer, cfg.max_mer, cfg.thr_low, cfg.thr_high, load, emit);
            }
        }
        list_append(bail, entry, hard, n_hard);
    }
    __syncthreads();
    for (int i = threadIdx.x; i < kStageSlots; i += blockDim.x) {
        const u32 st = s_meta[i], c = s_cnt[i];
        if (st != 0u && st != kStageLock && c != 0u) table_add_impl(cfg.slots, cfg.slot_mask, cfg.error_flag, st & 0x7fffffffu, s_key[i], 0ULL, (u64)c);
    }
}


struct LongArgs {
    const u32* survivors; const u32* n_survivors; int packed_probes;
    u32 s_cap, max_slices;
    unsigned short* stats; u32* emis;
    u32* hard; u32* n_hard;
    unsigned long long* total_survivors;
};

__global__ void __launch_bounds__(TREW_THREAD_BLOCK, 4) trew_long_stats_kernel(DevCfg cfg, DevBatch b, LongArgs a) {
    u32* work = reinterpret_cast<u32*>(g_smem);
    const et::Mem m{work + threadIdx.x, TREW_THREAD_BLOCK};
    const u32 n = min(*a.n_survivors, a.s_cap);
    const u32 warps = gridDim.x * (blockDim.x >> 5), lane = lane_id();
    et::ClsSpill<et::u64> x;
    for (u32 idx = blockIdx.x * (blockDim.x >> 5) + (threadIdx.x >> 5); idx < n; idx += warps) {
        u32 u = a.survivors[idx];
        if (a.packed_probes) u &= (1u << kProbeShift) - 1u;
        const u32 b0 = __ldg(b.bit_off + u);
        const int len = (int)(__ldg(b.bit_off + u + 1) - b0);
        if (len < cfg.slice_len) continue;
        const et::LongGeom g(len, cfg.slice_len);
        PlaneLoad load{m, b.hi, b.lo, b.val, {b0, 0u}};
        unsigned short* row = a.stats + (size_t)idx * (a.max_slices + 1);
        for (int t = 1 + (int)lane; t <= g.snum; t += 32) {
            u32 r = 0;
            if (g.len(t) <= et::kMaxRead) r = et::long_slice_stats(m, g, t, cfg.min_mer, cfg.max_mer, cfg.thr_low, cfg.thr_high, load, x);
            row[t] = (unsigned short)r;
        }
    }
}

__global__ void __launch_bounds__(256) trew_long_walk_kernel(DevCfg cfg, DevBatch b, LongArgs a) {
    const u32 n_all = *a.n_survivors;
    if (blockIdx.x == 0 && threadIdx.x == 0 && a.total_survivors) atomicAdd(a.total_survivors, (unsigned long long)n_all);
    const u32 stride = gridDim.x * blockDim.x, n_round = (n_all + 31u) & ~31u;
    for (u32 idx = blockIdx.x * blockDim.x + threadIdx.x; idx < n_round; idx += stride) {
        bool bail = false;
        u32 entry = 0;
        if (idx < n_all) {
            entry = a.survivors[idx];
            u32 u = entry;
            if (a.packed_probes) u &= (1u << kProbeShift) - 1u;
            const int len = (int)(__ldg(b.bit_off + u + 1) - __ldg(b.bit_off + u));
            if (idx >= a.s_cap) bail = len >= cfg.slice_len;
            else if (len >= cfg.slice_len) {
                const et::LongGeom g(len, cfg.slice_len);
                const unsigned short* row = a.stats + (size_t)idx * (a.max_slices + 1);
                u32* em = a.emis + (size_t)idx * (a.max_slices + 1);
                for (int t = 1; t <= g.snum; t++) em[t] = 0u;
                auto stat = [&](int t) { return (u32)row[t]; };
                auto task = [&](const et::LongTask& tk) {
                    const int tb = tk.table_folded & 7, c = tb & 1;
                    const bool backward = (tb & 6) == et::T_B;
                    const u32 byte = (u32)tk.k | ((tk.table_folded & 8) ? 0x80u : 0u);
                    em[tk.slice] |= byte << (8 * ((backward ? 2 : 0) + c));
                };
                bail = !et::long_walk(g, stat, task);
                if (bail) for (int t = 1; t <= g.snum; t++) em[t] = 0u;
            }
        }
        list_append(bail, entry, a.hard, a.n_hard);
    }
}

__global__ void __launch_bounds__(TREW_THREAD_BLOCK, 4) trew_long_emit_kernel(DevCfg cfg, DevBatch b, LongArgs a) {
    u32* work = reinterpret_cast<u32*>(g_smem);
    u64* s_key = reinterpret_cast<u64*>(work + et::Lay<et::u64>::WORDS * TREW_THREAD_BLOCK);
    u32* s_meta = reinterpret_cast<u32*>(s_key + kStageSlots);
    u32* s_cnt = s_meta + kStageSlots;
    for (int i = threadIdx.x; i < kStageSlots; i += blockDim.x) { s_meta[i] = 0u; s_cnt[i] = 0u; }
    __syncthreads();
    const et::Mem m{work + threadIdx.x, TREW_THREAD_BLOCK};
    StageEmit emit{s_meta, s_cnt, s_key, cfg.slots, cfg.slot_mask, cfg.error_flag};
    const u32 n = min(*a.n_survivors, a.s_cap);
    const u32 warps = gridDim.x * (blockDim.x >> 5), lane = lane_id();
    et::ClsSpill<et::u64> x;
    for (u32 idx = blockIdx.x * (blockDim.x >> 5) + (threadIdx.x >> 5); idx < n; idx += warps) {
        u32 u = a.survivors[idx];
        if (a.packed_probes) u &= (1u << kProbeShift) - 1u;
        const u32 b0 = __ldg(b.bit_off + u);
        const int len = (int)(__ldg(b.bit_off + u + 1) - b0);
        if (len < cfg.slice_len) continue;
        const et::LongGeom g(len, cfg.slice_len);
        PlaneLoad load{m, b.hi, b.lo, b.val, {b0, 0u}};
        const u32* em = a.emis + (size_t)idx * (a.max_slices + 1);
        for (int t = 1 + (int)lane; t <= g.snum; t += 32) {
            const u32 e = em[t];
            if (e == 0u) continue;
            for (int f = 0; f < 4; f++) {
                const u32 byte = (e >> (8 * f)) & 0xffu;
                if (byte == 0u) continue;
                const int c = f & 1;
                const bool folded = (byte & 0x80u) != 0u;
                const int table = (f >= 2 ? et::T_B : (folded ? et::T_O : et::T_F)) + c;
                et::LongTask tk{(unsigned short)t, (unsigned char)(byte & 0x7fu), (unsigned char)(table | (folded ? 8 : 0))};
                et::long_emit(m, g, tk, load, x, emit);
            }
        }
    }
    __syncthreads();
    for (int i = threadIdx.x; i < kStageSlots; i += blockDim.x) {
        const u32 st = s_meta[i], c = s_cnt[i];
        if (st != 0u && st != kStageLock && c != 0u) table_add_impl(cfg.slots, cfg.slot_mask, cfg.error_flag, st & 0x7fffffffu, s_key[i], 0ULL, (u64)c);
    }
}

bool long_thread_path_applies(const DevCfg& cfg) { return cfg.mode == 2 && cfg.max_mer <= 32 && cfg.slice_len <= et::kMaxRead; }

size_t long_thread_scratch_bytes(unsigned int s_cap, unsigned int max_slices) {
    return (size_t)s_cap * (max_slices + 1) * (sizeof(unsigned short) + sizeof(u32)) + 64;
}

void launch_long_thread(const DevCfg& cfg, const DevBatch& b, const unsigned int* survivors, const unsigned int* n_survivors,
                        int packed_probes, unsigned int s_cap, unsigned int max_slices, unsigned char* scratch, unsigned int* hard,
                        unsigned int* n_hard, unsigned long long* total_survivors, int sm_count, cudaStream_t stream) {
    LongArgs a{};
    a.survivors = survivors; a.n_survivors = n_survivors; a.packed_probes = packed_probes;
    a.s_cap = s_cap; a.max_slices = max_slices;
    a.emis = reinterpret_cast<u32*>(scratch);
    a.stats = reinterpret_cast<unsigned short*>(scratch + (size_t)s_cap * (max_slices + 1) * sizeof(u32));
    a.hard = hard; a.n_hard = n_hard; a.total_survivors = total_survivors;
    const size_t smem_stats = (size_t)et::Lay<et::u64>::WORDS * TREW_THREAD_BLOCK * sizeof(u32);
    trew_long_stats_kernel<<<sm_count * 4, TREW_THREAD_BLOCK, smem_stats, stream>>>(cfg, b, a);
    trew_long_walk_kernel<<<sm_count * 2, 256, 0, stream>>>(cfg, b, a);
    trew_long_emit_kernel<<<sm_count * 4, TREW_THREAD_BLOCK, kThreadKernelSmem, stream>>>(cfg, b, a);
}

bool thread_path_applies(const DevCfg& cfg, unsigned int max_read_len) {
    if (cfg.max_mer > 64) return false;
    if (cfg.mode == 0) return true;
    return cfg.mode == 1 && max_read_len >= 4u * (unsigned)cfg.max_mer;
}

void launch_exact_thread(const DevCfg& cfg, const DevBatch& b, const unsigned int* survivors, const unsigned int* n_survivors,
                         int packed_probes, unsigned int* hard, unsigned int* n_hard, unsigned long long* total_survivors, int sm_count,
                         int blocks_per_sm, unsigned int* work_counter, cudaStream_t stream) {
    const bool wide = cfg.max_mer > 32;
#define TREW_LAUNCH_THREAD(MODE, K)                                                                                               \
    trew_exact_thread_kernel<MODE, K><<<sm_count * (blocks_per_sm > 0 ? blocks_per_sm : thread_kernel_bps<MODE, K>()),            \
                                        TREW_THREAD_BLOCK, thread_kernel_smem<K>(), stream>>>(                                    \
        cfg, b, survivors, n_survivors, packed_probes, hard, n_hard, total_survivors, work_counter)
    if (cfg.mode == 0) { if (wide) TREW_LAUNCH_THREAD(0, et::u128); else TREW_LAUNCH_THREAD(0, et::u64); }
    else               { if (wide) TREW_LAUNCH_THREAD(1, et::u128); else TREW_LAUNCH_THREAD(1, et::u64); }
#undef TREW_LAUNCH_THREAD
}

template <int MODE>
__global__ void __launch_bounds__(kExactWarps * 32, TREW_EXACT_BPS) trew_exact_kernel(DevCfg cfg, DevBatch b, ExactArgs a) {
    const int wid = threadIdx.x >> 5;
    const u32 lane = lane_id();
    WS ws;
    ws.cap = a.run_cap; ws.hs = exact_hash_slots(a.run_cap);
    ws.off = (u32)((size_t)wid * exact_warp_bytes(a.run_cap)); ws.lane = lane; ws.flags = a.exp_flags;
    TableRef tr{cfg.slots, cfg.slot_mask, cfg.error_flag};
    ws.hdr()[lane] = lane == HD_CUR_LEN || lane == HD_EV_LEN || lane == HD_EV_K ? 0xffffffffu : 0u;
    __syncwarp();
    const u32 n = *a.n_survivors;
    if (blockIdx.x == 0 && threadIdx.x == 0 && a.total_survivors) atomicAdd(a.total_survivors, (u64)n);
    unsigned char* scratch = a.slice_scratch + (size_t)(blockIdx.x * kExactWarps + wid) * a.slice_scratch_stride;
    for (;;) {
        u32 idx = 0;
        if (lane == 0) idx = atomicAdd(a.work_counter, 1u);
        idx = __shfl_sync(0xffffffffu, idx, 0);
        if (idx >= n) break;
        u32 u = a.reverse ? *(a.survivors - idx) : a.survivors[idx], pm = 0xfu;
        if (a.packed_probes) { pm = u >> kProbeShift; u &= (1u << kProbeShift) - 1u; }
        if constexpr (MODE == 0) route_short(cfg, tr, ws, b, u, pm);
        else if constexpr (MODE == 1) route_pair(cfg, tr, ws, b, u);
        else route_long(cfg, tr, ws, b, u, scratch);
    }
}

constexpr int kExactBlocksPerSM = TREW_EXACT_BPS;
int exact_warps_total(int sm_count) { return sm_count * kExactBlocksPerSM * kExactWarps; }

cudaError_t prepare_exact(int run_cap_max) {
    int bytes = (int)exact_smem_bytes(run_cap_max, true);
    cudaError_t e = cudaFuncSetAttribute(trew_exact_kernel<0>, cudaFuncAttributeMaxDynamicSharedMemorySize, bytes);
    if (e == cudaSuccess) e = cudaFuncSetAttribute(trew_exact_kernel<1>, cudaFuncAttributeMaxDynamicSharedMemorySize, bytes);
    if (e == cudaSuccess) e = cudaFuncSetAttribute(trew_exact_kernel<2>, cudaFuncAttributeMaxDynamicSharedMemorySize, bytes);
    if (e == cudaSuccess) e = cudaFuncSetAttribute(trew_exact_thread_kernel<0, et::u64>, cudaFuncAttributeMaxDynamicSharedMemorySize, (int)thread_kernel_smem<et::u64>());
    if (e == cudaSuccess) e = cudaFuncSetAttribute(trew_exact_thread_kernel<1, et::u64>, cudaFuncAttributeMaxDynamicSharedMemorySize, (int)thread_kernel_smem<et::u64>());
    if (e == cudaSuccess) e = cudaFuncSetAttribute(trew_exact_thread_kernel<0, et::u128>, cudaFuncAttributeMaxDynamicSharedMemorySize, (int)thread_kernel_smem<et::u128>());
    if (e == cudaSuccess) e = cudaFuncSetAttribute(trew_exact_thread_kernel<1, et::u128>, cudaFuncAttributeMaxDynamicSharedMemorySize, (int)thread_kernel_smem<et::u128>());
    if (e == cudaSuccess) e = cudaFuncSetAttribute(trew_long_stats_kernel, cudaFuncAttributeMaxDynamicSharedMemorySize, (int)kThreadKernelSmem);
    if (e == cudaSuccess) e = cudaFuncSetAttribute(trew_long_emit_kernel, cudaFuncAttributeMaxDynamicSharedMemorySize, (int)kThreadKernelSmem);
    return e;
}

LaunchPlan default_launch_plan(int sm_count) { return LaunchPlan{sm_count * 128, sm_count * 4, sm_count * kExactBlocksPerSM}; }

void launch_exact(const DevCfg& cfg, const DevBatch& b, const ExactArgs& a, const LaunchPlan& plan, cudaStream_t stream) {
    size_t smem = exact_smem_bytes(a.run_cap, true);
    dim3 grid(plan.exact_blocks), block(kExactWarps * 32);
    if (cfg.mode == 0) trew_exact_kernel<0><<<grid, block, smem, stream>>>(cfg, b, a);
    else if (cfg.mode == 1) trew_exact_kernel<1><<<grid, block, smem, stream>>>(cfg, b, a);
    else trew_exact_kernel<2><<<grid, block, smem, stream>>>(cfg, b, a);
}

}
```

### trew_b200/csrc/scan_kernels.cuh

```cuda
#pragma once
#include <cstdint>
#include <cuda_runtime.h>

#include "../../include/trew_b200.h"

namespace trew {

constexpr int kThrTableSize = 1025;
constexpr int kMaxWindow = 1023;

struct __align__(32) Slot {
    unsigned long long seq_lo;
    unsigned long long seq_hi;
    unsigned long long count;
    unsigned int meta;
    unsigned int state;
};

struct DevCfg {
    int mode, min_mer, max_mer, slice_len;
    double low, high;
    Slot* slots;
    unsigned int slot_mask;
    unsigned int* error_flag;
    const unsigned short* thr_low;
    const unsigned short* thr_high;
};

struct DevBatch {
    unsigned int n_reads;
    const unsigned int* bit_off;
    const unsigned int* hi;
    const unsigned int* lo;
    const unsigned int* val;
};

struct ExactArgs {
    const unsigned int* survivors;
    const unsigned int* n_survivors;
    unsigned int* work_counter;
    unsigned char* slice_scratch;
    unsigned int slice_scratch_stride;
    int run_cap;
    unsigned long long* total_survivors;
    int packed_probes;
    int reverse;
    unsigned int exp_flags;
};

struct LaunchPlan { int screen_blocks, decide_blocks, exact_blocks; };
LaunchPlan default_launch_plan(int sm_count);

void launch_filter(const DevCfg& cfg, const DevBatch& b, unsigned int n_units, unsigned int max_read_len,
                   unsigned int* deferred, unsigned int* n_deferred, unsigned int* survivors, unsigned int* n_survivors,
                   const LaunchPlan& plan, cudaStream_t stream, cudaEvent_t after_screen,
                   unsigned int* surv_b_top, unsigned int* n_surv_b, unsigned int* work_counter);
size_t exact_smem_bytes(int run_cap, bool wide);
cudaError_t prepare_exact(int run_cap_max);
void launch_exact(const DevCfg& cfg, const DevBatch& b, const ExactArgs& a, const LaunchPlan& plan, cudaStream_t stream);
int exact_warps_total(int sm_count);
bool long_thread_path_applies(const DevCfg& cfg);
size_t long_thread_scratch_bytes(unsigned int s_cap, unsigned int max_slices);
void launch_long_thread(const DevCfg& cfg, const DevBatch& b, const unsigned int* survivors, const unsigned int* n_survivors,
                        int packed_probes, unsigned int s_cap, unsigned int max_slices, unsigned char* scratch, unsigned int* hard,
                        unsigned int* n_hard, unsigned long long* total_survivors, int sm_count, cudaStream_t stream);
bool thread_path_applies(const DevCfg& cfg, unsigned int max_read_len);
void launch_exact_thread(const DevCfg& cfg, const DevBatch& b, const unsigned int* survivors, const unsigned int* n_survivors,
                         int packed_probes, unsigned int* hard, unsigned int* n_hard, unsigned long long* total_survivors, int sm_count,
                         int blocks_per_sm, unsigned int* work_counter, cudaStream_t stream);
void launch_compact(const Slot* slots, unsigned int n_slots, trew_entry* out, unsigned int* d_n, cudaStream_t stream, unsigned int cap);
cudaError_t sort_entries_radix(const trew_entry* d_entries, trew_entry* d_out, unsigned int n, bool wide, void* d_temp,
                               size_t* temp_bytes, cudaStream_t stream);
cudaError_t combine_sorted_rows(const trew_entry* d_sorted, unsigned int n, trew_entry* d_out, unsigned int* d_n_out, void* d_temp,
                                size_t* temp_bytes, cudaStream_t stream);
cudaError_t filter_report_rows(const trew_entry* d_rows, unsigned int n, unsigned int min_total, trew_entry* d_out, unsigned int* d_n_out,
                               void* d_temp, size_t* temp_bytes, cudaStream_t stream);
void launch_clear_invalid(unsigned int* val, const unsigned int* rec, unsigned int n, cudaStream_t stream);
void launch_merge_entries(const DevCfg& cfg, const trew_entry* entries, unsigned int n, cudaStream_t stream);

void launch_synth(unsigned long long seed, unsigned int n_reads, unsigned int read_len, unsigned int tel_thr,
                  unsigned int half_thr, unsigned int n_thr, unsigned int sub_thr, unsigned int flavor, unsigned int* bit_off,
                  unsigned int* hi, unsigned int* lo, unsigned int* val, size_t plane_words, cudaStream_t stream);

}
```

Measured before the change: 1036.

## Pool exact-stage work across up to sixteen resident batches into single launches

```diff
diff --git a/trew_b200/csrc/device_ctx.cu b/trew_b200/csrc/device_ctx.cu
--- a/trew_b200/csrc/device_ctx.cu
+++ b/trew_b200/csrc/device_ctx.cu
@@ -36,6 +36,15 @@
 
 struct RangeInfo { uint32_t r0, r1; uint64_t bases; uint32_t max_len; };
 
+struct ScanOut {
+    DevBatch b;
+    uint32_t n_units, max_read_len;
+    unsigned int* d_survivors;
+    unsigned int* d_counters;
+    bool thread_path;
+    const trew_resident* r;
+};
+
 }
 
 struct trew_resident {
@@ -45,9 +54,7 @@
     uint64_t bases = 0;
     unsigned int* d_survivors = nullptr;
     unsigned int* d_counters = nullptr;
-    unsigned char* d_scratch = nullptr;
-    size_t scratch_bytes = 0;
-    cudaEvent_t ev[4] = {nullptr, nullptr, nullptr, nullptr};
+    cudaEvent_t ev[3] = {nullptr, nullptr, nullptr};
     bool ev_pending = false;
 };
 
@@ -90,6 +97,10 @@
     cudaEvent_t ev_t0 = nullptr, ev_t1 = nullptr;
     double screen_ms = 0, decide_ms = 0, exact_ms = 0; uint64_t n_prof_scans = 0;
     std::vector<trew_resident*> pending_prof;
+    std::vector<ScanOut> pool_pending;
+    unsigned char* d_pool_scratch = nullptr; size_t pool_scratch_bytes = 0;
+    std::vector<cudaEvent_t> flush_ev;
+    size_t n_flush_ev = 0;
     void* h_export = nullptr; size_t h_export_bytes = 0;
     unsigned int report_min = 0;
     trew_entry* d_filtered = nullptr; size_t d_filtered_cap = 0;
@@ -156,16 +167,7 @@
 }
 
 int launch_scan(trew_ctx* ctx, const DevBatch& b, uint32_t n_units, uint32_t max_read_len, unsigned int* d_survivors,
-                unsigned int* d_counters, unsigned char** d_scratch, size_t* scratch_bytes, cudaStream_t st,
-                cudaEvent_t* ev = nullptr) {
-    unsigned int stride, s_cap, max_slices;
-    size_t long_off;
-    size_t need = scratch_need(ctx, max_read_len, n_units, &stride, &long_off, &s_cap, &max_slices);
-    if (need > *scratch_bytes) {
-        if (*d_scratch) { CK(cudaStreamSynchronize(st)); CK(cudaFree(*d_scratch)); *d_scratch = nullptr; }
-        CK(cudaMalloc((void**)d_scratch, need));
-        *scratch_bytes = need;
-    }
+                unsigned int* d_counters, cudaStream_t st, cudaEvent_t* ev, ScanOut* out) {
     ctx->export_valid = false;
     CK(cudaMemsetAsync(d_counters, 0, kScanCounters * sizeof(unsigned int), st));
     if (ev) CK(cudaEventRecord(ev[0], st));
@@ -174,32 +176,64 @@
                   ev ? ev[1] : nullptr, thread_path ? d_survivors + n_units - 1 : nullptr, thread_path ? d_counters + 4 : nullptr,
                   d_counters + 7);
     if (ev) CK(cudaEventRecord(ev[2], st));
+    CK(cudaGetLastError());
+    ctx->stats.kernel_launches += 2;
+    *out = ScanOut{b, n_units, max_read_len, d_survivors, d_counters, thread_path, nullptr};
+    return TREW_OK;
+}
+
+int launch_exact_stage(trew_ctx* ctx, const ScanOut* p, int n, unsigned char** d_scratch, size_t* scratch_bytes, cudaStream_t st) {
+    if (n < 1 || n > kPoolBatches) return fail(ctx, TREW_ERR_ARG, "exact stage of %d batches", n);
+    uint32_t max_len = 0;
+    for (int i = 0; i < n; i++) max_len = std::max(max_len, p[i].max_read_len);
+    unsigned int stride, s_cap, max_slices;
+    size_t long_off;
+    size_t need = scratch_need(ctx, max_len, p[0].n_units, &stride, &long_off, &s_cap, &max_slices);
+    if (need > *scratch_bytes) {
+        if (*d_scratch) { CK(cudaStreamSynchronize(st)); CK(cudaFree(*d_scratch)); *d_scratch = nullptr; }
+        CK(cudaMalloc((void**)d_scratch, need));
+        *scratch_bytes = need;
+    }
+    const bool long_thread = s_cap > 0 && p[0].n_units < (1u << 28);
+    if (long_thread && n != 1) return fail(ctx, TREW_ERR_ARG, "long-read thread path: one batch per exact stage");
+    auto seg = [](const ScanOut& o, const unsigned int* list, const unsigned int* count, int reverse) {
+        ExactSeg g{};
+        g.b = o.b; g.list = list; g.count = count; g.reverse = reverse; g.packed_probes = o.n_units < (1u << 28) ? 1 : 0;
+        g.hard = o.d_survivors + o.n_units; g.n_hard = o.d_counters + 3;
+        return g;
+    };
+    ExactPool tp{}, wp{};
+    for (int i = 0; i < n; i++) {
+        const ScanOut& o = p[i];
+        if (o.thread_path) {
+            tp.seg[tp.n_seg++] = seg(o, o.d_survivors, o.d_counters, 0);
+            wp.seg[wp.n_seg++] = seg(o, o.d_survivors + o.n_units - 1, o.d_counters + 4, 1);
+        } else if (!long_thread) {
+            wp.seg[wp.n_seg++] = seg(o, o.d_survivors, o.d_counters, 0);
+        }
+    }
+    wp.n_counted = wp.n_seg;
+    tp.n_counted = tp.n_seg;
+    for (int i = 0; i < n; i++)
+        if (p[i].thread_path || long_thread) wp.seg[wp.n_seg++] = seg(p[i], p[i].d_survivors + p[i].n_units, p[i].d_counters + 3, 0);
+    if (tp.n_seg) {
+        launch_exact_thread(ctx->dcfg, tp, ctx->d_total_surv, ctx->sm_count, env_blocks_thread(), p[0].d_counters + 6, st);
+        ctx->stats.kernel_launches += 1;
+    }
+    if (long_thread) {
+        const ScanOut& o = p[0];
+        launch_long_thread(ctx->dcfg, o.b, o.d_survivors, o.d_counters, 1, s_cap, max_slices, *d_scratch + long_off, o.d_survivors + o.n_units,
+                           o.d_counters + 3, ctx->d_total_surv, ctx->sm_count, st);
+        ctx->stats.kernel_launches += 3;
+    }
     ExactArgs a{};
-    a.survivors = d_survivors; a.n_survivors = d_counters; a.work_counter = d_counters + 1;
-    a.slice_scratch = *d_scratch; a.slice_scratch_stride = stride; a.run_cap = run_cap_for(ctx->cfg, max_read_len);
+    a.work_counter = p[0].d_counters + 1;
+    a.slice_scratch = *d_scratch; a.slice_scratch_stride = stride; a.run_cap = run_cap_for(ctx->cfg, max_len);
     a.total_survivors = ctx->d_total_surv;
-    a.packed_probes = n_units < (1u << 28) ? 1 : 0;
     a.exp_flags = ctx->exact_flags;
-    if (thread_path) {
-        unsigned int* hard = d_survivors + n_units;
-        launch_exact_thread(ctx->dcfg, b, d_survivors, d_counters, a.packed_probes, hard, d_counters + 3, ctx->d_total_surv,
-                            ctx->sm_count, env_blocks_thread(), d_counters + 6, st);
-        ExactArgs ab = a;
-        ab.survivors = d_survivors + n_units - 1; ab.reverse = 1; ab.n_survivors = d_counters + 4;
-        launch_exact(ctx->dcfg, b, ab, ctx->plan, st);
-        a.survivors = hard; a.n_survivors = d_counters + 3; a.work_counter = d_counters + 5; a.total_survivors = nullptr;
-        ctx->stats.kernel_launches += 2;
-    } else if (s_cap > 0 && n_units < (1u << 28)) {
-        unsigned int* hard = d_survivors + n_units;
-        launch_long_thread(ctx->dcfg, b, d_survivors, d_counters, a.packed_probes, s_cap, max_slices, *d_scratch + long_off, hard,
-                           d_counters + 3, ctx->d_total_surv, ctx->sm_count, st);
-        a.survivors = hard; a.n_survivors = d_counters + 3; a.total_survivors = nullptr;
-        ctx->stats.kernel_launches += 3;
-    }
-    launch_exact(ctx->dcfg, b, a, ctx->plan, st);
-    if (ev) CK(cudaEventRecord(ev[3], st));
+    launch_exact(ctx->dcfg, wp, a, ctx->plan, st);
     CK(cudaGetLastError());
-    ctx->stats.kernel_launches += 3;
+    ctx->stats.kernel_launches += 1;
     return TREW_OK;
 }
 
@@ -325,8 +359,9 @@
     b.hi = (const unsigned int*)((char*)s.d_buf + ((char*)v.hi - (char*)s.h_buf));
     b.lo = b.hi + v.plane_words; b.val = d_val;
     uint32_t n_units = ctx->cfg.mode == TREW_MODE_PAIR ? n / 2 : n;
-    rc = launch_scan(ctx, b, n_units, max_len, s.d_survivors, s.d_counters, &s.d_scratch, &s.scratch_bytes, s.stream);
-    if (rc) return rc;
+    ScanOut so;
+    if ((rc = launch_scan(ctx, b, n_units, max_len, s.d_survivors, s.d_counters, s.stream, nullptr, &so)) != TREW_OK) return rc;
+    if ((rc = launch_exact_stage(ctx, &so, 1, &s.d_scratch, &s.scratch_bytes, s.stream)) != TREW_OK) return rc;
     CK(cudaMemcpyAsync(s.h_keys, ctx->d_error + 1, sizeof(unsigned int), cudaMemcpyDeviceToHost, s.stream));
     CK(cudaEventRecord(s.ev_done, s.stream));
     s.in_flight = true;
@@ -414,16 +449,23 @@
 int collect_prof(trew_ctx* ctx) {
     for (trew_resident* r : ctx->pending_prof) {
         if (!r->ev_pending) continue;
-        CK(cudaEventSynchronize(r->ev[3]));
-        float a = 0, b = 0, c = 0;
+        CK(cudaEventSynchronize(r->ev[2]));
+        float a = 0, b = 0;
         CK(cudaEventElapsedTime(&a, r->ev[0], r->ev[1]));
         CK(cudaEventElapsedTime(&b, r->ev[1], r->ev[2]));
-        CK(cudaEventElapsedTime(&c, r->ev[2], r->ev[3]));
-        ctx->screen_ms += a; ctx->decide_ms += b; ctx->exact_ms += c; ctx->n_prof_scans++;
-        ctx->stats.device_ms += a + b + c;
+        ctx->screen_ms += a; ctx->decide_ms += b; ctx->n_prof_scans++;
+        ctx->stats.device_ms += a + b;
         r->ev_pending = false;
     }
     ctx->pending_prof.clear();
+    for (size_t i = 0; i < ctx->n_flush_ev; i++) {
+        CK(cudaEventSynchronize(ctx->flush_ev[2 * i + 1]));
+        float c = 0;
+        CK(cudaEventElapsedTime(&c, ctx->flush_ev[2 * i], ctx->flush_ev[2 * i + 1]));
+        ctx->exact_ms += c;
+        ctx->stats.device_ms += c;
+    }
+    ctx->n_flush_ev = 0;
     return TREW_OK;
 }
 
@@ -439,6 +481,29 @@
     CK(cudaEventRecord(ctx->ev_join, ctx->main_stream));
     CK(cudaStreamWaitEvent(ctx->aux_stream, ctx->ev_join, 0));
     return TREW_OK;
+}
+
+int flush_pool(trew_ctx* ctx) {
+    if (ctx->pool_pending.empty()) return TREW_OK;
+    int rc = join_aux(ctx);
+    if (rc) return rc;
+    if (ctx->flush_ev.size() < 2 * ctx->n_flush_ev + 2) {
+        for (int i = 0; i < 2; i++) {
+            cudaEvent_t e = nullptr;
+            CK(cudaEventCreate(&e));
+            ctx->flush_ev.push_back(e);
+        }
+    }
+    cudaEvent_t* ev = &ctx->flush_ev[2 * ctx->n_flush_ev];
+    CK(cudaEventRecord(ev[0], ctx->main_stream));
+    rc = launch_exact_stage(ctx, ctx->pool_pending.data(), (int)ctx->pool_pending.size(), &ctx->d_pool_scratch, &ctx->pool_scratch_bytes,
+                            ctx->main_stream);
+    ctx->pool_pending.clear();
+    if (rc) return rc;
+    CK(cudaEventRecord(ev[1], ctx->main_stream));
+    CK(cudaEventRecord(ctx->ev_b, ctx->main_stream));
+    ctx->n_flush_ev++;
+    return fork_aux(ctx);
 }
 
 int check_device_error(trew_ctx* ctx) {
@@ -615,6 +680,8 @@
     if (ctx->d_filtered) cudaFree(ctx->d_filtered);
     if (ctx->d_sort_tmp) cudaFree(ctx->d_sort_tmp);
     if (ctx->d_n) cudaFree(ctx->d_n);
+    if (ctx->d_pool_scratch) cudaFree(ctx->d_pool_scratch);
+    for (cudaEvent_t e : ctx->flush_ev) cudaEventDestroy(e);
     if (ctx->h_export) cudaFreeHost(ctx->h_export);
     if (ctx->main_stream) cudaStreamDestroy(ctx->main_stream);
     if (ctx->aux_stream) cudaStreamDestroy(ctx->aux_stream);
@@ -678,8 +745,9 @@
     b.hi = (const unsigned int*)((char*)s.d_buf + ((char*)v.hi - (char*)s.h_buf));
     b.lo = b.hi + v.plane_words; b.val = b.lo + v.plane_words;
     uint32_t n_units = ctx->cfg.mode == TREW_MODE_PAIR ? n / 2 : n;
-    rc = launch_scan(ctx, b, n_units, batch->max_read_len, s.d_survivors, s.d_counters, &s.d_scratch, &s.scratch_bytes, s.stream);
-    if (rc) return rc;
+    ScanOut so;
+    if ((rc = launch_scan(ctx, b, n_units, batch->max_read_len, s.d_survivors, s.d_counters, s.stream, nullptr, &so)) != TREW_OK) return rc;
+    if ((rc = launch_exact_stage(ctx, &so, 1, &s.d_scratch, &s.scratch_bytes, s.stream)) != TREW_OK) return rc;
     CK(cudaMemcpyAsync(s.h_keys, ctx->d_error + 1, sizeof(unsigned int), cudaMemcpyDeviceToHost, s.stream));
     CK(cudaEventRecord(s.ev_done, s.stream));
     s.in_flight = true;
@@ -720,27 +788,36 @@
     CK(cudaSetDevice(ctx->cfg.device));
     trew_resident* r = const_cast<trew_resident*>(rb);
     ctx->keys_seen = std::max<unsigned int>(ctx->keys_seen, (unsigned int)(ctx->n_slots / 16 + 1));
+    for (const ScanOut& o : ctx->pool_pending)
+        if (o.r == r) { int rc0 = flush_pool(ctx); if (rc0) return rc0; break; }
     if (r->ev_pending) { int rc0 = collect_prof(ctx); if (rc0) return rc0; }
-    if (!r->ev[0]) for (int i = 0; i < 4; i++) CK(cudaEventCreate(&r->ev[i]));
+    if (!r->ev[0]) for (int i = 0; i < 3; i++) CK(cudaEventCreate(&r->ev[i]));
     cudaStream_t st = (ctx->resident_streams == 2 && (ctx->resident_seq++ & 1)) ? ctx->aux_stream : ctx->main_stream;
     CK(cudaEventRecord(ctx->ev_a, st));
-    int rc = launch_scan(ctx, r->batch, r->n_units, r->max_read_len, r->d_survivors, r->d_counters, &r->d_scratch,
-                         &r->scratch_bytes, st, r->ev);
+    ScanOut so;
+    int rc = launch_scan(ctx, r->batch, r->n_units, r->max_read_len, r->d_survivors, r->d_counters, st, r->ev, &so);
     r->ev_pending = true; ctx->pending_prof.push_back(r);
     if (rc) return rc;
-    CK(cudaEventRecord(ctx->ev_b, st));
+    so.r = r;
+    ctx->pool_pending.push_back(so);
     ctx->stats.reads += r->n_reads; ctx->stats.bases += r->bases; ctx->stats.units += r->n_units;
+    const bool single = long_thread_path_applies(ctx->dcfg) && (ctx->exact_flags & 16u);
+    if (single || ctx->pool_pending.size() == (size_t)kPoolBatches) return flush_pool(ctx);
     return TREW_OK;
 }
 
 void trew_dev_free_resident(trew_ctx* ctx, trew_resident* r) {
     if (!r) return;
-    if (ctx) { cudaSetDevice(ctx->cfg.device); cudaStreamSynchronize(ctx->main_stream); cudaStreamSynchronize(ctx->aux_stream); collect_prof(ctx); }
-    for (int i = 0; i < 4; i++) if (r->ev[i]) cudaEventDestroy(r->ev[i]);
+    if (ctx) {
+        cudaSetDevice(ctx->cfg.device);
+        flush_pool(ctx);
+        cudaStreamSynchronize(ctx->main_stream); cudaStreamSynchronize(ctx->aux_stream);
+        collect_prof(ctx);
+    }
+    for (int i = 0; i < 3; i++) if (r->ev[i]) cudaEventDestroy(r->ev[i]);
     if (r->d_buf) cudaFree(r->d_buf);
     if (r->d_survivors) cudaFree(r->d_survivors);
     if (r->d_counters) cudaFree(r->d_counters);
-    if (r->d_scratch) cudaFree(r->d_scratch);
     delete r;
 }
 
@@ -748,6 +825,7 @@
     if (!ctx) return TREW_ERR_ARG;
     CK(cudaSetDevice(ctx->cfg.device));
     for (auto& s : ctx->slots) { int rc = retire_slot(ctx, s); if (rc) return rc; }
+    { int rc = flush_pool(ctx); if (rc) return rc; }
     { int rc = join_aux(ctx); if (rc) return rc; }
     CK(cudaStreamSynchronize(ctx->main_stream));
     { int rc = collect_prof(ctx); if (rc) return rc; }
@@ -1008,6 +1086,7 @@
 int trew_dev_get_stats(trew_ctx* ctx, trew_stats* out) {
     if (!ctx || !out) return TREW_ERR_ARG;
     CK(cudaSetDevice(ctx->cfg.device));
+    { int rc = flush_pool(ctx); if (rc) return rc; }
     unsigned long long s = 0;
     CK(cudaMemcpy(&s, ctx->d_total_surv, sizeof(s), cudaMemcpyDeviceToHost));
     ctx->stats.survivors = s;
@@ -1017,6 +1096,8 @@
 
 int trew_dev_last_resident_ms(trew_ctx* ctx, float* ms) {
     if (!ctx || !ms) return TREW_ERR_ARG;
+    CK(cudaSetDevice(ctx->cfg.device));
+    { int rc = flush_pool(ctx); if (rc) return rc; }
     CK(cudaEventSynchronize(ctx->ev_b));
     CK(cudaEventElapsedTime(ms, ctx->ev_a, ctx->ev_b));
     return TREW_OK;
@@ -1032,6 +1113,7 @@
 int trew_dev_timer_stop(trew_ctx* ctx, float* ms) {
     if (!ctx || !ms) return TREW_ERR_ARG;
     CK(cudaSetDevice(ctx->cfg.device));
+    { int rc = flush_pool(ctx); if (rc) return rc; }
     { int rc = join_aux(ctx); if (rc) return rc; }
     CK(cudaEventRecord(ctx->ev_t1, ctx->main_stream));
     CK(cudaEventSynchronize(ctx->ev_t1));
@@ -1042,6 +1124,7 @@
 int trew_dev_kernel_times(trew_ctx* ctx, double* screen_ms, double* decide_ms, double* exact_ms, uint64_t* n_scans) {
     if (!ctx) return TREW_ERR_ARG;
     CK(cudaSetDevice(ctx->cfg.device));
+    { int rc0 = flush_pool(ctx); if (rc0) return rc0; }
     { int rc0 = join_aux(ctx); if (rc0) return rc0; }
     CK(cudaStreamSynchronize(ctx->main_stream));
     int rc = collect_prof(ctx);
diff --git a/trew_b200/csrc/scan_kernels.cu b/trew_b200/csrc/scan_kernels.cu
--- a/trew_b200/csrc/scan_kernels.cu
+++ b/trew_b200/csrc/scan_kernels.cu
@@ -1611,14 +1611,33 @@
 #define TREW_THREAD_BLOCK 128
 #endif
 template <class K>
-constexpr size_t thread_kernel_smem() { return (size_t)et::Lay<K>::WORDS * TREW_THREAD_BLOCK * sizeof(u32) + (size_t)kStageSlots * 16; }
-constexpr size_t kThreadKernelSmem = thread_kernel_smem<et::u64>();
+__host__ __device__ constexpr size_t thread_work_smem(int extra_words = 0) {
+    return (size_t)(et::Lay<K>::WORDS + extra_words) * TREW_THREAD_BLOCK * sizeof(u32) + (size_t)kStageSlots * 16;
+}
+template <class K>
+constexpr size_t thread_kernel_smem() { return thread_work_smem<K>(1) + kPoolBatches * sizeof(ExactSeg) + (2 * kPoolBatches + 1) * sizeof(u32); }
+constexpr size_t kThreadKernelSmem = thread_work_smem<et::u64>();
 template <int MODE, class K>
 constexpr int thread_kernel_bps() { return (sizeof(K) == 8 ? 6 : 5) - (MODE == 1 ? 1 : 0); }
 
+struct ParamBatch {
+    const DevBatch* b;
+    __device__ __forceinline__ const DevBatch& operator()(const et::Mem&) const { return *b; }
+};
+
+template <class K>
+struct LaneBatch {
+    __device__ __forceinline__ const DevBatch& operator()(const et::Mem& m) const {
+        return reinterpret_cast<const ExactSeg*>(g_smem + thread_work_smem<K>(1))[m[et::Lay<K>::WORDS]].b;
+    }
+};
+
+template <class BatchOf>
 struct PlaneLoad {
-    et::Mem m; const u32 *hi, *lo, *val; u32 b0[2];
+    et::Mem m; BatchOf batch; u32 b0[2];
     __device__ __forceinline__ void operator()(int mate, int off, int len) const {
+        const DevBatch& b = batch(m);
+        const u32 *hi = b.hi, *lo = b.lo, *val = b.val;
         const u32 pos = b0[mate] + (u32)off, w0 = pos >> 5, sh = pos & 31u;
         for (int j = 0; j < et::kReadWords + 2; j++) {
             const u32 msk = low_mask(min(32, max(0, len - 32 * j)));
@@ -1633,19 +1652,41 @@
     }
 };
 
+__device__ __forceinline__ void pool_prefix(const ExactPool& pool, u32* s_first) {
+    static_assert(2 * kPoolBatches <= 32, "one lane per segment");
+    if (threadIdx.x >= 32) return;
+    const u32 lane = threadIdx.x;
+    u32 c = (int)lane < pool.n_seg ? *pool.seg[lane].count : 0u;
+    for (u32 d = 1; d < 32; d <<= 1) {
+        const u32 v = __shfl_up_sync(0xffffffffu, c, d);
+        if (lane >= d) c += v;
+    }
+    s_first[lane + 1] = c;
+    if (lane == 0) s_first[0] = 0u;
+}
+
+__device__ __forceinline__ int pool_segment(const u32* s_first, int n_seg, u32 i) {
+    int s = 0;
+    for (int t = 1; t < n_seg; t++) s += i >= s_first[t] ? 1 : 0;
+    return s;
+}
+
 template <int MODE, class K>
-__global__ void __launch_bounds__(TREW_THREAD_BLOCK, (thread_kernel_bps<MODE, K>())) trew_exact_thread_kernel(DevCfg cfg, DevBatch b, const u32* __restrict__ survivors,
-                                                                              const u32* __restrict__ n_survivors, int packed_probes,
-                                                                              u32* __restrict__ hard, u32* __restrict__ n_hard,
+__global__ void __launch_bounds__(TREW_THREAD_BLOCK, (thread_kernel_bps<MODE, K>())) trew_exact_thread_kernel(DevCfg cfg, const __grid_constant__ ExactPool pool,
                                                                               unsigned long long* total_survivors, u32* work_counter) {
     u32* work = reinterpret_cast<u32*>(g_smem);
-    u64* s_key = reinterpret_cast<u64*>(work + et::Lay<K>::WORDS * TREW_THREAD_BLOCK);
+    u64* s_key = reinterpret_cast<u64*>(work + (et::Lay<K>::WORDS + 1) * TREW_THREAD_BLOCK);
     u32* s_meta = reinterpret_cast<u32*>(s_key + kStageSlots);
     u32* s_cnt = s_meta + kStageSlots;
+    ExactSeg* s_seg = reinterpret_cast<ExactSeg*>(s_cnt + kStageSlots);
+    u32* s_first = reinterpret_cast<u32*>(s_seg + kPoolBatches);
     for (int i = threadIdx.x; i < kStageSlots; i += blockDim.x) { s_meta[i] = 0u; s_cnt[i] = 0u; }
+    for (int i = threadIdx.x; i < pool.n_seg; i += blockDim.x) s_seg[i] = pool.seg[i];
+    pool_prefix(pool, s_first);
     __syncthreads();
     const et::Mem m{work + threadIdx.x, TREW_THREAD_BLOCK};
-    const u32 n = *n_survivors;
+    const int n_seg = pool.n_seg;
+    const u32 n = s_first[n_seg];
     if (blockIdx.x == 0 && threadIdx.x == 0 && total_survivors) atomicAdd(total_survivors, (unsigned long long)n);
     StageEmit emit{s_meta, s_cnt, s_key, cfg.slots, cfg.slot_mask, cfg.error_flag};
     for (;;) {
@@ -1654,29 +1695,33 @@
         base = __shfl_sync(0xffffffffu, base, 0);
         if (base >= n) break;
         const u32 i = base + lane_id();
-        bool bail = false;
-        u32 entry = 0;
         if (i < n) {
-            entry = survivors[i];
-            u32 u = entry, pm = 3u;
-            if (packed_probes) { pm = entry >> kProbeShift; u &= (1u << kProbeShift) - 1u; }
+            const int s = pool_segment(s_first, n_seg, i);
+            m[et::Lay<K>::WORDS] = (u32)s;
+            const DevBatch& b = s_seg[s].b;
+            const u32 entry = s_seg[s].list[i - s_first[s]];
+            const u32 u = entry & ((1u << kProbeShift) - 1u), pm = entry >> kProbeShift;
+            bool bail;
             if (MODE == 0) {
                 const u32 b0 = __ldg(b.bit_off + u);
                 const int len = (int)(__ldg(b.bit_off + u + 1) - b0);
                 if (len > et::kMaxRead) {
                     bail = true;
                 } else {
-                    PlaneLoad load{m, b.hi, b.lo, b.val, {b0, 0u}};
+                    PlaneLoad<LaneBatch<K>> load{m, {}, {b0, 0u}};
                     bail = !et::route_short_thread<K>(m, len, pm & 7u, cfg.min_mer, cfg.max_mer, cfg.thr_low, cfg.thr_high, load, emit);
                 }
             } else {
                 const u32 a0 = __ldg(b.bit_off + 2 * u), a1 = __ldg(b.bit_off + 2 * u + 1), a2 = __ldg(b.bit_off + 2 * u + 2);
                 const int n1 = (int)(a1 - a0), n2 = (int)(a2 - a1);
-                PlaneLoad load{m, b.hi, b.lo, b.val, {a0, a1}};
+                PlaneLoad<LaneBatch<K>> load{m, {}, {a0, a1}};
                 bail = !et::route_pair_thread<K>(m, n1, n2, cfg.min_mer, cfg.max_mer, cfg.thr_low, cfg.thr_high, load, emit);
             }
-        }
-        list_append(bail, entry, hard, n_hard);
+            if (bail) {
+                const ExactSeg& sg = s_seg[m[et::Lay<K>::WORDS]];
+                sg.hard[atomicAdd(sg.n_hard, 1u)] = entry;
+            }
+        }
     }
     __syncthreads();
     for (int i = threadIdx.x; i < kStageSlots; i += blockDim.x) {
@@ -1694,7 +1739,7 @@
     unsigned long long* total_survivors;
 };
 
-__global__ void __launch_bounds__(TREW_THREAD_BLOCK, 4) trew_long_stats_kernel(DevCfg cfg, DevBatch b, LongArgs a) {
+__global__ void __launch_bounds__(TREW_THREAD_BLOCK, 4) trew_long_stats_kernel(DevCfg cfg, const __grid_constant__ DevBatch b, LongArgs a) {
     u32* work = reinterpret_cast<u32*>(g_smem);
     const et::Mem m{work + threadIdx.x, TREW_THREAD_BLOCK};
     const u32 n = min(*a.n_survivors, a.s_cap);
@@ -1707,7 +1752,7 @@
         const int len = (int)(__ldg(b.bit_off + u + 1) - b0);
         if (len < cfg.slice_len) continue;
         const et::LongGeom g(len, cfg.slice_len);
-        PlaneLoad load{m, b.hi, b.lo, b.val, {b0, 0u}};
+        PlaneLoad<ParamBatch> load{m, {&b}, {b0, 0u}};
         unsigned short* row = a.stats + (size_t)idx * (a.max_slices + 1);
         for (int t = 1 + (int)lane; t <= g.snum; t += 32) {
             u32 r = 0;
@@ -1750,7 +1795,7 @@
     }
 }
 
-__global__ void __launch_bounds__(TREW_THREAD_BLOCK, 4) trew_long_emit_kernel(DevCfg cfg, DevBatch b, LongArgs a) {
+__global__ void __launch_bounds__(TREW_THREAD_BLOCK, 4) trew_long_emit_kernel(DevCfg cfg, const __grid_constant__ DevBatch b, LongArgs a) {
     u32* work = reinterpret_cast<u32*>(g_smem);
     u64* s_key = reinterpret_cast<u64*>(work + et::Lay<et::u64>::WORDS * TREW_THREAD_BLOCK);
     u32* s_meta = reinterpret_cast<u32*>(s_key + kStageSlots);
@@ -1769,7 +1814,7 @@
         const int len = (int)(__ldg(b.bit_off + u + 1) - b0);
         if (len < cfg.slice_len) continue;
         const et::LongGeom g(len, cfg.slice_len);
-        PlaneLoad load{m, b.hi, b.lo, b.val, {b0, 0u}};
+        PlaneLoad<ParamBatch> load{m, {&b}, {b0, 0u}};
         const u32* em = a.emis + (size_t)idx * (a.max_slices + 1);
         for (int t = 1 + (int)lane; t <= g.snum; t += 32) {
             const u32 e = em[t];
@@ -1819,21 +1864,20 @@
     return cfg.mode == 1 && max_read_len >= 4u * (unsigned)cfg.max_mer;
 }
 
-void launch_exact_thread(const DevCfg& cfg, const DevBatch& b, const unsigned int* survivors, const unsigned int* n_survivors,
-                         int packed_probes, unsigned int* hard, unsigned int* n_hard, unsigned long long* total_survivors, int sm_count,
+void launch_exact_thread(const DevCfg& cfg, const ExactPool& pool, unsigned long long* total_survivors, int sm_count,
                          int blocks_per_sm, unsigned int* work_counter, cudaStream_t stream) {
     const bool wide = cfg.max_mer > 32;
 #define TREW_LAUNCH_THREAD(MODE, K)                                                                                               \
     trew_exact_thread_kernel<MODE, K><<<sm_count * (blocks_per_sm > 0 ? blocks_per_sm : thread_kernel_bps<MODE, K>()),            \
-                                        TREW_THREAD_BLOCK, thread_kernel_smem<K>(), stream>>>(                                    \
-        cfg, b, survivors, n_survivors, packed_probes, hard, n_hard, total_survivors, work_counter)
+                                        TREW_THREAD_BLOCK, thread_kernel_smem<K>(), stream>>>(cfg, pool, total_survivors, work_counter)
     if (cfg.mode == 0) { if (wide) TREW_LAUNCH_THREAD(0, et::u128); else TREW_LAUNCH_THREAD(0, et::u64); }
     else               { if (wide) TREW_LAUNCH_THREAD(1, et::u128); else TREW_LAUNCH_THREAD(1, et::u64); }
 #undef TREW_LAUNCH_THREAD
 }
 
 template <int MODE>
-__global__ void __launch_bounds__(kExactWarps * 32, TREW_EXACT_BPS) trew_exact_kernel(DevCfg cfg, DevBatch b, ExactArgs a) {
+__global__ void __launch_bounds__(kExactWarps * 32, TREW_EXACT_BPS) trew_exact_kernel(DevCfg cfg, const __grid_constant__ ExactPool pool, ExactArgs a) {
+    __shared__ u32 s_first[2 * kPoolBatches + 1];
     const int wid = threadIdx.x >> 5;
     const u32 lane = lane_id();
     WS ws;
@@ -1841,20 +1885,25 @@
     ws.off = (u32)((size_t)wid * exact_warp_bytes(a.run_cap)); ws.lane = lane; ws.flags = a.exp_flags;
     TableRef tr{cfg.slots, cfg.slot_mask, cfg.error_flag};
     ws.hdr()[lane] = lane == HD_CUR_LEN || lane == HD_EV_LEN || lane == HD_EV_K ? 0xffffffffu : 0u;
-    __syncwarp();
-    const u32 n = *a.n_survivors;
-    if (blockIdx.x == 0 && threadIdx.x == 0 && a.total_survivors) atomicAdd(a.total_survivors, (u64)n);
+    pool_prefix(pool, s_first);
+    __syncthreads();
+    const int n_seg = pool.n_seg;
+    const u32 n = s_first[n_seg];
+    if (blockIdx.x == 0 && threadIdx.x == 0 && a.total_survivors) atomicAdd(a.total_survivors, (u64)s_first[pool.n_counted]);
     unsigned char* scratch = a.slice_scratch + (size_t)(blockIdx.x * kExactWarps + wid) * a.slice_scratch_stride;
     for (;;) {
         u32 idx = 0;
         if (lane == 0) idx = atomicAdd(a.work_counter, 1u);
         idx = __shfl_sync(0xffffffffu, idx, 0);
         if (idx >= n) break;
-        u32 u = a.reverse ? *(a.survivors - idx) : a.survivors[idx], pm = 0xfu;
-        if (a.packed_probes) { pm = u >> kProbeShift; u &= (1u << kProbeShift) - 1u; }
-        if constexpr (MODE == 0) route_short(cfg, tr, ws, b, u, pm);
-        else if constexpr (MODE == 1) route_pair(cfg, tr, ws, b, u);
-        else route_long(cfg, tr, ws, b, u, scratch);
+        const int s = pool_segment(s_first, n_seg, idx);
+        const ExactSeg& sg = pool.seg[s];
+        const u32 j = idx - s_first[s];
+        u32 u = sg.reverse ? *(sg.list - j) : sg.list[j], pm = 0xfu;
+        if (sg.packed_probes) { pm = u >> kProbeShift; u &= (1u << kProbeShift) - 1u; }
+        if constexpr (MODE == 0) route_short(cfg, tr, ws, sg.b, u, pm);
+        else if constexpr (MODE == 1) route_pair(cfg, tr, ws, sg.b, u);
+        else route_long(cfg, tr, ws, sg.b, u, scratch);
     }
 }
 
@@ -1877,12 +1926,12 @@
 
 LaunchPlan default_launch_plan(int sm_count) { return LaunchPlan{sm_count * 128, sm_count * 4, sm_count * kExactBlocksPerSM}; }
 
-void launch_exact(const DevCfg& cfg, const DevBatch& b, const ExactArgs& a, const LaunchPlan& plan, cudaStream_t stream) {
+void launch_exact(const DevCfg& cfg, const ExactPool& pool, const ExactArgs& a, const LaunchPlan& plan, cudaStream_t stream) {
     size_t smem = exact_smem_bytes(a.run_cap, true);
     dim3 grid(plan.exact_blocks), block(kExactWarps * 32);
-    if (cfg.mode == 0) trew_exact_kernel<0><<<grid, block, smem, stream>>>(cfg, b, a);
-    else if (cfg.mode == 1) trew_exact_kernel<1><<<grid, block, smem, stream>>>(cfg, b, a);
-    else trew_exact_kernel<2><<<grid, block, smem, stream>>>(cfg, b, a);
-}
-
-}
+    if (cfg.mode == 0) trew_exact_kernel<0><<<grid, block, smem, stream>>>(cfg, pool, a);
+    else if (cfg.mode == 1) trew_exact_kernel<1><<<grid, block, smem, stream>>>(cfg, pool, a);
+    else trew_exact_kernel<2><<<grid, block, smem, stream>>>(cfg, pool, a);
+}
+
+}
diff --git a/trew_b200/csrc/scan_kernels.cuh b/trew_b200/csrc/scan_kernels.cuh
--- a/trew_b200/csrc/scan_kernels.cuh
+++ b/trew_b200/csrc/scan_kernels.cuh
@@ -35,16 +35,30 @@
     const unsigned int* val;
 };
 
+constexpr int kPoolBatches = 16;
+
+struct ExactSeg {
+    DevBatch b;
+    const unsigned int* list;
+    const unsigned int* count;
+    unsigned int* hard;
+    unsigned int* n_hard;
+    int reverse;
+    int packed_probes;
+};
+
+struct ExactPool {
+    ExactSeg seg[2 * kPoolBatches];
+    int n_seg;
+    int n_counted;
+};
+
 struct ExactArgs {
-    const unsigned int* survivors;
-    const unsigned int* n_survivors;
     unsigned int* work_counter;
     unsigned char* slice_scratch;
     unsigned int slice_scratch_stride;
     int run_cap;
     unsigned long long* total_survivors;
-    int packed_probes;
-    int reverse;
     unsigned int exp_flags;
 };
 
@@ -57,7 +71,7 @@
                    unsigned int* surv_b_top, unsigned int* n_surv_b, unsigned int* work_counter);
 size_t exact_smem_bytes(int run_cap, bool wide);
 cudaError_t prepare_exact(int run_cap_max);
-void launch_exact(const DevCfg& cfg, const DevBatch& b, const ExactArgs& a, const LaunchPlan& plan, cudaStream_t stream);
+void launch_exact(const DevCfg& cfg, const ExactPool& pool, const ExactArgs& a, const LaunchPlan& plan, cudaStream_t stream);
 int exact_warps_total(int sm_count);
 bool long_thread_path_applies(const DevCfg& cfg);
 size_t long_thread_scratch_bytes(unsigned int s_cap, unsigned int max_slices);
@@ -65,8 +79,7 @@
                         int packed_probes, unsigned int s_cap, unsigned int max_slices, unsigned char* scratch, unsigned int* hard,
                         unsigned int* n_hard, unsigned long long* total_survivors, int sm_count, cudaStream_t stream);
 bool thread_path_applies(const DevCfg& cfg, unsigned int max_read_len);
-void launch_exact_thread(const DevCfg& cfg, const DevBatch& b, const unsigned int* survivors, const unsigned int* n_survivors,
-                         int packed_probes, unsigned int* hard, unsigned int* n_hard, unsigned long long* total_survivors, int sm_count,
+void launch_exact_thread(const DevCfg& cfg, const ExactPool& pool, unsigned long long* total_survivors, int sm_count,
                          int blocks_per_sm, unsigned int* work_counter, cudaStream_t stream);
 void launch_compact(const Slot* slots, unsigned int n_slots, trew_entry* out, unsigned int* d_n, cudaStream_t stream, unsigned int cap);
 cudaError_t sort_entries_radix(const trew_entry* d_entries, trew_entry* d_out, unsigned int n, bool wide, void* d_temp,
```

Result: faster. 1058, median of 6 (+2.2%).
